# Krual-T/OutfitX

Hardware: AMD Instinct MI355X
Metric: outfits/sec CP forward (8-item sets, 224^2, bf16) (higher is better)
Workload: dtype f16

## Files before the change

include/ofx.h:

```cpp
#ifndef OFX_H
#define OFX_H
#include <stddef.h>
#include <stdint.h>

#ifdef __cplusplus
extern "C" {
#endif

#define OFX_ABI_VERSION 6

enum { OFX_OK = 0, OFX_EINVAL = -1, OFX_ESHAPE = -2, OFX_EHIP = -3, OFX_EWORKSPACE = -4, OFX_ESTATE = -5 };
enum ofx_dtype { OFX_F32 = 0, OFX_BF16 = 1, OFX_F16 = 2 };
enum ofx_act { OFX_ACT_NONE = 0, OFX_ACT_QUICK_GELU = 1, OFX_ACT_GELU = 2, OFX_ACT_MISH = 3, OFX_ACT_MISH_GRAD = 4 };
enum ofx_precision { OFX_PREC_BF16 = 0, OFX_PREC_F16 = 1, OFX_PREC_BF16X3 = 2, OFX_PREC_F16W2 = 3 };
enum ofx_out_kind { OFX_OUT_F32 = 0, OFX_OUT_OP = 1, OFX_OUT_SPLIT3 = 2 };

typedef struct ofx_handle ofx_handle;
typedef void* ofx_stream;

const char* ofx_last_error(void);
int ofx_abi_version(void);

typedef struct ofx_model_desc {
    int d_model, n_head, d_ffn, n_layers, max_items;
    int outfit_act;
    int outfit_precision;
    int vit_width, vit_layers, vit_heads, vit_mlp, vit_patch, vit_image, vit_act;
    int txt_width, txt_layers, txt_heads, txt_mlp, txt_vocab, txt_max_pos, txt_act, txt_eos_id;
    int proj_dim;
    int tower_precision;
    float ln_eps;
    int vit_w2_mask, txt_x3, proj_x3, vit_x3;
    int txt_w2_mask, vit_w2_qkv_layers, vit_w2_fc1_layers, vit_w2_out_layers, vit_w2_fc2_layers;
} ofx_model_desc;
enum { OFX_W2_PATCH = 1, OFX_W2_QKV = 2, OFX_W2_OUT = 4, OFX_W2_FC1 = 8, OFX_W2_FC2 = 16 };

void ofx_default_desc(ofx_model_desc* d);

ofx_handle* ofx_create(int device, const ofx_model_desc* desc);
void ofx_destroy(ofx_handle* h);

int ofx_pack_outfit_weights(ofx_handle* h, const void* const* fp32_params, int n_params, ofx_stream stream);
int ofx_pack_vision_weights(ofx_handle* h, const void* const* fp32_params, int n_params, ofx_stream stream);
int ofx_pack_text_weights(ofx_handle* h, const void* const* fp32_params, int n_params, ofx_stream stream);

enum ofx_op { OFX_OP_SET_ENCODER = 0, OFX_OP_VIT = 1, OFX_OP_TEXT = 2, OFX_OP_TOPK = 3 };
size_t ofx_workspace_bytes(ofx_handle* h, int op, int n, int len);

int ofx_set_encoder_fwd(ofx_handle* h, const float* x, const uint8_t* pad_mask, const float* prefix,
                        int prefix_stride, int B, int L, float* out_row0, void* ws, size_t ws_bytes,
                        ofx_stream stream);
int ofx_cp_head(ofx_handle* h, const float* row0, int B, float* logits, ofx_stream stream);
int ofx_cir_head(ofx_handle* h, const float* row0, int B, float* emb, void* ws, size_t ws_bytes, ofx_stream stream);
int ofx_cir_prefix(ofx_handle* h, const float* target_text_emb, int B, float* prefix_out, ofx_stream stream);

int ofx_vit_b32_fwd(ofx_handle* h, const float* pixels, int N, float* emb, int emb_ld, int emb_col,
                    int normalize, void* ws, size_t ws_bytes, ofx_stream stream);
int ofx_clip_text_fwd(ofx_handle* h, const int64_t* ids, const int64_t* attn_mask, const int* lengths_host,
                      int N, int T, float* emb, int emb_ld, int emb_col, int normalize, void* ws,
                      size_t ws_bytes, ofx_stream stream);
int ofx_clip_text_fwd_shared(ofx_handle* h, const int64_t* ids, const int64_t* attn_mask, const int* lengths_host,
                             int N, int T, float* emb, int emb_ld, int emb_col, int normalize, int shared_first, void* ws,
                             size_t ws_bytes, ofx_stream stream);

int ofx_fitb_argmin(const float* y_hat, const float* cand, int B, int C, int D, int64_t* idx, float* dist,
                    ofx_stream stream);
int ofx_fitb_argmin_indexed(const float* table, int ld, long long n_table, const int* cand_index, const float* y_hat, int B, int C, int D,
                            const int64_t* answer, int64_t* idx, float* dist, int* n_correct, ofx_stream stream);
// ... 32 lines not shown
int ofx_cp_train_fwd_indexed(ofx_handle* h, const float* table, int ld, long long n_table, const int* item_index, const int* cu_items,
                             int B, int max_len, float* logits, void* tape, size_t tape_bytes, void* ws, size_t ws_bytes,
                             float dropout_p, unsigned seed, ofx_stream stream);
int ofx_cir_train_fwd(ofx_handle* h, const float* x, const uint8_t* pad_mask, const float* table, int ld, long long n_table,
                      const int* item_index, const int* cu_items, const float* target_text, int B, int L, float* y, void* tape,
                      size_t tape_bytes, void* ws, size_t ws_bytes, float dropout_p, unsigned seed, ofx_stream stream);
int ofx_cir_train_bwd(ofx_handle* h, void* tape, size_t tape_bytes, const float* dy, int B, int L, float* grads, size_t grad_floats,
                      void* ws, size_t ws_bytes, float dropout_p, unsigned seed, ofx_stream stream);
int ofx_cp_train_bwd_into(ofx_handle* h, void* tape, size_t tape_bytes, const float* dlogits, int B, int L, float* const* grad_ptrs,
                          int n_ptrs, int accumulate, void* ws, size_t ws_bytes, float dropout_p, unsigned seed, ofx_stream stream);
int ofx_cir_train_bwd_into(ofx_handle* h, void* tape, size_t tape_bytes, const float* dy, int B, int L, float* const* grad_ptrs,
                           int n_ptrs, int accumulate, void* ws, size_t ws_bytes, float dropout_p, unsigned seed, ofx_stream stream);
int ofx_train_arm_layer_events(ofx_handle* h, void* const* events, int n);
int ofx_dropout_mask(float dropout_p, unsigned seed, int site, int rows, int cols, float* out, ofx_stream stream);
int ofx_focal_loss(const float* logits, const float* labels, int B, float alpha, float gamma, float upstream, float* loss, float* dlogits,
                   ofx_stream stream);
int ofx_focal_loss_ex(const float* logits, const float* labels, int B, float alpha, float gamma, float upstream, int reduction, float* loss,
                      float* per_elem, float* dlogits, ofx_stream stream);
size_t ofx_set_rank_loss_ws_bytes(int B, int K, int D);
int ofx_set_rank_loss(const float* y, const float* y_hat, const float* neg, const uint8_t* neg_mask, int B, int K, int D, float margin,
                      float upstream, float* loss, float* dy_hat, float* d_pos, float* d_neg, void* ws, size_t ws_bytes, ofx_stream stream);
int ofx_set_rank_loss_indexed(const float* table, int ld, long long n_table, const int* pos_index, const int* neg_index, const float* y_hat,
                              int B, int K, int D, float margin, float upstream, float* loss, float* dy_hat, float* d_pos, float* d_neg,
                              void* ws, size_t ws_bytes, ofx_stream stream);

int ofx_cir_sample_batch(const int* outfit_cu, const int* outfit_rows, int n_outfits, int n_outfit_rows, const int* pos_cu, const int* pos_slots,
                         int n_pos_slots, const int* pool_cu, const int* pool_rows, int n_pools, int n_pool_rows, const int* row_pool,
                         const int* row_slot, int n_table, const int* outfit_ids, int B, unsigned seed, unsigned draw, int K, int max_len,
                         int* item_index, int* cu_seqlens, int* target_item_index, int* neg_items_index, ofx_stream stream);

typedef struct ofx_opt_segment { float* param; long long offset; long long numel; } ofx_opt_segment;
size_t ofx_adamw_step_ws_bytes(long long n_arena);
int ofx_adamw_step(const ofx_opt_segment* segments, int n_segments, float* grad, float* exp_avg, float* exp_avg_sq, long long n_arena,
                   float* step, double lr, double beta1, double beta2, double eps, double weight_decay, double max_norm, double grad_scale,
                   float* grad_norm, int* skipped, void* ws, size_t ws_bytes, ofx_stream stream);

void ofx_profile_enable(int on);
int ofx_profile_read(double* ms, double* flops, long long* launches);
typedef struct ofx_prof_record { int cat, M, N, K, kind, kmul; float ms; double flops; double bytes; } ofx_prof_record;
int ofx_profile_records(ofx_prof_record* out, int cap);

int ofx_tune(int knob, int value);
unsigned ofx_config_generation(void);
int ofx_profile_enabled(void);
int ofx_stream_create_low_priority(int device, ofx_stream* out);
int ofx_stream_destroy(ofx_stream stream);

int ofx_gemm(const void* A, const void* W, void* C, const float* bias, const float* resid, int M, int N, int K,
             int lda, int ldc, int ldr, int act, int out_kind, int op_dtype, ofx_stream stream);
int ofx_gemm_w2(const void* A, const void* W2, void* C, const float* bias, const float* resid, int M, int N, int K,
                int lda, int ldc, int ldr, int act, int out_kind, int op_dtype, ofx_stream stream);
int ofx_gemm_x3(const void* A3, const void* W3, void* C, const float* bias, const float* resid, int M, int N, int K,
                int lda, int ldc, int ldr, int act, int out_kind, int op_dtype, ofx_stream stream);
int ofx_pack_lo8(const void* W2, void* W8, void* scale8, int N, int K, ofx_stream stream);
int ofx_gemm_w2f8(const void* A, const void* W2, const void* W8, const void* scale8, void* C, const float* bias, const float* resid, int M, int N, int K,
                  int lda, int ldc, int ldr, int act, int out_kind, ofx_stream stream);
int ofx_gemm_w2f8_fold(const void* A, const void* W2, const void* W8, const void* scale8, void* C, const float* bias, const float* row_stat, const float* col_sum,
                       int M, int N, int K, int lda, int ldc, int act, ofx_stream stream);
size_t ofx_gemm_tn_ws(int M, int N, int K);
int ofx_gemm_tn(const void* A, int lda, const void* B, int ldb, float* C, int ldc, int M, int N, int K, const int* k_dev,
                void* slab, size_t slab_bytes, int op_dtype, ofx_stream stream);
size_t ofx_gemm_splitk_ws(int M, int N, int K);
int ofx_gemm_splitk(const void* A, const void* W, void* C, const float* bias, const float* resid, int M, int N, int K,
                    int lda, int ldc, int ldr, int act, int out_kind, int op_dtype, void* slab, size_t slab_bytes, ofx_stream stream);
int ofx_gemm_train(const void* A, const void* W, void* C, const float* bias, const float* resid, float* aux_out, int M, const int* m_dev,
                   int N, int K, int lda, int ldc, int ldr, int act, int out_kind, float dropout_p, unsigned seed, int site, int op_dtype,
                   void* slab, size_t slab_bytes, ofx_stream stream);
int ofx_gemm_tn_into(const void* A, int lda, const void* B, int ldb, float* C, int ldc, int M, int N, int K, const int* k_dev,
                     int m_valid, int n_valid, int accumulate, void* slab, size_t slab_bytes, int op_dtype, ofx_stream stream);
int ofx_transpose_cast(const float* src, void* dst, int R, int C, int ldd, void* row_dst, int ld_row, int op_dtype, ofx_stream stream);
size_t ofx_layernorm_bwd_ws(int D);
int ofx_layernorm_bwd(const float* dy, const float* x, const float* stats, const float* gamma, const float* add, const int* add_map,
                      float* dx, void* dx_op, float* dgamma, float* dbeta, float* dcols, int M, const int* m_dev, int D, float dropout_p,
                      unsigned seed, int site, int accumulate, int op_dtype, void* ws, size_t ws_bytes, ofx_stream stream);
size_t ofx_colsum_ws(int C);
int ofx_colsum(const void* x, int x_kind, int ld, const int* gather, const float* row_scale, float* out0, float* out1, float* out2, int seg,
               int C, int valid, int M, const int* m_dev, int accumulate, int op_dtype, void* ws, size_t ws_bytes, ofx_stream stream);
int ofx_head_bwd(const float* dlogits, const float* w, const int* cu, float* dX, void* dXb, float* db, int B, int D, float dropout_p,
                 unsigned seed, int head_site, int below_site, int accumulate, int op_dtype, ofx_stream stream);
int ofx_gemm_fold_producer(const void* A, const void* W, const void* W8, const void* scale8, void* xb, void* xlo, float* stat_part, const float* bias,
                           const float* resid, int M, int N, int K, int lda, int ldr, int act, int w_form, int op_dtype, ofx_stream stream);
int ofx_gemm_fold(const void* A, const void* W, void* C, const float* bias, const float* row_stat, int stat_ld, const float* col_sum, int M, int N, int K,
                  int lda, int ldc, int act, int w_form, int op_dtype, ofx_stream stream);
int ofx_stats_finalize(const float* stat_part, int slots, int W, float eps, float* stat, int rows, ofx_stream stream);
int ofx_row_stats_cast(const float* x, void* xb, void* xlo, float* stat, int rows, int W, float eps, int op_dtype, ofx_stream stream);
int ofx_fold_pack(const float* w, const float* gamma, const float* beta, const float* bias, void* wf, float* col_sum, float* bias_f, int N, int K, int split,
                  int op_dtype, ofx_stream stream);
int ofx_vit_embed_ln(const float* patch_out, const float* cls, const float* pos, const float* gamma, const float* beta, float* x, void* xb, void* xlo,
                     float* stat, int N, int S, int D, float eps, int op_dtype, ofx_stream stream);
int ofx_gather_hilo(const void* hi, const void* lo, const int* idx, float* dst, int rows, int W, int op_dtype, ofx_stream stream);
int ofx_layernorm(const float* x, const int* row_idx, const float* gamma, const float* beta, void* y, int rows,
                  int D, int ldy, int out_kind, int op_dtype, float eps, ofx_stream stream);
int ofx_attention(const void* qkv, void* out, const int64_t* key_mask, int nseq, int seq_len, int n_head, int ld,
                  int ldo, int k_off, int v_off, int mask_ld, int causal, float scale, int op_dtype, ofx_stream stream);
int ofx_attention_ex(const void* qkv, void* out, const int64_t* key_mask, int nseq, int seq_len, int n_head, int ld, int ldo, int k_off,
                     int v_off, int mask_ld, int causal, int only_row0, int split3_w, float scale, int op_dtype, ofx_stream stream);
int ofx_set_attention(const float* qkv, void* out, const int* cu_seqlens, int nseq, int n_head, int D, int ldo,
                      int out_kind, int max_len, int only_row0, float scale, int op_dtype, ofx_stream stream);
int ofx_set_attention_slabs(const float* slabs, size_t plane_floats, int splits, const float* bias, void* out, const int* cu_seqlens, int nseq,
                            int n_head, int D, int ldo, int out_kind, int max_len, int only_row0, float scale, int op_dtype, ofx_stream stream);
int ofx_splitk_reduce_ln(const float* slab, size_t plane_floats, int splits, const float* bias, const float* resid, int ldr, float* x, int ldx,
                         const float* gamma, const float* beta, void* y, int ldy, int out_kind, float eps, int rows, const int* m_dev, int D,
                         int op_dtype, ofx_stream stream);
int ofx_attention_varlen(const void* qkv, void* out, const int* cu_seqlens, int nseq, int max_len, int n_head, int ld, int ldo, int k_off,
                         int v_off, int only_row0, float scale, float dropout_p, unsigned seed, int site, int op_dtype, ofx_stream stream);
int ofx_set_attention_op(const void* qkv, void* out, const int* cu_seqlens, int nseq, int n_head, int D, int ldo, int out_kind, int max_len,
                         int only_row0, float scale, float dropout_p, unsigned seed, int site, int op_dtype, ofx_stream stream);
int ofx_set_attention_bwd(const void* qkv, const float* d_o, void* dqkv, const int* cu_seqlens, int nseq, int n_head, int D, int max_len,
                          int only_row0, float scale, float dropout_p, unsigned seed, int site, int mfma, int op_dtype, ofx_stream stream);
int ofx_fused_qkv_attention(const void* X, const void* Wqkv, const float* bias, const float* row_stat, const float* col_sum, void* out,
                            int nseq, int seq_len, int width, int n_head, int ldx, int ldo, float scale, int op_dtype, ofx_stream stream);
int ofx_fused_qkv_attention_w2(const void* X, const void* Wqkv2, const float* bias, const float* row_stat, const float* col_sum, void* out,
                               int nseq, int seq_len, int width, int n_head, int ldx, int ldo, float scale, int op_dtype, ofx_stream stream);
int ofx_attention_f32(const float* qkv, void* out, const int64_t* key_mask, int nseq, int seq_len, int n_head, int D, int ldo, int out_kind,
                      int mask_ld, int causal, float scale, int op_dtype, ofx_stream stream);
int ofx_convert(const float* src, void* dst, int rows, int cols, int mode, int op_dtype, ofx_stream stream);

#ifdef __cplusplus
}
#endif
#endif
```

outfitx_amd/_lib.py:

```python
from __future__ import annotations

import ctypes as C
import os

_HERE = os.path.dirname(os.path.abspath(__file__))
LIB_PATH = os.environ.get("OFX_LIB") or os.path.join(_HERE, "libofx_hip.so")

OFX_OK = 0
ABI_VERSION = 6
F32, BF16, F16 = 0, 1, 2
ACT_NONE, ACT_QUICK_GELU, ACT_GELU, ACT_MISH = 0, 1, 2, 3
PREC_BF16, PREC_F16, PREC_BF16X3 = 0, 1, 2
OUT_F32, OUT_OP, OUT_SPLIT3 = 0, 1, 2
OP_SET_ENCODER, OP_VIT, OP_TEXT, OP_TOPK = 0, 1, 2, 3
PREC_F16W2 = 3
PRECISIONS = {"bf16": PREC_BF16, "f16": PREC_F16, "fp16": PREC_F16, "bf16x3": PREC_BF16X3, "f16w2": PREC_F16W2}
W2_PATCH, W2_QKV, W2_OUT, W2_FC1, W2_FC2 = 1, 2, 4, 8, 16
TOWER_SCHEMES = {
    "bf16": (PREC_BF16, 0, 0, 0, 0), "f16": (PREC_F16, 0, 0, 0, 0), "fp16": (PREC_F16, 0, 0, 0, 0),
    "f16w2": (PREC_F16, W2_PATCH | W2_OUT | W2_FC2, 1, 1, 0),
    "bf16w2": (PREC_BF16, W2_PATCH | W2_OUT | W2_FC2, 1, 1, 0),
    "f16w2q": (PREC_F16, W2_PATCH | W2_QKV | W2_OUT | W2_FC2, 1, 1, 0),
    "f16w2f": (PREC_F16, W2_PATCH | W2_OUT | W2_FC1 | W2_FC2, 1, 1, 0),
    "f16w2x": (PREC_F16, W2_PATCH | W2_QKV | W2_OUT | W2_FC1 | W2_FC2, 1, 1, 0),
    "f16x3": (PREC_F16, W2_PATCH, 1, 1, 1), "bf16x3": (PREC_BF16, W2_PATCH, 1, 1, 1),
}
SCHEME_ALIASES = {"f16w2h": "f16w2x@qkv=0-5"}
DEFAULT_TOWER_PRECISION = "f16w2x"


def _layer_bits(spec: str) -> int:
    m = 0
    for part in spec.split(","):
        a, _, b = part.partition("-")
        for l in range(int(a), int(b or a) + 1):
            m |= 1 << l
    return m


def tower_scheme(name: str) -> dict:
    name = SCHEME_ALIASES.get(name, name)
    base, _, opts = name.partition("@")
    if base not in TOWER_SCHEMES:
        raise ValueError(f"unknown tower_precision {name!r}; one of {sorted(list(TOWER_SCHEMES) + list(SCHEME_ALIASES))} [+ '@txt=w2;qkv=<layers>;fc1=<layers>']")
    prec, mask, txt_x3, proj_x3, vit_x3 = TOWER_SCHEMES[base]
    d = {"tower_precision": prec, "vit_w2_mask": mask, "txt_x3": txt_x3, "proj_x3": proj_x3, "vit_x3": vit_x3,
         "txt_w2_mask": 0, "vit_w2_qkv_layers": 0, "vit_w2_fc1_layers": 0, "vit_w2_out_layers": 0, "vit_w2_fc2_layers": 0}
    for o in filter(None, opts.split(";")):
        k, _, v = o.partition("=")
        try:
            if k == "txt" and v == "w2":
                d["txt_x3"], d["txt_w2_mask"] = 0, W2_QKV | W2_OUT | W2_FC1 | W2_FC2
            elif k in ("qkv", "fc1", "out", "fc2"):
                bits = _layer_bits(v) if v not in ("", "none") else 0
                if bits == 0:
                    d["vit_w2_mask"] &= ~{"qkv": W2_QKV, "fc1": W2_FC1, "out": W2_OUT, "fc2": W2_FC2}[k]
                d[f"vit_w2_{k}_layers"] = bits
            else:
                raise ValueError
        except ValueError:
            raise ValueError(f"tower_precision {name!r}: bad option {o!r} (txt=w2 | qkv= / fc1= / out= / fc2=<layers>, layers like 0-5,8 or none)") from None
    return d
ACTS = {"none": ACT_NONE, "quick_gelu": ACT_QUICK_GELU, "gelu": ACT_GELU, "mish": ACT_MISH}


class OfxError(RuntimeError):
# ... 29 lines not shown
    "ofx_pack_outfit_weights": (_i, [_vp, C.POINTER(_vp), _i, _vp]),
    "ofx_pack_vision_weights": (_i, [_vp, C.POINTER(_vp), _i, _vp]),
    "ofx_pack_text_weights": (_i, [_vp, C.POINTER(_vp), _i, _vp]),
    "ofx_workspace_bytes": (_sz, [_vp, _i, _i, _i]),
    "ofx_set_encoder_fwd": (_i, [_vp, _vp, _vp, _vp, _i, _i, _i, _vp, _vp, _sz, _vp]),
    "ofx_cp_head": (_i, [_vp, _vp, _i, _vp, _vp]),
    "ofx_cir_head": (_i, [_vp, _vp, _i, _vp, _vp, _sz, _vp]),
    "ofx_cir_prefix": (_i, [_vp, _vp, _i, _vp, _vp]),
    "ofx_vit_b32_fwd": (_i, [_vp, _vp, _i, _vp, _i, _i, _i, _vp, _sz, _vp]),
    "ofx_clip_text_fwd": (_i, [_vp, _vp, _vp, C.POINTER(_i), _i, _i, _vp, _i, _i, _i, _vp, _sz, _vp]),
    "ofx_clip_text_fwd_shared": (_i, [_vp, _vp, _vp, C.POINTER(_i), _i, _i, _vp, _i, _i, _i, _i, _vp, _sz, _vp]),
    "ofx_fitb_argmin": (_i, [_vp, _vp, _i, _i, _i, _vp, _vp, _vp]),
    "ofx_fitb_argmin_indexed": (_i, [_vp, _i, C.c_longlong, _vp, _vp, _i, _i, _i, _vp, _vp, _vp, _vp, _vp]),
    "ofx_l2_topk": (_i, [_vp, _vp, _vp, _i, _i, _i, _i, _i64, _vp, _vp, _vp, _sz, _vp]),
    "ofx_l2_topk_grouped_ws": (_sz, [_i, _i, _i]),
    "ofx_l2_topk_grouped": (_i, [_vp, _vp, _vp, _i, _i, _i, _i, _vp, _i, _i, _vp, _vp, _vp, _vp, _vp, _sz, _vp]),
    "ofx_topk_merge": (_i, [_vp, _vp, _i, _i, _i, _vp, _vp, _vp]),
    "ofx_clip_preprocess_ws": (_sz, [_vp, _vp, _i, _i, _i]),
    "ofx_clip_preprocess": (_i, [_vp, _vp, _vp, _vp, _i, _i, _i, _vp, _vp, _vp, _vp, _sz, _vp]),
    "ofx_clip_preprocess_patches": (_i, [_vp, _vp, _vp, _vp, _i, _i, _i, _i, _vp, _vp, _vp, _i, _vp, _sz, _vp]),
    "ofx_patchify": (_i, [_vp, _vp, _i, _i, _i, _i, _vp]),
    "ofx_vit_b32_u8_ws_bytes": (_sz, [_vp, _vp, _vp, _i, _i]),
    "ofx_vit_b32_fwd_u8": (_i, [_vp, _vp, _vp, _vp, _vp, _i, _i, _vp, _vp, _vp, _i, _i, _i, _vp, _sz, _vp]),
    "ofx_set_encoder_fwd_indexed": (_i, [_vp, _vp, _i, C.c_longlong, _vp, _vp, _vp, _i, _i, _i, _vp, _vp, _sz, _vp]),
    "ofx_cp_train_fwd_indexed": (_i, [_vp, _vp, _i, C.c_longlong, _vp, _vp, _i, _i, _vp, _vp, _sz, _vp, _sz, _f, C.c_uint, _vp]),
    "ofx_cp_train_tape_bytes": (_sz, [_vp, _i, _i]),
    "ofx_cp_train_ws_bytes": (_sz, [_vp, _i, _i]),
    "ofx_cp_train_grad_floats": (_sz, [_vp, C.POINTER(_sz), _i]),
    "ofx_cp_train_fwd": (_i, [_vp, _vp, _vp, _i, _i, _vp, _vp, _sz, _vp, _sz, _f, C.c_uint, _vp]),
    "ofx_cp_train_bwd": (_i, [_vp, _vp, _sz, _vp, _i, _i, _vp, _sz, _vp, _sz, _f, C.c_uint, _vp]),
    "ofx_cir_train_fwd": (_i, [_vp, _vp, _vp, _vp, _i, C.c_longlong, _vp, _vp, _vp, _i, _i, _vp, _vp, _sz, _vp, _sz, _f, C.c_uint, _vp]),
    "ofx_cir_train_bwd": (_i, [_vp, _vp, _sz, _vp, _i, _i, _vp, _sz, _vp, _sz, _f, C.c_uint, _vp]),
    "ofx_cp_train_bwd_into": (_i, [_vp, _vp, _sz, _vp, _i, _i, C.POINTER(_vp), _i, _i, _vp, _sz, _f, C.c_uint, _vp]),
    "ofx_cir_train_bwd_into": (_i, [_vp, _vp, _sz, _vp, _i, _i, C.POINTER(_vp), _i, _i, _vp, _sz, _f, C.c_uint, _vp]),
    "ofx_train_arm_layer_events": (_i, [_vp, C.POINTER(_vp), _i]),
    "ofx_dropout_mask": (_i, [_f, C.c_uint, _i, _i, _i, _vp, _vp]),
    "ofx_focal_loss": (_i, [_vp, _vp, _i, _f, _f, _f, _vp, _vp, _vp]),
    "ofx_focal_loss_ex": (_i, [_vp, _vp, _i, _f, _f, _f, _i, _vp, _vp, _vp, _vp]),
    "ofx_set_rank_loss_ws_bytes": (_sz, [_i, _i, _i]),
    "ofx_set_rank_loss": (_i, [_vp, _vp, _vp, _vp, _i, _i, _i, _f, _f, _vp, _vp, _vp, _vp, _vp, _sz, _vp]),
    "ofx_set_rank_loss_indexed": (_i, [_vp, _i, C.c_longlong, _vp, _vp, _vp, _i, _i, _i, _f, _f, _vp, _vp, _vp, _vp, _vp, _sz, _vp]),
    "ofx_cir_sample_batch": (_i, [_vp, _vp, _i, _i, _vp, _vp, _i, _vp, _vp, _i, _i, _vp, _vp, _i, _vp, _i, C.c_uint, C.c_uint, _i, _i, _vp, _vp, _vp, _vp, _vp]),
    "ofx_adamw_step_ws_bytes": (_sz, [C.c_longlong]),
    "ofx_adamw_step": (_i, [_vp, _i, _vp, _vp, _vp, C.c_longlong, _vp] + [C.c_double] * 7 + [_vp, _vp, _vp, _sz, _vp]),
    "ofx_profile_enable": (None, [_i]),
    "ofx_profile_read": (_i, [C.POINTER(C.c_double), C.POINTER(C.c_double), C.POINTER(C.c_longlong)]),
    "ofx_profile_records": (_i, [C.POINTER(ProfRecord), _i]),
    "ofx_tune": (_i, [_i, _i]),
    "ofx_config_generation": (C.c_uint, []),
    "ofx_profile_enabled": (_i, []),
    "ofx_gemm": (_i, [_vp, _vp, _vp, _vp, _vp, _i, _i, _i, _i, _i, _i, _i, _i, _i, _vp]),
    "ofx_gemm_w2": (_i, [_vp, _vp, _vp, _vp, _vp, _i, _i, _i, _i, _i, _i, _i, _i, _i, _vp]),
    "ofx_gemm_x3": (_i, [_vp, _vp, _vp, _vp, _vp, _i, _i, _i, _i, _i, _i, _i, _i, _i, _vp]),
    "ofx_pack_lo8": (_i, [_vp, _vp, _vp, _i, _i, _vp]),
    "ofx_gemm_w2f8": (_i, [_vp, _vp, _vp, _vp, _vp, _vp, _vp, _i, _i, _i, _i, _i, _i, _i, _i, _vp]),
    "ofx_gemm_w2f8_fold": (_i, [_vp, _vp, _vp, _vp, _vp, _vp, _vp, _vp, _i, _i, _i, _i, _i, _i, _vp]),
    "ofx_gemm_tn_ws": (_sz, [_i, _i, _i]),
    "ofx_gemm_tn": (_i, [_vp, _i, _vp, _i, _vp, _i, _i, _i, _i, _vp, _vp, _sz, _i, _vp]),
    "ofx_gemm_splitk_ws": (_sz, [_i, _i, _i]),
    "ofx_gemm_splitk": (_i, [_vp, _vp, _vp, _vp, _vp, _i, _i, _i, _i, _i, _i, _i, _i, _i, _vp, _sz, _vp]),
    "ofx_gemm_train": (_i, [_vp, _vp, _vp, _vp, _vp, _vp, _i, _vp, _i, _i, _i, _i, _i, _i, _i, _f, C.c_uint, _i, _i, _vp, _sz, _vp]),
    "ofx_gemm_tn_into": (_i, [_vp, _i, _vp, _i, _vp, _i, _i, _i, _i, _vp, _i, _i, _i, _vp, _sz, _i, _vp]),
    "ofx_transpose_cast": (_i, [_vp, _vp, _i, _i, _i, _vp, _i, _i, _vp]),
    "ofx_layernorm_bwd_ws": (_sz, [_i]),
    "ofx_layernorm_bwd": (_i, [_vp] * 11 + [_i, _vp, _i, _f, C.c_uint, _i, _i, _i, _vp, _sz, _vp]),
    "ofx_colsum_ws": (_sz, [_i]),
    "ofx_colsum": (_i, [_vp, _i, _i, _vp, _vp, _vp, _vp, _vp, _i, _i, _i, _i, _vp, _i, _i, _vp, _sz, _vp]),
    "ofx_head_bwd": (_i, [_vp, _vp, _vp, _vp, _vp, _vp, _i, _i, _f, C.c_uint, _i, _i, _i, _i, _vp]),
    "ofx_gemm_fold_producer": (_i, [_vp] * 9 + [_i] * 8 + [_vp]),
    "ofx_gemm_fold": (_i, [_vp, _vp, _vp, _vp, _vp, _i, _vp, _i, _i, _i, _i, _i, _i, _i, _i, _vp]),
    "ofx_stats_finalize": (_i, [_vp, _i, _i, _f, _vp, _i, _vp]),
    "ofx_row_stats_cast": (_i, [_vp, _vp, _vp, _vp, _i, _i, _f, _i, _vp]),
    "ofx_fold_pack": (_i, [_vp] * 7 + [_i, _i, _i, _i, _vp]),
    "ofx_vit_embed_ln": (_i, [_vp] * 9 + [_i, _i, _i, _f, _i, _vp]),
    "ofx_gather_hilo": (_i, [_vp, _vp, _vp, _vp, _i, _i, _i, _vp]),
    "ofx_layernorm": (_i, [_vp, _vp, _vp, _vp, _vp, _i, _i, _i, _i, _i, _f, _vp]),
    "ofx_attention": (_i, [_vp, _vp, _vp, _i, _i, _i, _i, _i, _i, _i, _i, _i, _f, _i, _vp]),
    "ofx_attention_ex": (_i, [_vp, _vp, _vp, _i, _i, _i, _i, _i, _i, _i, _i, _i, _i, _i, _f, _i, _vp]),
    "ofx_set_attention_slabs": (_i, [_vp, _sz, _i, _vp, _vp, _vp, _i, _i, _i, _i, _i, _i, _i, _f, _i, _vp]),
    "ofx_splitk_reduce_ln": (_i, [_vp, _sz, _i, _vp, _vp, _i, _vp, _i, _vp, _vp, _vp, _i, _i, _f, _i, _vp, _i, _i, _vp]),
    "ofx_fused_qkv_attention": (_i, [_vp, _vp, _vp, _vp, _vp, _vp, _i, _i, _i, _i, _i, _i, _f, _i, _vp]),
    "ofx_fused_qkv_attention_w2": (_i, [_vp, _vp, _vp, _vp, _vp, _vp, _i, _i, _i, _i, _i, _i, _f, _i, _vp]),
    "ofx_set_attention": (_i, [_vp, _vp, _vp, _i, _i, _i, _i, _i, _i, _i, _f, _i, _vp]),
    "ofx_attention_varlen": (_i, [_vp, _vp, _vp, _i, _i, _i, _i, _i, _i, _i, _i, _f, _f, C.c_uint, _i, _i, _vp]),
    "ofx_set_attention_op": (_i, [_vp, _vp, _vp, _i, _i, _i, _i, _i, _i, _i, _f, _f, C.c_uint, _i, _i, _vp]),
    "ofx_set_attention_bwd": (_i, [_vp, _vp, _vp, _vp, _i, _i, _i, _i, _i, _f, _f, C.c_uint, _i, _i, _i, _vp]),
    "ofx_attention_f32": (_i, [_vp, _vp, _vp, _i, _i, _i, _i, _i, _i, _i, _i, _f, _i, _vp]),
    "ofx_convert": (_i, [_vp, _vp, _i, _i, _i, _i, _vp]),
}

_lib = None


def load() -> C.CDLL:
    global _lib
    if _lib is not None:
        return _lib
    if not os.path.exists(LIB_PATH):
        raise OfxError(f"{LIB_PATH} not found: build it with `make` (or __graft_entry__.build()); "
                       "outfitx_amd has no CPU/PyTorch fallback for the scoring path")
    lib = C.CDLL(LIB_PATH)
    for name, (res, args) in SIGNATURES.items():
        fn = getattr(lib, name)
        fn.restype, fn.argtypes = res, args
    if lib.ofx_abi_version() != ABI_VERSION:
        raise OfxError("libofx_hip.so ABI version mismatch; rebuild")
    for kv in filter(None, os.environ.get("OFX_TUNE", "").split(",")):
        knob, _, val = kv.partition(":")
        if lib.ofx_tune(int(knob), int(val)) != OFX_OK:
            raise OfxError(f"OFX_TUNE: ofx_tune({knob}, {val}) was refused")
    _lib = lib
    return lib


def check(rc: int, what: str = "") -> None:
    if rc != OFX_OK:
        msg = load().ofx_last_error()
        raise OfxError(f"{what or 'ofx call'} failed (code {rc}): {msg.decode() if msg else ''}")


def default_desc() -> ModelDesc:
    d = ModelDesc()
    load().ofx_default_desc(C.byref(d))
    return d
```

outfitx_amd/csrc/api.hip:

```cpp
#include <stdarg.h>
#include <string.h>

#include <algorithm>
#include <vector>
#include <mutex>
#include <cstring>

#include "ofx_weights.h"

static thread_local char g_err[512] = "";
void ofx_set_error(const char* fmt, ...) {
    va_list ap;
    va_start(ap, fmt);
    vsnprintf(g_err, sizeof(g_err), fmt, ap);
    va_end(ap);
}
extern "C" const char* ofx_last_error(void) { return g_err; }
extern "C" int ofx_abi_version(void) { return OFX_ABI_VERSION; }
extern "C" int ofx_stream_create_low_priority(int device, ofx_stream* out) {
    OFX_REQUIRE(out, OFX_EINVAL, "stream_create_low_priority: NULL argument");
    int prev = 0, least = 0, greatest = 0;
    OFX_HIP(hipGetDevice(&prev));
    OFX_HIP(hipSetDevice(device));
    hipStream_t s = nullptr;
// ... 499 lines not shown
    if (fused) {
        TRY(ofx_launch_fused_qkv_attn(w.XB, L.qkv.w, L.qkv.bias, w.S, L.qkv.col_sum, w.H, nseq, S, W, heads, W, W, 0.125f, dt, s, L.qkv.form == W_SPLIT));
    } else {
        GemmArgs g1{}; g1.A = w.XB; g1.C = w.QKV; g1.row_stat = w.S; g1.M = rows; g1.N = 3 * W;
        g1.ldc = 3 * W; g1.act = OFX_ACT_NONE; g1.out_kind = OFX_OUT_OP;
        use_gemm(g1, L.qkv, W);
        const bool prune = pool_idx && pool_first && g_prune_q;
        if (prune) {
            GemmArgs kv = g1;
            kv.W = (const char*)g1.W + (size_t)W * g1.K * 2; kv.bias = g1.bias + W; kv.col_sum = g1.col_sum + W; kv.C = (char*)w.QKV + (size_t)W * 2; kv.N = 2 * W;
            if (g1.W8) { kv.W8 = (const char*)g1.W8 + (size_t)W * W; kv.w8_scale = (const char*)g1.w8_scale + W; }
            TRY(ofx_launch_gemm(kv, dt, s));
            GemmArgs q = g1;
            q.M = nseq; q.N = W; q.lda = S * W; q.ldc = S * 3 * W; q.stat_ld = S;
            TRY(ofx_launch_gemm(q, dt, s));
        } else
            TRY(ofx_launch_gemm(g1, dt, s));
        AttnArgs at{w.QKV, w.H, key_mask, nseq, S, heads, 3 * W, W, W, 2 * W, mask_ld, causal, 0.125f};
        at.only_row0 = prune ? 1 : 0;
        TRY(ofx_launch_attention_mfma(at, dt, s));
    }
    char* H = w.H; char* U = w.U; int M = rows;
    if (pool_idx) {
        TRY(ofx_launch_gather_rows(w.H, pool_idx, w.HP, nseq, W * 2, W * 2, s));
        TRY(ofx_launch_gather_hilo(w.XB, w.XLO, pool_idx, w.XP, nseq, W, dt, s));
        H = w.HP; U = w.UP; M = nseq;
    }
    auto to_stream = [&](GemmArgs& g) {
        g.M = M; g.N = W; g.ldc = W; g.ldr = W; g.act = OFX_ACT_NONE;
        if (pool_idx) { g.C = w.XP; g.resid = w.XP; g.out_kind = OFX_OUT_F32; g.slab = w.slab; g.slab_bytes = w.slab_bytes; }
        else { g.C = w.XB; g.xb_out = w.XB; g.xlo = w.XLO; g.stat_part = w.P; g.out_kind = OFX_OUT_OP; }
    };
    GemmArgs g2{}; g2.A = H;
    use_gemm(g2, L.o, W); to_stream(g2);
    TRY(ofx_launch_gemm(g2, dt, s));
    GemmArgs g3{}; g3.C = U; g3.M = M; g3.N = MLP; g3.ldc = MLP; g3.act = act; g3.out_kind = OFX_OUT_OP;
    if (pool_idx) {
        LnArgs ln2{w.XP, nullptr, L.g2, L.be2, H, M, W, W, OFX_OUT_OP, eps};
        TRY(ofx_launch_layernorm(ln2, dt, s));
        g3.A = H; g3.slab = w.slab; g3.slab_bytes = w.slab_bytes;
    } else {
        TRY(ofx_launch_stats_finalize(w.P, W / 64, W, eps, w.S, M, s));
        g3.A = w.XB; g3.row_stat = w.S;
    }
    use_gemm(g3, L.fc1, W);
    TRY(ofx_launch_gemm(g3, dt, s));
    GemmArgs g4{}; g4.A = U;
    use_gemm(g4, L.fc2, MLP); to_stream(g4);
    TRY(ofx_launch_gemm(g4, dt, s));
    if (!pool_idx) TRY(ofx_launch_stats_finalize(w.P, W / 64, W, eps, w.S, M, s));
    return OFX_OK;
}

static int clip_layer_x3(const ClipLayer& L, const ClipWs& w, int rows, int nseq, int S, int W, int MLP, int heads, int act,
                         float eps, int causal, const int64_t* key_mask, int mask_ld, int dt, const int* pool_idx, hipStream_t s, bool mfma_attn = false,
                         int shared_first = 0) {
    LnArgs ln{w.X, nullptr, L.g1, L.be1, w.H, rows, W, 3 * W, OFX_OUT_SPLIT3, eps};
    TRY(ofx_launch_layernorm(ln, dt, s));
    GemmArgs g1{}; g1.A = w.H; g1.C = w.QKV; g1.M = rows; g1.N = 3 * W;
    use_gemm(g1, L.qkv, W);
    const bool f32_attn = S <= 64 && !mfma_attn;
    OFX_REQUIRE(!shared_first || f32_attn, OFX_EINVAL, "clip_layer_x3: a shared first row needs the fp32 set attention");
    g1.ldc = 3 * W; g1.act = OFX_ACT_NONE; g1.out_kind = f32_attn ? OFX_OUT_F32 : OFX_OUT_OP;
    TRY(ofx_launch_gemm(g1, dt, s));
    if (f32_attn) {
        SetAttnArgs sa{w.QKV, w.H, nullptr, nseq, heads, W, 3 * W, OFX_OUT_SPLIT3, S, 0, 0.125f};
        sa.fixed_len = S; sa.causal = causal; sa.key_mask = key_mask; sa.mask_ld = mask_ld; sa.shared_first = shared_first;
        TRY(ofx_launch_set_attention(sa, dt, s));
    } else {
        AttnArgs at{w.QKV, w.H, key_mask, nseq, S, heads, 3 * W, 3 * W, W, 2 * W, mask_ld, causal, 0.125f};
        at.split3_w = W;
        TRY(ofx_launch_attention_mfma(at, dt, s));
    }
    float* X = w.X; char* H = w.H; char* U = w.U; int M = rows;
    if (pool_idx) {
        TRY(ofx_launch_gather_rows(w.H, pool_idx, w.HP, nseq, 3 * W * 2, 3 * W * 2, s));
        TRY(ofx_launch_gather_rows(w.X, pool_idx, w.XP, nseq, W * 4, W * 4, s));
        X = w.XP; H = w.HP; U = w.UP; M = nseq;
    }
    GemmArgs g2{}; g2.A = H; g2.C = X; g2.resid = X; g2.M = M; g2.N = W; g2.ldc = W; g2.ldr = W; g2.act = OFX_ACT_NONE; g2.out_kind = OFX_OUT_F32;
    use_gemm(g2, L.o, W);
    if (pool_idx) { g2.slab = w.slab; g2.slab_bytes = w.slab_bytes; }
    TRY(ofx_launch_gemm(g2, dt, s));
    LnArgs ln2{X, nullptr, L.g2, L.be2, H, M, W, 3 * W, OFX_OUT_SPLIT3, eps};
    TRY(ofx_launch_layernorm(ln2, dt, s));
    GemmArgs g3{}; g3.A = H; g3.C = U; g3.M = M; g3.N = MLP; g3.ldc = 3 * MLP; g3.act = act; g3.out_kind = OFX_OUT_SPLIT3;
    use_gemm(g3, L.fc1, W);
    if (pool_idx) { g3.slab = w.slab; g3.slab_bytes = w.slab_bytes; }
    TRY(ofx_launch_gemm(g3, dt, s));
    GemmArgs g4{}; g4.A = U; g4.C = X; g4.resid = X; g4.M = M; g4.N = W; g4.ldc = W; g4.ldr = W; g4.act = OFX_ACT_NONE; g4.out_kind = OFX_OUT_F32;
    use_gemm(g4, L.fc2, MLP);
    if (pool_idx) { g4.slab = w.slab; g4.slab_bytes = w.slab_bytes; }
    return ofx_launch_gemm(g4, dt, s);
}

static int clip_layers(const std::vector<ClipLayer>& Ls, const ClipWs& w, int rows, int nseq, int S, int W, int MLP,
                       int heads, int act, float eps, int causal, const int64_t* key_mask, int mask_ld, int dt,
                       const int* pool_idx, hipStream_t s, bool pool_first, bool x3, int shared_first = 0) {
    OFX_REQUIRE(!shared_first || x3, OFX_EINVAL, "clip_layers: a shared first row exists in the three-product path only");
    if (x3) {
        for (size_t l = 0; l < Ls.size(); ++l)
            TRY(clip_layer_x3(Ls[l], w, rows, nseq, S, W, MLP, heads, act, eps, causal, key_mask, mask_ld, dt, l + 1 == Ls.size() ? pool_idx : nullptr, s, !causal && !key_mask && !g_x3_vit_f32_attn,
                              shared_first));
        return OFX_OK;
    }
    for (size_t l = 0; l < Ls.size(); ++l)
        TRY(clip_layer(Ls[l], w, rows, nseq, S, W, MLP, heads, act, eps, causal, key_mask, mask_ld, dt,
                       l + 1 == Ls.size() ? pool_idx : nullptr, s, pool_first));
    return OFX_OK;
}

struct RawImages {
    const uint8_t* src; const long long* offsets; const int* heights; const int* widths; int channels; const float* mean; const float* stdv;
    void* ws; size_t ws_bytes;
};

static int vit_core(ofx_handle* h, const float* pixels, const RawImages* raw, int N, float* emb, int emb_ld, int emb_col,
                    int normalize, void* ws, size_t ws_bytes, ofx_stream stream) {
    OFX_REQUIRE(h && h->vis_ready, OFX_ESTATE, "vit_b32_fwd: vision weights not packed");
    OFX_REQUIRE((pixels || raw) && emb && ws && N > 0, OFX_EINVAL, "vit_b32_fwd: bad argument");
    const ofx_model_desc& d = h->d;
    OFX_REQUIRE(emb_ld >= emb_col + d.proj_dim && emb_ld % 4 == 0 && emb_col % 4 == 0, OFX_ESHAPE, "vit_b32_fwd: bad emb_ld/emb_col");
    hipStream_t s = (hipStream_t)stream;
    const int g = d.vit_image / d.vit_patch, S = g * g + 1, W = d.vit_width, KP = 3 * d.vit_patch * d.vit_patch, dt = h->tw_dtype;
    int chunk = std::min(N, VIT_CHUNK_MAX);
    while (chunk > 1 && vit_bytes(h, chunk, nullptr, nullptr, ~(size_t)0) > ws_bytes) chunk = (chunk + 1) / 2;
    OFX_REQUIRE(vit_bytes(h, chunk, nullptr, nullptr, ~(size_t)0) <= ws_bytes, OFX_EWORKSPACE, "vit_b32_fwd: workspace %zu bytes cannot hold one image", ws_bytes);
    const size_t px_per_img = (size_t)3 * d.vit_image * d.vit_image;
    for (int n0 = 0; n0 < N; n0 += chunk) {
        const int n = std::min(chunk, N - n0);
        ClipWs w;
        vit_bytes(h, n, &w, ws, ws_bytes);
        const int rows = n * S;
        if (raw)
            TRY(ofx_preprocess_to(raw->src, raw->offsets + n0, raw->heights + n0, raw->widths + n0, n, raw->channels, d.vit_image, raw->mean, raw->stdv,
                                  nullptr, w.U, d.vit_patch, dt, raw->ws, raw->ws_bytes, s));
        else
            TRY(ofx_launch_patchify(pixels + (size_t)n0 * px_per_img, w.U, n, d.vit_image, d.vit_patch, dt, s));
        GemmArgs gp{}; gp.A = w.U; gp.C = w.QKV; gp.M = n * g * g; gp.N = W; gp.ldc = W;
        gp.act = OFX_ACT_NONE; gp.out_kind = OFX_OUT_F32;
        use_gemm(gp, h->v_patch, KP);
        TRY(ofx_launch_gemm(gp, dt, s));
        TRY(ofx_launch_vit_embed_ln((const float*)w.QKV, h->v_cls, h->v_pos, h->v_pre_g, h->v_pre_b, w.X, n, S, W, d.ln_eps, s, w.XB, w.S, dt, w.XLO));
        TRY(ofx_launch_iota_rows(w.idx, n, S, s));
        TRY(clip_layers(h->vl, w, rows, n, S, W, d.vit_mlp, d.vit_heads, d.vit_act, d.ln_eps, 0, nullptr, 0, dt, w.idx, s, true, h->vit_x3 != 0));
// ... 430 lines not shown
extern "C" int ofx_cir_sample_batch(const int* outfit_cu, const int* outfit_rows, int n_outfits, int n_outfit_rows, const int* pos_cu, const int* pos_slots,
                                    int n_pos_slots, const int* pool_cu, const int* pool_rows, int n_pools, int n_pool_rows, const int* row_pool,
                                    const int* row_slot, int n_table, const int* outfit_ids, int B, unsigned seed, unsigned draw, int K, int max_len,
                                    int* item_index, int* cu_seqlens, int* target_item_index, int* neg_items_index, ofx_stream stream) {
    OFX_REQUIRE(B >= 1, OFX_EINVAL, "cir_sample_batch: B = %d; needs B >= 1", B);
    OFX_REQUIRE(K >= 0 && K <= 64 && max_len >= 1 && max_len <= 31, OFX_ESHAPE, "cir_sample_batch: K = %d, max_len = %d; needs 0 <= K <= 64, 1 <= max_len <= 31",
                K, max_len);
    OFX_REQUIRE(n_outfits >= 1 && n_table >= 1 && n_outfit_rows >= 0 && n_pos_slots >= 0 && n_pools >= 0 && n_pool_rows >= 0, OFX_ESHAPE,
                "cir_sample_batch: n_outfits = %d, n_table = %d (both >= 1), n_outfit_rows = %d, n_pos_slots = %d, n_pools = %d, n_pool_rows = %d (all >= 0)",
                n_outfits, n_table, n_outfit_rows, n_pos_slots, n_pools, n_pool_rows);
    OFX_REQUIRE((long long)B * std::max(K, max_len) <= INT_MAX, OFX_ESHAPE, "cir_sample_batch: B * max(K, max_len) = %lld exceeds INT_MAX",
                (long long)B * std::max(K, max_len));
    const void* ptrs[] = {outfit_cu, outfit_rows, pos_cu, pos_slots, pool_cu, pool_rows, row_pool, row_slot, outfit_ids, item_index, cu_seqlens, target_item_index};
    uintptr_t bits = (uintptr_t)neg_items_index;
    for (const void* p : ptrs) {
        OFX_REQUIRE(p, OFX_EINVAL, "cir_sample_batch: NULL argument");
        bits |= (uintptr_t)p;
    }
    OFX_REQUIRE(neg_items_index || K == 0, OFX_EINVAL, "cir_sample_batch: NULL neg_items_index with K = %d", K);
    OFX_REQUIRE((bits & 15) == 0, OFX_EINVAL, "cir_sample_batch: every array must be 16-byte aligned");
    CirSampleArgs a{outfit_cu, outfit_rows, pos_cu, pos_slots, pool_cu, pool_rows, row_pool, row_slot, outfit_ids,
                    n_outfits, n_outfit_rows, n_pos_slots, n_pools, n_pool_rows, n_table, B, K, max_len, seed, draw,
                    item_index, cu_seqlens, target_item_index, neg_items_index};
    return ofx_launch_cir_sample_batch(a, (hipStream_t)stream);
}

static bool adamw_shape_ok(long long n_arena) { return n_arena > 0 && n_arena % 64 == 0; }
extern "C" size_t ofx_adamw_step_ws_bytes(long long n_arena) { return adamw_shape_ok(n_arena) ? ofx_adamw_step_ws(n_arena) : 0; }
extern "C" int ofx_adamw_step(const ofx_opt_segment* segments, int n_segments, float* grad, float* exp_avg, float* exp_avg_sq, long long n_arena,
                              float* step, double lr, double beta1, double beta2, double eps, double weight_decay, double max_norm, double grad_scale,
                              float* grad_norm, int* skipped, void* ws, size_t ws_bytes, ofx_stream stream) {
    OFX_REQUIRE(segments && grad && exp_avg && exp_avg_sq && step && grad_norm && skipped && ws, OFX_EINVAL, "adamw_step: NULL argument");
    OFX_REQUIRE(n_segments >= 1 && n_segments <= 1024, OFX_ESHAPE, "adamw_step: n_segments = %d; needs 1 <= n_segments <= 1024", n_segments);
    OFX_REQUIRE(adamw_shape_ok(n_arena), OFX_ESHAPE, "adamw_step: n_arena = %lld; needs a positive multiple of 64", n_arena);
    OFX_REQUIRE((((uintptr_t)grad | (uintptr_t)exp_avg | (uintptr_t)exp_avg_sq | (uintptr_t)ws) & 15) == 0 && ((uintptr_t)segments & 7) == 0, OFX_EINVAL,
                "adamw_step: grad, exp_avg, exp_avg_sq and ws must be 16-byte aligned, segments 8-byte aligned");
    OFX_REQUIRE(ws_bytes >= ofx_adamw_step_ws(n_arena), OFX_EWORKSPACE, "adamw_step: workspace %zu < %zu bytes", ws_bytes, ofx_adamw_step_ws(n_arena));
    return ofx_launch_adamw_step(segments, n_segments, grad, exp_avg, exp_avg_sq, n_arena, step, lr, beta1, beta2, eps, weight_decay, max_norm,
                                 grad_scale, grad_norm, skipped, ws, (hipStream_t)stream);
}

extern "C" int ofx_tune(int knob, int value) {
    ++g_config_generation;
    switch (knob) {
        case 2: case 5: case 11: case 15: case 16: case 18: return ofx_gemm_tune(knob, value);
        case 6: if (value != 2) { ofx_set_error("ofx_tune(6): %d is not 2 (the towers' LayerNorms are always folded)", value); return OFX_EINVAL; } return OFX_OK;
        case 7: g_train_mfma_attn = value; return OFX_OK;
        case 8: g_prune_q = value; return OFX_OK;
        case 9: g_fuse_qkv = value; return OFX_OK;
        case 10: g_set_fuse = value; return OFX_OK;
        case 17: g_topk_filter = value != 0; return OFX_OK;
        case 20: g_x3_vit_f32_attn = value != 0; return OFX_OK;
        case 21: g_text_shared_first = value != 0; return OFX_OK;
        default: ofx_set_error("ofx_tune: unknown knob %d", knob); return OFX_EINVAL;
    }
}

static GemmArgs op_gemm(const void* A, const void* W, void* C, const float* bias, const float* resid, int M, int N, int K, int lda, int ldc, int ldr,
                        int act, int out_kind) {
    GemmArgs g{}; g.A = A; g.W = W; g.C = C; g.bias = bias; g.resid = resid; g.M = M; g.N = N; g.K = K; g.lda = lda; g.ldc = ldc;
    g.ldr = ldr; g.act = act; g.out_kind = out_kind;
    return g;
}
extern "C" int ofx_gemm(const void* A, const void* W, void* C, const float* bias, const float* resid, int M, int N, int K,
                        int lda, int ldc, int ldr, int act, int out_kind, int op_dtype, ofx_stream stream) {
    return ofx_launch_gemm(op_gemm(A, W, C, bias, resid, M, N, K, lda, ldc, ldr, act, out_kind), op_dtype, (hipStream_t)stream);
}
extern "C" int ofx_gemm_w2(const void* A, const void* W2, void* C, const float* bias, const float* resid, int M, int N, int K,
                           int lda, int ldc, int ldr, int act, int out_kind, int op_dtype, ofx_stream stream) {
    GemmArgs g = op_gemm(A, W2, C, bias, resid, M, N, 2 * K, lda, ldc, ldr, act, out_kind); g.a_wrap = K;
    return ofx_launch_gemm(g, op_dtype, (hipStream_t)stream);
}
extern "C" int ofx_gemm_x3(const void* A3, const void* W3, void* C, const float* bias, const float* resid, int M, int N, int K,
                           int lda, int ldc, int ldr, int act, int out_kind, int op_dtype, ofx_stream stream) {
    GemmArgs g = op_gemm(A3, W3, C, bias, resid, M, N, 3 * K, lda, ldc, ldr, act, out_kind); g.k_mult = 3;
    return ofx_launch_gemm(g, op_dtype, (hipStream_t)stream);
}
extern "C" int ofx_pack_lo8(const void* W2, void* W8, void* scale8, int N, int K, ofx_stream stream) {
    return ofx_launch_pack_lo8(W2, W8, scale8, N, K, (hipStream_t)stream);
}
extern "C" int ofx_gemm_w2f8(const void* A, const void* W2, const void* W8, const void* scale8, void* C, const float* bias, const float* resid, int M, int N, int K,
                             int lda, int ldc, int ldr, int act, int out_kind, ofx_stream stream) {
    GemmArgs g = op_gemm(A, W2, C, bias, resid, M, N, 2 * K, lda, ldc, ldr, act, out_kind); g.a_wrap = K; g.W8 = W8; g.w8_scale = scale8;
    return ofx_launch_gemm(g, OFX_F16, (hipStream_t)stream);
}
extern "C" int ofx_gemm_w2f8_fold(const void* A, const void* W2, const void* W8, const void* scale8, void* C, const float* bias, const float* row_stat, const float* col_sum,
                                  int M, int N, int K, int lda, int ldc, int act, ofx_stream stream) {
    OFX_REQUIRE(row_stat && col_sum, OFX_EINVAL, "gemm_w2f8_fold: row_stat and col_sum are required");
    GemmArgs g = op_gemm(A, W2, C, bias, nullptr, M, N, 2 * K, lda, ldc, 0, act, OFX_OUT_OP); g.a_wrap = K; g.W8 = W8; g.w8_scale = scale8;
    g.row_stat = row_stat; g.col_sum = col_sum; g.stat_ld = 1;
    return ofx_launch_gemm(g, OFX_F16, (hipStream_t)stream);
}
extern "C" size_t ofx_gemm_splitk_ws(int M, int N, int K) { return ofx_gemm_splitk_bytes(M, N, K); }
extern "C" int ofx_gemm_splitk(const void* A, const void* W, void* C, const float* bias, const float* resid, int M, int N, int K,
                               int lda, int ldc, int ldr, int act, int out_kind, int op_dtype, void* slab, size_t slab_bytes, ofx_stream stream) {
    GemmArgs g = op_gemm(A, W, C, bias, resid, M, N, K, lda, ldc, ldr, act, out_kind); g.slab = slab; g.slab_bytes = slab_bytes;
    return ofx_launch_gemm(g, op_dtype, (hipStream_t)stream);
}
extern "C" size_t ofx_gemm_tn_ws(int M, int N, int K) { return ofx_gemm_tn_slab_bytes(M, N, K); }
extern "C" int ofx_gemm_tn(const void* A, int lda, const void* B, int ldb, float* C, int ldc, int M, int N, int K, const int* k_dev,
                           void* slab, size_t slab_bytes, int op_dtype, ofx_stream stream) {
    return ofx_launch_gemm_tn(A, lda, B, ldb, C, ldc, M, N, K, k_dev, slab, slab_bytes, op_dtype, (hipStream_t)stream);
}
static bool op_dtype_ok(int op_dtype) { return op_dtype == OFX_BF16 || op_dtype == OFX_F16; }
static bool drop_p_ok(float p) { return p >= 0.f && p < 1.f; }
static bool aligned_to(size_t mask, std::initializer_list<const void*> ptrs) {
    for (const void* p : ptrs) if ((uintptr_t)p & mask) return false;
    return true;
}
extern "C" int ofx_gemm_train(const void* A, const void* W, void* C, const float* bias, const float* resid, float* aux_out, int M, const int* m_dev,
                              int N, int K, int lda, int ldc, int ldr, int act, int out_kind, float dropout_p, unsigned seed, int site, int op_dtype,
                              void* slab, size_t slab_bytes, ofx_stream stream) {
    OFX_REQUIRE(A && W && C && drop_p_ok(dropout_p) && (act != OFX_ACT_MISH_GRAD || resid), OFX_EINVAL, "gemm_train: bad argument");
    OFX_REQUIRE(aligned_to(15, {bias, resid, aux_out, slab}) && aligned_to(3, {m_dev}), OFX_EINVAL,
                "gemm_train: bias, resid, aux_out and slab must be 16-byte aligned");
    GemmArgs g = op_gemm(A, W, C, bias, resid, M, N, K, lda, ldc, ldr, act, out_kind); g.slab = slab; g.slab_bytes = slab_bytes;
    g.aux_out = aux_out; g.m_dev = m_dev; g.drop = make_drop(dropout_p, seed, (unsigned)site);
    return ofx_launch_gemm(g, op_dtype, (hipStream_t)stream);
}
extern "C" int ofx_gemm_tn_into(const void* A, int lda, const void* B, int ldb, float* C, int ldc, int M, int N, int K, const int* k_dev,
                                int m_valid, int n_valid, int accumulate, void* slab, size_t slab_bytes, int op_dtype, ofx_stream stream) {
    OFX_REQUIRE(A && B && C && m_valid >= 0 && n_valid >= 0, OFX_EINVAL, "gemm_tn_into: bad argument");
    OFX_REQUIRE(aligned_to(15, {slab}) && aligned_to(3, {k_dev}), OFX_EINVAL, "gemm_tn_into: slab must be 16-byte aligned");
    return ofx_launch_gemm_tn(A, lda, B, ldb, C, ldc, M, N, K, k_dev, slab, slab_bytes, op_dtype, (hipStream_t)stream, m_valid, n_valid, accumulate ? 1 : 0);
}
extern "C" int ofx_transpose_cast(const float* src, void* dst, int R, int C, int ldd, void* row_dst, int ld_row, int op_dtype, ofx_stream stream) {
    OFX_REQUIRE(src && dst && op_dtype_ok(op_dtype), OFX_EINVAL, "transpose_cast: bad argument");
    OFX_REQUIRE(aligned_to(3, {src}) && aligned_to(1, {dst, row_dst}), OFX_EINVAL, "transpose_cast: misaligned pointer");
    OFX_REQUIRE(R > 0 && C > 0, OFX_ESHAPE, "transpose_cast: R=%d C=%d", R, C);
// ... 149 lines not shown
                                    const float* gamma, const float* beta, void* y, int ldy, int out_kind, float eps, int rows, const int* m_dev, int D,
                                    int op_dtype, ofx_stream stream) {
    OFX_REQUIRE(slab && x && gamma && beta && y && op_dtype_ok(op_dtype) && aligned_to(15, {slab, bias, resid, x, gamma, beta}) && aligned_to(out_kind == 0 ? 15 : 7, {y}) && aligned_to(3, {m_dev}) &&
                    plane_floats % 4 == 0,
                OFX_EINVAL, "splitk_reduce_ln: bad argument (a NULL or misaligned pointer or op_dtype = %d)", op_dtype);
    OFX_REQUIRE(out_kind >= 0 && out_kind <= 2 && (splits <= 1 || plane_floats >= (size_t)rows * D), OFX_ESHAPE, "splitk_reduce_ln: out_kind=%d, or slabs that overlap", out_kind);
    SplitKLnArgs a{slab, plane_floats, splits, bias, resid, ldr, x, ldx, gamma, beta, y, ldy, out_kind, eps, rows, D, m_dev};
    return ofx_launch_splitk_reduce_ln(a, op_dtype, (hipStream_t)stream);
}
extern "C" int ofx_fused_qkv_attention(const void* X, const void* Wqkv, const float* bias, const float* row_stat, const float* col_sum, void* out,
                                       int nseq, int seq_len, int width, int n_head, int ldx, int ldo, float scale, int op_dtype, ofx_stream stream) {
    return ofx_launch_fused_qkv_attn(X, Wqkv, bias, row_stat, col_sum, out, nseq, seq_len, width, n_head, ldx, ldo, scale, op_dtype, (hipStream_t)stream);
}
extern "C" int ofx_fused_qkv_attention_w2(const void* X, const void* Wqkv2, const float* bias, const float* row_stat, const float* col_sum, void* out,
                                          int nseq, int seq_len, int width, int n_head, int ldx, int ldo, float scale, int op_dtype, ofx_stream stream) {
    return ofx_launch_fused_qkv_attn(X, Wqkv2, bias, row_stat, col_sum, out, nseq, seq_len, width, n_head, ldx, ldo, scale, op_dtype, (hipStream_t)stream, true);
}
extern "C" int ofx_set_attention(const float* qkv, void* out, const int* cu_seqlens, int nseq, int n_head, int D, int ldo,
                                 int out_kind, int max_len, int only_row0, float scale, int op_dtype, ofx_stream stream) {
    SetAttnArgs a{qkv, out, cu_seqlens, nseq, n_head, D, ldo, out_kind, max_len, only_row0, scale};
    return ofx_launch_set_attention(a, op_dtype, (hipStream_t)stream);
}
static bool train_attn_args_ok(const void* a, const void* b, const void* c, int nseq, float dropout_p) {
    return a && b && c && nseq > 0 && dropout_p >= 0.f && dropout_p < 1.f;
}
extern "C" int ofx_attention_varlen(const void* qkv, void* out, const int* cu_seqlens, int nseq, int max_len, int n_head, int ld, int ldo, int k_off,
                                    int v_off, int only_row0, float scale, float dropout_p, unsigned seed, int site, int op_dtype, ofx_stream stream) {
    OFX_REQUIRE(train_attn_args_ok(qkv, out, cu_seqlens, nseq, dropout_p), OFX_EINVAL, "attention_varlen: bad argument");
    OFX_REQUIRE(n_head > 0 && k_off == n_head * 64 && v_off == 2 * k_off && ld >= 3 * k_off, OFX_ESHAPE,
                "attention_varlen: q | k | v rows of D = n_head * 64 columns (k_off=%d v_off=%d ld=%d n_head=%d); heads of 96 take ofx_set_attention", k_off, v_off, ld, n_head);
    AttnArgs a{qkv, out, nullptr, nseq, max_len, n_head, ld, ldo, k_off, v_off, 0, 0, scale};
    a.cu_seqlens = cu_seqlens; a.only_row0 = only_row0 ? 1 : 0; a.drop = make_drop(dropout_p, seed, (unsigned)site);
    return ofx_launch_attention_mfma(a, op_dtype, (hipStream_t)stream);
}
extern "C" int ofx_set_attention_op(const void* qkv, void* out, const int* cu_seqlens, int nseq, int n_head, int D, int ldo, int out_kind, int max_len,
                                    int only_row0, float scale, float dropout_p, unsigned seed, int site, int op_dtype, ofx_stream stream) {
    OFX_REQUIRE(train_attn_args_ok(qkv, out, cu_seqlens, nseq, dropout_p) && n_head > 0, OFX_EINVAL, "set_attention_op: bad argument");
    SetAttnArgs a{qkv, out, cu_seqlens, nseq, n_head, D, ldo, out_kind, max_len, only_row0 ? 1 : 0, scale};
    a.drop = make_drop(dropout_p, seed, (unsigned)site); a.qkv_op = 1;
    return ofx_launch_set_attention(a, op_dtype, (hipStream_t)stream);
}
extern "C" int ofx_set_attention_bwd(const void* qkv, const float* d_o, void* dqkv, const int* cu_seqlens, int nseq, int n_head, int D, int max_len,
                                     int only_row0, float scale, float dropout_p, unsigned seed, int site, int mfma, int op_dtype, ofx_stream stream) {
    OFX_REQUIRE(train_attn_args_ok(qkv, d_o, dqkv, nseq, dropout_p) && cu_seqlens && n_head > 0, OFX_EINVAL, "set_attention_bwd: bad argument");
    const auto launch = mfma ? ofx_launch_set_attention_bwd_mfma : ofx_launch_set_attention_bwd;
    return launch(qkv, d_o, dqkv, cu_seqlens, nseq, n_head, D, max_len, scale, op_dtype, make_drop(dropout_p, seed, (unsigned)site), only_row0 ? 1 : 0, (hipStream_t)stream);
}
extern "C" int ofx_attention_f32(const float* qkv, void* out, const int64_t* key_mask, int nseq, int seq_len, int n_head, int D, int ldo, int out_kind,
                                 int mask_ld, int causal, float scale, int op_dtype, ofx_stream stream) {
    SetAttnArgs a{qkv, out, nullptr, nseq, n_head, D, ldo, out_kind, seq_len, 0, scale};
    a.fixed_len = seq_len; a.causal = causal; a.key_mask = key_mask; a.mask_ld = mask_ld;
    return ofx_launch_set_attention(a, op_dtype, (hipStream_t)stream);
}
extern "C" int ofx_convert(const float* src, void* dst, int rows, int cols, int mode, int op_dtype, ofx_stream stream) {
    return ofx_launch_pack_rows(src, dst, rows, rows, cols, cols, cols, mode, op_dtype, (hipStream_t)stream);
}
```

outfitx_amd/csrc/attention.hip:

```cpp
#include "attn_wave.h"

namespace {

struct AttnK {
    const char* qkv;
    char* out;
    const int64_t* key_mask;
    int nseq, S, n_head, ld, ldo, k_off, v_off, mask_ld, causal;
    float scale;
    const int* cu;
    int only_row0;
    DropArgs drop;
    int split3_w;
};

template <typename T, int NT>
__global__ __launch_bounds__(256, 3) void attention_mfma_kernel(AttnK a) {
    typedef typename OpT<T>::v8 v8;
    constexpr int KS = attn_ksteps(NT), VROWS = 32 * KS, VT = VROWS * ATTN_V_ROW;
    __shared__ __attribute__((aligned(16))) char smem[4 * VT];
    const int lane = threadIdx.x & 63, wave = threadIdx.x >> 6;
    const int npairs = a.nseq * a.n_head;
    const int pair_raw = blockIdx.x * 4 + wave;
    const bool live = pair_raw < npairs;
    const int pair = live ? pair_raw : npairs - 1;
    const int seq = pair / a.n_head, head = pair % a.n_head;
    const int row_first = a.cu ? a.cu[seq] : seq * a.S;
    const int S = a.cu ? min(a.cu[seq + 1] - row_first, 16 * NT) : a.S;
    const T* base = (const T*)a.qkv + (size_t)row_first * a.ld + head * 64;
    const int r16 = lane & 15, q4 = lane >> 4;

    OFX_LDS char* vl = (OFX_LDS char*)smem + wave * VT;
#pragma unroll
    for (int it = 0; it < VROWS / 8; ++it) {
        const int key = it * 8 + (lane >> 3);
        v8 val;
#pragma unroll
        for (int e = 0; e < 8; ++e) val[e] = (T)0.0f;
        if (key < S) val = *(const v8*)(base + (size_t)key * a.ld + a.v_off + (lane & 7) * 8);
        *(OFX_LDS v8*)(vl + key * ATTN_V_ROW + (lane & 7) * 16) = val;
    }

    v8 kf[NT][2], qf[NT][2];
#pragma unroll
    for (int t = 0; t < NT; ++t) {
        int row = 16 * t + r16;
        row = row < S ? row : S - 1;
        const T* rp = base + (size_t)row * a.ld + q4 * 8;
#pragma unroll
        for (int ks = 0; ks < 2; ++ks) {
            kf[t][ks] = *(const v8*)(rp + a.k_off + ks * 32);
            qf[t][ks] = *(const v8*)(rp + ks * 32);
        }
// ... 148 lines not shown
        for (int c = 0; c < C4; ++c) {
            const f32x4 x = qp[c], y = kp[c];
            d += x[0] * y[0] + x[1] * y[1] + x[2] * y[2] + x[3] * y[3];
        }
        bool dead = a.causal && j > i;
        if (!dead && a.key_mask) dead = a.key_mask[(size_t)mb * a.mask_ld + j] == 0;
        sc[i * (SMAX + 4) + j] = dead ? -INFINITY : d * a.scale;
    }
    __syncthreads();
    if (lane >= q0 && lane < nq) {
        float* row = sc + lane * (SMAX + 4);
        float m = -INFINITY;
        for (int j = 0; j < S; ++j) m = fmaxf(m, row[j]);
        if (m == -INFINITY) m = 0.f;
        float sum = 0.f;
        for (int j = 0; j < S; ++j) { const float e = expf(row[j] - m); row[j] = e; sum += e; }
        const float inv = sum > 0.f ? 1.0f / sum : 0.f;
        if (a.drop.thresh) for (int j = 0; j < S; ++j) row[j] *= inv * drop_mul(a.drop, blockIdx.x, lane * 32 + j);
        else for (int j = 0; j < S; ++j) row[j] *= inv;
    }
    __syncthreads();
    if (a.out_kind == 0) {
        for (int i = q0; i < nq; ++i) {
            const float* row = sc + i * (SMAX + 4);
            float acc = 0.f;
#pragma unroll
            for (int j = 0; j < SMAX; ++j) acc += (j < S ? row[j] : 0.f) * vreg[j];
            ((float*)a.out)[(size_t)row_of(i) * a.ldo + h * HD + lane] = acc;
            if constexpr (WIDE) {
                float acc2 = 0.f;
#pragma unroll
                for (int j = 0; j < SMAX; ++j) acc2 += (j < S ? row[j] : 0.f) * vreg2[j];
                if (two) ((float*)a.out)[(size_t)row_of(i) * a.ldo + h * HD + 64 + lane] = acc2;
            }
        }
        return;
    }
    for (int i = q0; i < nq; ++i) {
        const float* row = sc + i * (SMAX + 4);
        float acc = 0.f;
#pragma unroll
        for (int j = 0; j < SMAX; ++j) acc += (j < S ? row[j] : 0.f) * vreg[j];
        qs[i * STR + lane] = acc;
        if constexpr (WIDE) {
            float acc2 = 0.f;
#pragma unroll
            for (int j = 0; j < SMAX; ++j) acc2 += (j < S ? row[j] : 0.f) * vreg2[j];
            if (two) qs[i * STR + 64 + lane] = acc2;
        }
    }
    __syncthreads();
    auto store_row = [&](int i, int c8) {
        const f32x4 x0 = *(const f32x4*)(qs + i * STR + c8), x1 = *(const f32x4*)(qs + i * STR + c8 + 4);
        store8<T>(a.out, (size_t)row_of(i) * a.ldo + h * HD + c8, x0, x1, a.out_kind, D);
    };
    if constexpr (!WIDE) {
        const int c8 = (lane & 7) * 8, r8 = lane >> 3;
        for (int i0 = 0; i0 < nq; i0 += 8) {
            const int i = i0 + r8;
            if (i >= q0 && i < nq) store_row(i, c8);
        }
    } else {
        for (int f = lane + q0 * C8; f < nq * C8; f += 64) store_row(f / C8, (f % C8) * 8);
    }
}


struct AttnBwdK {
    const char* qkv;
    const float* d_o;
    char* dqkv;
    const int* cu;
    int nseq, n_head, D, only_row0;
    float scale;
    DropArgs drop;
};

__device__ __forceinline__ float drop_dp(float dp, float mk) {
#pragma clang fp contract(off)
    return dp * mk;
}

template <typename T, int NT>
__global__ __launch_bounds__(256) void set_attention_bwd_mfma_kernel(AttnBwdK a) {
    typedef typename OpT<T>::v8 v8;
    typedef typename OpT<T>::v4 v4;
    constexpr int KS = attn_ksteps(NT), VROWS = 32 * KS, VT = VROWS * ATTN_V_ROW;
    __shared__ __attribute__((aligned(16))) char smem[4 * 3 * VT];
    const int lane = threadIdx.x & 63, wave = threadIdx.x >> 6;
    const int npairs = a.nseq * a.n_head;
    const int pair_raw = blockIdx.x * 4 + wave;
    const bool live = pair_raw < npairs;
    const int pair = live ? pair_raw : npairs - 1;
    const int seq = pair / a.n_head, head = pair % a.n_head;
    const int D = a.D, ld = 3 * D;
    const int row_first = a.cu[seq];
    const int S = min(a.cu[seq + 1] - row_first, 16 * NT);
    const T* base = (const T*)a.qkv + (size_t)row_first * ld + head * 64;
    const int r16 = lane & 15, q4 = lane >> 4;
    const int n_go = a.only_row0 ? 1 : S;

    OFX_LDS char* kl = (OFX_LDS char*)smem + wave * 3 * VT;
    OFX_LDS char* ql = kl + VT;
    OFX_LDS char* gl = ql + VT;
#pragma unroll
    for (int it = 0; it < VROWS / 8; ++it) {
        const int row = it * 8 + (lane >> 3), c8 = (lane & 7) * 8;
        v8 kv, qv, gv;
#pragma unroll
        for (int e = 0; e < 8; ++e) { kv[e] = (T)0.0f; qv[e] = (T)0.0f; gv[e] = (T)0.0f; }
        if (row < S) {
            kv = *(const v8*)(base + (size_t)row * ld + D + c8);
            qv = *(const v8*)(base + (size_t)row * ld + c8);
        }
        if (row < n_go) {
            const float* gp = a.d_o + (size_t)(a.only_row0 ? seq : row_first + row) * D + head * 64 + c8;
// ... 129 lines not shown
        for (int nd = 0; nd < 4; ++nd) {
            v8 af[KS];
#pragma unroll
            for (int ks = 0; ks < KS; ++ks) af[ks] = attn_tr_frag<T>(img, 32 * ks, 16 * nd + 4 * (r16 & 3));
#pragma unroll
            for (int u = 0; u < NT; ++u) {
                f32x4 c = {0.f, 0.f, 0.f, 0.f};
#pragma unroll
                for (int ks = 0; ks < KS; ++ks) c = OpT<T>::mfma16(af[ks], bop[u][ks], c);
                const int orow = 16 * u + r16;
                if (live && orow < n_rows_out) {
                    v4 o;
#pragma unroll
                    for (int r = 0; r < 4; ++r) o[r] = (T)c[r];
                    *(v4*)(obase + (size_t)orow * ld + col_off + 16 * nd + 4 * q4) = o;
                }
            }
        }
    };
    product(kl, dsT, 0, S);
    product(ql, dsN, D, S);
    product(gl, pdN, 2 * D, S);
}

}

int ofx_launch_attention_mfma(const AttnArgs& g, int op_dtype, hipStream_t s) {
    OFX_REQUIRE(g.seq_len >= 1 && g.seq_len <= 64, OFX_ESHAPE, "attention: seq_len=%d must be in [1,64]", g.seq_len);
    OFX_REQUIRE(g.nseq > 0 && g.n_head > 0, OFX_ESHAPE, "attention: nseq=%d n_head=%d", g.nseq, g.n_head);
    OFX_REQUIRE(g.seq_len <= 32 || !g.drop.thresh, OFX_ESHAPE, "attention: dropout columns are keyed query * 32 + key");
    OFX_REQUIRE(g.ld % 8 == 0 && g.ldo % 4 == 0 && g.k_off % 8 == 0 && g.v_off % 8 == 0, OFX_ESHAPE, "attention: strides must keep 16-byte alignment");
    OFX_REQUIRE((uintptr_t)g.qkv % 16 == 0 && (uintptr_t)g.out % 8 == 0, OFX_EINVAL, "attention: misaligned pointers");
    AttnK k;
    k.qkv = (const char*)g.qkv; k.out = (char*)g.out; k.key_mask = g.key_mask; k.nseq = g.nseq; k.S = g.seq_len;
    k.n_head = g.n_head; k.ld = g.ld; k.ldo = g.ldo; k.k_off = g.k_off; k.v_off = g.v_off; k.mask_ld = g.mask_ld;
    k.causal = g.causal; k.scale = g.scale; k.cu = g.cu_seqlens; k.only_row0 = g.only_row0; k.drop = g.drop; k.split3_w = g.split3_w;
    OFX_REQUIRE(g.split3_w == 0 || (g.split3_w % 8 == 0 && g.ldo >= 3 * g.split3_w), OFX_ESHAPE, "attention: split3 output needs ldo >= 3 W");
    const int grid = (g.nseq * g.n_head + 3) / 4;
    ProfScope prof(PROF_ATTN, s);
#define AT(T, N) hipLaunchKernelGGL((attention_mfma_kernel<T, N>), dim3(grid), dim3(256), 0, s, k)
    const int nt = g.seq_len <= 16 ? 1 : g.seq_len <= 32 ? 2 : 4;
    if (op_dtype == OFX_F16) { if (nt == 1) AT(f16_t, 1); else if (nt == 2) AT(f16_t, 2); else AT(f16_t, 4); }
    else { if (nt == 1) AT(bf16_t, 1); else if (nt == 2) AT(bf16_t, 2); else AT(bf16_t, 4); }
#undef AT
    OFX_LAUNCH_CHECK();
    return OFX_OK;
}

int ofx_launch_set_attention(const SetAttnArgs& g, int op_dtype, hipStream_t s) {
    OFX_REQUIRE(g.n_head > 0 && (g.D == g.n_head * 64 || g.D == g.n_head * 96), OFX_ESHAPE, "set_attention: head_dim must be 64 or 96 (D=%d heads=%d)", g.D, g.n_head);
    const bool wide = g.D == g.n_head * 96;
    OFX_REQUIRE(g.max_len >= 1 && g.max_len <= 64, OFX_ESHAPE, "set_attention: %d rows per sequence exceed 64", g.max_len);
    OFX_REQUIRE(g.max_len <= 32 || !g.drop.thresh, OFX_ESHAPE, "set_attention: dropout columns are keyed query * 32 + key");
    OFX_REQUIRE(g.ldo >= (g.out_kind == 2 ? 3 * g.D : g.D) && (g.out_kind == 0 || g.ldo % 8 == 0), OFX_ESHAPE, "set_attention: bad ldo=%d (operand-type rows leave as 16-byte stores)", g.ldo);
    OFX_REQUIRE(g.cu_seqlens || (g.fixed_len >= 1 && g.fixed_len <= g.max_len), OFX_EINVAL, "set_attention: needs cu_seqlens or a fixed length <= max_len");
    SetK k;
    k.qkv = g.qkv; k.out = (char*)g.out; k.cu = g.cu_seqlens; k.nseq = g.nseq; k.n_head = g.n_head; k.D = g.D; k.ldo = g.ldo;
    k.out_kind = g.out_kind; k.only_row0 = g.only_row0; k.scale = g.scale; k.drop = g.drop;
    k.fixed_S = g.fixed_len; k.causal = g.causal; k.mask_ld = g.mask_ld; k.key_mask = g.key_mask;
    OFX_REQUIRE(!g.shared_first || (!g.cu_seqlens && g.causal && g.fixed_len >= 2 && !g.only_row0 && !g.qkv_op && g.splits <= 1 && !g.drop.thresh), OFX_EINVAL,
                "set_attention: a shared first row needs the fixed-length causal mode on fp32 q|k|v, >= 2 rows per sequence, all queries, no slabs, no dropout");
    k.shared_first = g.shared_first ? 1 : 0;
    OFX_REQUIRE(g.splits <= 1 || (!g.qkv_op && g.bias && g.plane > 0 && g.max_len <= 32), OFX_EINVAL, "set_attention: slab input needs fp32 q|k|v, the bias, the slab stride and sets of <= 32 rows");
    k.splits = g.splits > 1 ? g.splits : 1; k.plane = g.plane; k.bias = g.bias;
    const int grid = (g.nseq + (g.shared_first ? 1 : 0)) * g.n_head;
    ProfScope prof(PROF_ATTN, s);
#define SA(T, N) do { if (wide) { if (g.qkv_op) hipLaunchKernelGGL((set_attention_kernel<T, N, T, 96>), dim3(grid), dim3(64), 0, s, k); \
                                      else hipLaunchKernelGGL((set_attention_kernel<T, N, float, 96>), dim3(grid), dim3(64), 0, s, k); } \
                      else if (g.qkv_op) hipLaunchKernelGGL((set_attention_kernel<T, N, T>), dim3(grid), dim3(64), 0, s, k); \
                      else hipLaunchKernelGGL((set_attention_kernel<T, N, float>), dim3(grid), dim3(64), 0, s, k); } while (0)
    if (op_dtype == OFX_F16) { if (g.max_len <= 8) SA(f16_t, 8); else if (g.max_len <= 20) SA(f16_t, 20); else if (g.max_len <= 32) SA(f16_t, 32); else SA(f16_t, 64); }
    else { if (g.max_len <= 8) SA(bf16_t, 8); else if (g.max_len <= 20) SA(bf16_t, 20); else if (g.max_len <= 32) SA(bf16_t, 32); else SA(bf16_t, 64); }
#undef SA
    OFX_LAUNCH_CHECK();
    return OFX_OK;
}

int ofx_launch_set_attention_bwd_mfma(const void* qkv, const float* d_o, void* dqkv, const int* cu, int nseq, int n_head, int D, int max_len,
                                      float scale, int op_dtype, const DropArgs& drop, int only_row0, hipStream_t s) {
    OFX_REQUIRE(D == n_head * 64 && max_len >= 1 && max_len <= 32, OFX_ESHAPE, "set_attention_bwd_mfma: bad shape");
    AttnBwdK k{(const char*)qkv, d_o, (char*)dqkv, cu, nseq, n_head, D, only_row0, scale, drop};
    const int grid = (nseq * n_head + 3) / 4;
    ProfScope prof(PROF_ATTN, s);
#define AB(T, N) hipLaunchKernelGGL((set_attention_bwd_mfma_kernel<T, N>), dim3(grid), dim3(256), 0, s, k)
    if (op_dtype == OFX_F16) { if (max_len <= 16) AB(f16_t, 1); else AB(f16_t, 2); }
    else { if (max_len <= 16) AB(bf16_t, 1); else AB(bf16_t, 2); }
#undef AB
    OFX_LAUNCH_CHECK();
    return OFX_OK;
}
```

outfitx_amd/csrc/gemm.hip:

```cpp
#include "gemm_common.h"

namespace {
template <typename T, int MT = 4>
__global__ __launch_bounds__(256, 2) void gemm_128x128_kernel(KArgs p) {
    constexpr int BMT = 32 * MT, STAGE_T = (BMT + BN) * BK * 2, EPI_T = 16 * MT * EPI_STRIDE * 4;
    typedef typename OpT<T>::v8 v8;
    extern __shared__ __attribute__((aligned(16))) char smem[];
    OFX_LDS char* lds = (OFX_LDS char*)smem;

    const int tid = threadIdx.x, lane = tid & 63;
    const int wave = __builtin_amdgcn_readfirstlane(tid >> 6);
    const int wm = wave >> 1, wn = wave & 1;

    int tm, tn;
    grouped_tile(xcd_remap(blockIdx.x, p.nwg), p.group_m, p.tiles_m, p.tiles_n, tm, tn);
    const int m0 = tm * BMT, n0 = tn * BN;
    if (clamp_live_rows(p.m_dev, p.M, m0)) return;

    const int lrow = lane >> 3, lchk = lane & 7;
    const char* a_src[MT];
    const char* w_src[4];
#pragma unroll
    for (int i = 0; i < 4; ++i) {
        const int c = wave * 4 + i;
// ... 55 lines not shown
        __builtin_amdgcn_s_setprio(1);
#pragma unroll
        for (int ks = 0; ks < 2; ++ks)
#pragma unroll
            for (int i = 0; i < MT; ++i)
#pragma unroll
                for (int j = 0; j < 4; ++j) acc[i][j] = OpT<T>::mfma16(wf[ks][j], af[ks][i], acc[i][j]);
        __builtin_amdgcn_s_setprio(0);
        asm volatile("s_waitcnt lgkmcnt(0)" ::: "memory");
        __builtin_amdgcn_s_barrier();
    }

    OFX_LDS float* ep = (OFX_LDS float*)(lds + wave * EPI_T);
#pragma unroll
    for (int i = 0; i < MT; ++i)
#pragma unroll
        for (int j = 0; j < 4; ++j)
            *(OFX_LDS f32x4*)(ep + (i * 16 + fr) * EPI_STRIDE + j * 16 + fq * 4) = acc[i][j];
    asm volatile("s_waitcnt lgkmcnt(0)" ::: "memory");
    if (p.splits > 1) {
        KArgs q = p;
        q.C = (char*)(p.slab + (size_t)blockIdx.y * p.m_slab * p.N); q.ldc = p.N; q.out_kind = 0; q.bias = nullptr; q.resid = nullptr; q.aux_out = nullptr; q.drop.thresh = 0;
        epilogue<T, OFX_ACT_NONE>(q, ep, m0 + wm * 16 * MT, n0 + wn * 64, lane, 16 * MT);
        return;
    }
    switch (p.act) {
        case OFX_ACT_QUICK_GELU: epilogue<T, OFX_ACT_QUICK_GELU>(p, ep, m0 + wm * 16 * MT, n0 + wn * 64, lane, 16 * MT); break;
        case OFX_ACT_GELU: epilogue<T, OFX_ACT_GELU>(p, ep, m0 + wm * 16 * MT, n0 + wn * 64, lane, 16 * MT); break;
        case OFX_ACT_MISH: epilogue<T, OFX_ACT_MISH>(p, ep, m0 + wm * 16 * MT, n0 + wn * 64, lane, 16 * MT); break;
        case OFX_ACT_MISH_GRAD: epilogue<T, OFX_ACT_MISH_GRAD>(p, ep, m0 + wm * 16 * MT, n0 + wn * 64, lane, 16 * MT); break;
        default: epilogue<T, OFX_ACT_NONE>(p, ep, m0 + wm * 16 * MT, n0 + wn * 64, lane, 16 * MT); break;
    }
}


}

static GemmKnobs g_knobs;
int ofx_gemm_tune(int knob, int value) {
    switch (knob) {
        case 2: g_knobs.kernel = value; return OFX_OK;
        case 5:
            if (value >= 2 && (value & 0xff) == 0) { ofx_set_error("ofx_tune(5): %d forces a split-K plan of 0 slices (low byte = slices, 1-16)", value); return OFX_EINVAL; }
            g_knobs.splitk = value; return OFX_OK;
        case 11: g_knobs.w2_persist = value; return OFX_OK;
        case 15: g_knobs.x3_kernel = value; return OFX_OK;
        case 16: g_knobs.x3_persist = value != 0; return OFX_OK;
        case 18: if (value != 0 && value != 1) { ofx_set_error("ofx_tune(18): %d is not 0 or 1", value); return OFX_EINVAL; } g_knobs.epi_direct = value; return OFX_OK;
        default: ofx_set_error("ofx_tune: unknown knob %d", knob); return OFX_EINVAL;
    }
}
size_t ofx_gemm_splitk_bytes(int M, int N, int K) { return gemm_splitk_slab_bytes(M, N, K, g_knobs); }

int ofx_launch_gemm(const GemmArgs& g, int op_dtype, hipStream_t s) {
    OFX_REQUIRE(g.M > 0 && g.N > 0 && g.K > 0, OFX_ESHAPE, "gemm: empty problem M=%d N=%d K=%d", g.M, g.N, g.K);
    OFX_REQUIRE(g.N % BN == 0, OFX_ESHAPE, "gemm: N=%d must be a multiple of %d (pad the weight at pack time)", g.N, BN);
    OFX_REQUIRE(g.K % BK == 0, OFX_ESHAPE, "gemm: K=%d must be a multiple of %d", g.K, BK);
    OFX_REQUIRE(g.a_wrap == 0 || (g.a_wrap > 0 && g.a_wrap % BK == 0 && g.K % g.a_wrap == 0), OFX_ESHAPE, "gemm: a_wrap=%d must be a multiple of %d dividing K=%d", g.a_wrap, BK, g.K);
    const int ka = g.a_wrap ? g.a_wrap : g.K;
    OFX_REQUIRE(g.lda >= ka && g.lda % 8 == 0, OFX_ESHAPE, "gemm: lda=%d must be >= K and a multiple of 8", g.lda);
    OFX_REQUIRE(g.ldc % (g.out_kind == 0 ? 4 : 8) == 0 && g.ldc >= (g.out_kind == 2 ? 3 * g.N : g.N), OFX_ESHAPE, "gemm: bad ldc=%d", g.ldc);
    OFX_REQUIRE(!g.resid || (g.ldr % 4 == 0 && g.ldr >= g.N), OFX_ESHAPE, "gemm: bad ldr=%d", g.ldr);
    OFX_REQUIRE(((uintptr_t)g.A % 16 == 0) && ((uintptr_t)g.W % 16 == 0) && ((uintptr_t)g.C % 16 == 0), OFX_EINVAL,
                "gemm: operands must be 16-byte aligned");
    OFX_REQUIRE(op_dtype == OFX_BF16 || op_dtype == OFX_F16, OFX_EINVAL, "gemm: operand dtype must be bf16 or f16");
    if (g.defer_splits) *g.defer_splits = 1;
    if (g.ln_done) *g.ln_done = false;
    const bool producer = g.xb_out || g.stat_part || g.xlo;
    OFX_REQUIRE(!producer || (g.xb_out && g.stat_part && g.xlo && g.C == g.xb_out && g.out_kind == 1 && g.ldc == g.N && g.N % 64 == 0), OFX_EINVAL,
                "gemm: a LayerNorm-fold producer takes xb_out, stat_part and xlo together, with C == xb_out in the operand type");
    OFX_REQUIRE(!g.row_stat || g.col_sum, OFX_EINVAL, "gemm: row_stat needs col_sum");
    OFX_REQUIRE(!(g.row_stat || producer) || (!g.aux_out && !g.drop.thresh && g.act != OFX_ACT_MISH && g.act != OFX_ACT_MISH_GRAD), OFX_EINVAL,
                "gemm: LayerNorm folding does not combine with the training epilogue features");
    OFX_REQUIRE(!(g.row_stat || producer) || !g.resid, OFX_EINVAL, "gemm: LayerNorm folding takes no residual (a producer's stream is (xb_out, xlo))");
    OFX_REQUIRE(!producer || g.act == OFX_ACT_NONE, OFX_EINVAL, "gemm: a LayerNorm-fold producer has no activation");

    GemmShape sh;
    sh.M = g.M; sh.N = g.N; sh.K = g.K; sh.lda = g.lda; sh.a_wrap = g.a_wrap; sh.k_mult = g.k_mult;
    sh.f16 = op_dtype == OFX_F16; sh.has_w8 = g.W8 && g.w8_scale; sh.has_m_dev = g.m_dev != nullptr;
    sh.can_split = g.slab && !producer && !g.row_stat; sh.defer = g.defer_splits != nullptr;
    sh.ln_fusable = g.ln_gamma && g.out_kind == 0 && g.act == OFX_ACT_NONE && !g.aux_out && !g.drop.thresh;
    sh.out_kind = g.out_kind; sh.resid = g.resid != nullptr; sh.aux = g.aux_out != nullptr; sh.xlo = g.xlo != nullptr;
    const GemmPlan pl = gemm_plan(sh, g_knobs, device_cu_count());
    if (pl.splits > 1) OFX_REQUIRE(g.slab_bytes >= (size_t)pl.splits * g.M * g.N * 4, OFX_EWORKSPACE, "gemm: split-K slab too small");

    if (g_ofx_prof_on) ofx_prof_set_tag(g.M, g.N, pl.k_logical, pl.kind, pl.kmul, pl.bytes);
    ProfScope prof(PROF_GEMM, s, pl.flops, true);
    KArgs k;
    k.A = (const char*)g.A; k.W = (const char*)g.W; k.C = (char*)g.C; k.bias = g.bias; k.resid = g.resid; k.aux_out = g.aux_out; k.m_dev = g.m_dev;
    k.M = g.M; k.N = g.N; k.K = g.K; k.lda = g.lda; k.ldc = g.ldc; k.ldr = g.ldr; k.act = g.act; k.out_kind = g.out_kind; k.drop = g.drop; k.n_valid = g.N;
    k.ka_tiles = ka / BK;
    k.xb_out = (char*)g.xb_out; k.stat_part = g.stat_part; k.row_stat = g.row_stat; k.col_sum = g.col_sum; k.stat_ld = g.stat_ld > 0 ? g.stat_ld : 1; k.xlo = (char*)g.xlo;
    k.tiles_m = pl.tiles_m; k.tiles_n = pl.tiles_n; k.nwg = pl.nwg; k.group_m = pl.group_m; k.epi_direct = pl.epi_direct;
    k.splits = pl.splits; k.kt_per_split = pl.kt_per_split; k.slab = (float*)g.slab; k.m_slab = g.M;
    if (gemm_kind_big_tile(pl.kind)) {
        if (pl.kind == GEMM_W2F8) { k.W8 = (const char*)g.W8; k.w8_scale = (const char*)g.w8_scale; TRY(ofx_gemm_launch_w2f8(&k, pl, s)); }
        else if (pl.kind == GEMM_X3) TRY(ofx_gemm_launch_x3(&k, pl, op_dtype, s));
        else if (pl.kind == GEMM_W2) TRY(ofx_gemm_launch_w2(&k, pl, op_dtype, s));
        else if (pl.kind == GEMM_PP) TRY(ofx_gemm_launch_pp(&k, pl, op_dtype, s));
        else TRY(ofx_gemm_launch_big(&k, pl, op_dtype, s));
        OFX_LAUNCH_CHECK();
        return OFX_OK;
    }
    static DeviceOnce attr_set;
    TRY(attr_set.run([]() -> int {
        OFX_HIP(hipFuncSetAttribute((const void*)gemm_128x128_kernel<bf16_t>, hipFuncAttributeMaxDynamicSharedMemorySize, GEMM_LDS_BYTES));
        OFX_HIP(hipFuncSetAttribute((const void*)gemm_128x128_kernel<f16_t>, hipFuncAttributeMaxDynamicSharedMemorySize, GEMM_LDS_BYTES));
        OFX_HIP(hipFuncSetAttribute((const void*)gemm_128x128_kernel<bf16_t, 2>, hipFuncAttributeMaxDynamicSharedMemorySize, GEMM64_LDS_BYTES));
        OFX_HIP(hipFuncSetAttribute((const void*)gemm_128x128_kernel<f16_t, 2>, hipFuncAttributeMaxDynamicSharedMemorySize, GEMM64_LDS_BYTES));
        return OFX_OK;
    }));
    const dim3 grid(pl.grid_x, pl.grid_y);
    const bool one = pl.second_pass == GEMM_PASS_NONE || pl.second_pass == GEMM_PASS_DEFERRED;
    if (pl.tile_m == 64) {
        if (op_dtype == OFX_F16) OFX_PLAUNCH(one, (gemm_128x128_kernel<f16_t, 2>), grid, dim3(256), GEMM64_LDS_BYTES, s, k);
        else OFX_PLAUNCH(one, (gemm_128x128_kernel<bf16_t, 2>), grid, dim3(256), GEMM64_LDS_BYTES, s, k);
    } else if (op_dtype == OFX_F16) OFX_PLAUNCH(one, gemm_128x128_kernel<f16_t>, grid, dim3(256), GEMM_LDS_BYTES, s, k);
    else OFX_PLAUNCH(one, gemm_128x128_kernel<bf16_t>, grid, dim3(256), GEMM_LDS_BYTES, s, k);
    if (pl.second_pass == GEMM_PASS_DEFERRED) *g.defer_splits = pl.splits;
    else if (pl.second_pass == GEMM_PASS_REDUCE_LN) {
        SplitKLnArgs a{(const float*)g.slab, (size_t)g.M * g.N, pl.splits, g.bias, g.resid, g.ldr, (float*)g.C, g.ldc,
                       g.ln_gamma, g.ln_beta, g.ln_out, g.ln_ld, g.ln_kind, g.ln_eps, g.M, g.N, g.m_dev};
        TRY(ofx_launch_splitk_reduce_ln(a, op_dtype, s, true));
        if (g.ln_done) *g.ln_done = true;
    } else if (pl.second_pass == GEMM_PASS_REDUCE) {
        if (op_dtype == OFX_F16) OFX_PLAUNCH(true, splitk_reduce_kernel<f16_t>, dim3(pl.reduce_grid), dim3(256), 0, s, k);
        else OFX_PLAUNCH(true, splitk_reduce_kernel<bf16_t>, dim3(pl.reduce_grid), dim3(256), 0, s, k);
    }
    OFX_LAUNCH_CHECK();
    return OFX_OK;
}
```

outfitx_amd/csrc/gemm_common.h:

```cpp
#pragma once
#include <type_traits>

#include "gemm_pingpong.h"
#include "gemm_plan.h"
#include "gemm_walk.h"
#include "ofx_common.h"

namespace {

constexpr int BM = 128, BN = 128, BK = 64;
constexpr int STAGE_BYTES = (BM + BN) * BK * 2;
constexpr int EPI_STRIDE = 68;
constexpr int EPI_BYTES_PER_WAVE = 64 * EPI_STRIDE * 4;
constexpr int GEMM_LDS_BYTES = 4 * EPI_BYTES_PER_WAVE > 2 * STAGE_BYTES ? 4 * EPI_BYTES_PER_WAVE : 2 * STAGE_BYTES;
constexpr int GEMM64_LDS_BYTES = 2 * (64 + BN) * BK * 2;

struct KArgs {
    const char* A;
    const char* W;
    char* C;
    const float* bias;
    const float* resid;
    float* aux_out;
    const int* m_dev;
// ... 47 lines not shown
    return v;
}

template <typename T, int ACT>
__device__ __forceinline__ void epilogue(const KArgs& p, OFX_LDS float* ep, int gm0, int gn0, int lane, int nrows = 64) {
    typedef typename OpT<T>::v4 v4;
    const int col = (lane & 15) * 4;
    const int gn = gn0 + col;
    f32x4 bias4 = {0.f, 0.f, 0.f, 0.f};
    if (p.bias) bias4 = *(const f32x4*)(p.bias + gn);
#pragma unroll 4
    for (int it = 0; it < nrows / 4; ++it) {
        const int row = it * 4 + (lane >> 4);
        const int gm = gm0 + row;
        f32x4 v = *(OFX_LDS f32x4*)(ep + row * EPI_STRIDE + col);
        if (gm < p.M) {
            if (p.row_stat) {
                const float mu = p.row_stat[2 * (size_t)gm * p.stat_ld], rs = p.row_stat[2 * (size_t)gm * p.stat_ld + 1];
                v = (v - *(const f32x4*)(p.col_sum + gn) * mu) * rs + bias4;
            } else v += bias4;
            if (p.aux_out) *(f32x4*)(p.aux_out + (size_t)gm * p.N + gn) = v;
#pragma unroll
            for (int e = 0; e < 4; ++e) v[e] = apply_act(v[e], ACT);
            if (p.drop.thresh) {
#pragma unroll
                for (int e = 0; e < 4; ++e) v[e] *= drop_mul(p.drop, gm, gn + e);
            }
            if (p.resid) {
                const f32x4 rr = *(const f32x4*)(p.resid + (size_t)gm * p.ldr + gn);
                if (ACT == OFX_ACT_MISH_GRAD) {
#pragma unroll
                    for (int e = 0; e < 4; ++e) v[e] *= act_mish_grad(rr[e]);
                } else v += rr;
            }
            if (p.xlo) {
                T* hp = (T*)p.xb_out + (size_t)gm * p.N + gn;
                T* lp = (T*)p.xlo + (size_t)gm * p.N + gn;
                const v4 h0 = *(const v4*)hp, l0 = *(const v4*)lp;
                v4 hb, lb;
#pragma unroll
                for (int e = 0; e < 4; ++e) { v[e] += (float)h0[e] + (float)l0[e]; hb[e] = (T)v[e]; lb[e] = lo_of<T>(v[e], hb[e]); }
                *(v4*)hp = hb; *(v4*)lp = lb;
                const float ssum = row16_sum_to_lane15((v[0] + v[1]) + (v[2] + v[3]));
                const float ssq = row16_sum_to_lane15((v[0] * v[0] + v[1] * v[1]) + (v[2] * v[2] + v[3] * v[3]));
                if ((lane & 15) == 15) *(f32x2*)(p.stat_part + ((size_t)gm * (p.N >> 6) + (gn0 >> 6)) * 2) = f32x2{ssum, ssq};
            } else store4<T>(p.C, (size_t)gm * p.ldc + gn, v, p.out_kind, p.N);
        }
    }
}

constexpr int EPI2_BYTES_PER_WAVE = 16 * 64 * 4;
constexpr int EPI_CONST_BIAS = 128, EPI_CONST_CSUM = 256, EPI_CONST_BYTES_PER_WAVE = 2048;

template <typename T, int ACT, int FOLD = 0, int RAMP = 0, int NP = 8, int JW = 4, int J0 = 0>
__device__ __forceinline__ void epilogue2(const KArgs& p, OFX_LDS char* ep, f32x4 (&acc)[NP][JW], int gm0, int gn0, int lane,
                                          OFX_LDS float* st = nullptr, OFX_LDS const float* cst = nullptr) {
    typedef typename OpT<T>::v8 v8;
    const int fr = lane & 15, fq = lane >> 4;
    if (FOLD != 3 && p.out_kind == 0) {
        constexpr int DEPTH = 2;
        const int chunk = lane & 15, rsub = lane >> 4;
        const int gn = gn0 + chunk * 4;
        f32x4 bias4 = {0.f, 0.f, 0.f, 0.f};
        if (cst) bias4 = *(OFX_LDS const f32x4*)(cst + EPI_CONST_BIAS + J0 * 16 + chunk * 4);
        else if (p.bias) bias4 = *(const f32x4*)(p.bias + gn);
        const bool has_res = p.resid != nullptr;
        f32x4 res[DEPTH + 1][4];
        auto fetch = [&](int pass, f32x4 (&dst)[4]) {
#pragma unroll
            for (int it = 0; it < 4; ++it) {
                const int gm = gm0 + pass * 16 + it * 4 + rsub;
                dst[it] = f32x4{0.f, 0.f, 0.f, 0.f};
                if (has_res && gm < p.M && gn < p.n_valid) dst[it] = *(const f32x4*)(p.resid + (size_t)gm * p.ldr + gn);
            }
        };
        f32x4 resr[RAMP ? NP : 1][4];
#pragma unroll
        for (int d = 0; d < DEPTH; ++d) {
            if (RAMP) fetch(d, resr[RAMP ? d : 0]);
            else fetch(d, res[d]);
        }
        if (RAMP) fetch(2, resr[RAMP ? 2 : 0]);
#pragma unroll
        for (int i = 0; i < NP; ++i) {
            if (RAMP) {
                if (i >= 1 && 2 * i + 1 < NP) fetch(2 * i + 1, resr[RAMP ? (2 * i + 1) % NP : 0]);
                if (i >= 1 && 2 * i + 2 < NP) fetch(2 * i + 2, resr[RAMP ? (2 * i + 2) % NP : 0]);
            } else if (i + DEPTH < NP) fetch(i + DEPTH, res[(i + DEPTH) % (DEPTH + 1)]);
#pragma unroll
            for (int j = 0; j < 4; ++j) *(OFX_LDS f32x4*)(ep + fr * 256 + (((j * 4 + fq) ^ (fr & 7)) << 4)) = acc[i][J0 + j];
#pragma unroll
            for (int it = 0; it < 4; ++it) {
                const int row = it * 4 + rsub;
                const int gm = gm0 + i * 16 + row;
                f32x4 v = *(OFX_LDS f32x4*)(ep + row * 256 + ((chunk ^ (row & 7)) << 4));
                if (gm < p.M && gn < p.n_valid) {
                    float mu = 0.f, rs = 1.f;
                    f32x4 cs = {0.f, 0.f, 0.f, 0.f};
                    if (FOLD == 2) { mu = p.row_stat[2 * (size_t)gm * p.stat_ld]; rs = p.row_stat[2 * (size_t)gm * p.stat_ld + 1]; cs = *(const f32x4*)(p.col_sum + gn); }
                    v = epi_value(p, v, ACT, FOLD == 2, mu, rs, cs, bias4, FOLD == 0, gm, gn);
                    v = epi_residual(v, RAMP ? resr[RAMP ? i : 0][it] : res[i % (DEPTH + 1)][it], ACT);
                    *(f32x4*)(p.C + ((size_t)gm * p.ldc + gn) * 4) = v;
                }
            }
        }
    } else {
        const int c8 = lane & 7, rsub = lane >> 3;
// ... 16 lines not shown
            else {
                const f32x2 a2 = *(const f32x2*)(p.row_stat + 2 * (size_t)ra * p.stat_ld), b2 = *(const f32x2*)(p.row_stat + 2 * (size_t)rb * p.stat_ld);
                pr = f32x4{a2[0], a2[1], b2[0], b2[1]};
            }
            *(OFX_LDS f32x4*)(st + 4 * lane) = pr;
            asm volatile("s_waitcnt lgkmcnt(0)" ::: "memory");
        }
        constexpr int D3 = NP < 2 ? NP : 2;
        v8 rh[FOLD == 3 ? D3 + 1 : 1][2], rl[FOLD == 3 ? D3 + 1 : 1][2];
        auto fetch_hl = [&](int pass, v8 (&dh)[2], v8 (&dl)[2]) {
#pragma unroll
            for (int it = 0; it < 2; ++it) {
                const int gm = min(gm0 + pass * 16 + it * 8 + rsub, p.M - 1);
                dh[it] = *(const v8*)((const T*)p.xb_out + (size_t)gm * p.N + gn);
                dl[it] = *(const v8*)((const T*)p.xlo + (size_t)gm * p.N + gn);
            }
        };
        if (FOLD == 3) {
#pragma unroll
            for (int d = 0; d < D3; ++d) fetch_hl(d, rh[FOLD == 3 ? d : 0], rl[FOLD == 3 ? d : 0]);
        }
        constexpr int KS = FOLD == 3 ? (NP + 3) / 4 : 1;
        float keep_s[KS], keep_q[KS];
#pragma unroll
        for (int k = 0; k < KS; ++k) { keep_s[k] = 0.f; keep_q[k] = 0.f; }
#pragma unroll
        for (int i = 0; i < NP; ++i) {
            if (FOLD == 3 && i + D3 < NP) fetch_hl(i + D3, rh[FOLD == 3 ? (i + D3) % (D3 + 1) : 0], rl[FOLD == 3 ? (i + D3) % (D3 + 1) : 0]);
#pragma unroll
            for (int j = 0; j < 4; ++j) *(OFX_LDS f32x4*)(ep + fr * 256 + (((j * 4 + fq) ^ (fr & 7)) << 4)) = acc[i][J0 + j];
#pragma unroll
            for (int it = 0; it < 2; ++it) {
                const int row = it * 8 + rsub;
                const int gm = gm0 + i * 16 + row;
                f32x4 v0 = *(OFX_LDS f32x4*)(ep + row * 256 + (((2 * c8) ^ (row & 7)) << 4));
                f32x4 v1 = *(OFX_LDS f32x4*)(ep + row * 256 + (((2 * c8 + 1) ^ (row & 7)) << 4));
                if (gm < p.M) {
                    float mu = 0.f, rs = 1.f;
                    if (FOLD == 2) {
                        if (st_lds) { const f32x2 ms = *(OFX_LDS f32x2*)(st + 2 * (i * 16 + row)); mu = ms[0]; rs = ms[1]; }
                        else { mu = p.row_stat[2 * (size_t)gm * p.stat_ld]; rs = p.row_stat[2 * (size_t)gm * p.stat_ld + 1]; }
                    }
                    v0 = epi_value(p, v0, ACT, FOLD == 2, mu, rs, cs0, b0, FOLD == 0, gm, gn);
                    v1 = epi_value(p, v1, ACT, FOLD == 2, mu, rs, cs1, b1, FOLD == 0, gm, gn + 4);
                    if (p.resid) {
                        const f32x4 r0 = *(const f32x4*)(p.resid + (size_t)gm * p.ldr + gn), r1 = *(const f32x4*)(p.resid + (size_t)gm * p.ldr + gn + 4);
                        v0 = epi_residual(v0, r0, ACT); v1 = epi_residual(v1, r1, ACT);
                    }
                    if (FOLD == 3) {
                        const v8 h = rh[FOLD == 3 ? i % (D3 + 1) : 0][it], l = rl[FOLD == 3 ? i % (D3 + 1) : 0][it];
#pragma unroll
                        for (int e = 0; e < 4; ++e) { v0[e] += (float)h[e] + (float)l[e]; v1[e] += (float)h[4 + e] + (float)l[4 + e]; }
                    }
                    store8<T>(p.C, (size_t)gm * p.ldc + gn, v0, v1, FOLD == 3 ? 1 : p.out_kind, p.N, FOLD == 3 ? p.xlo : nullptr);
                    if (FOLD == 3) {
                        const float ssum = row8_sum(((v0[0] + v0[1]) + (v0[2] + v0[3])) + ((v1[0] + v1[1]) + (v1[2] + v1[3])));
                        const float ssq = row8_sum(((v0[0] * v0[0] + v0[1] * v0[1]) + (v0[2] * v0[2] + v0[3] * v0[3])) +
                                                   ((v1[0] * v1[0] + v1[1] * v1[1]) + (v1[2] * v1[2] + v1[3] * v1[3])));
                        if (c8 == ((2 * i + it) & 7)) { keep_s[FOLD == 3 ? (2 * i + it) >> 3 : 0] = ssum; keep_q[FOLD == 3 ? (2 * i + it) >> 3 : 0] = ssq; }
                    }
                }
            }
        }
        if (FOLD == 3) {
#pragma unroll
            for (int k = 0; k < KS; ++k) {
                const int c = k * 8 + c8;
                const int gm = gm0 + (c >> 1) * 16 + (c & 1) * 8 + rsub;
                if (c < 2 * NP && gm < p.M) *(f32x2*)(p.stat_part + ((size_t)gm * (p.N >> 6) + (gn0 >> 6)) * 2) = f32x2{keep_s[k], keep_q[k]};
            }
        }
    }
}

template <typename T, int ACT, int FOLD, int NP, int JW>
__device__ __forceinline__ void epilogue_direct(const KArgs& p, f32x4 (&acc)[NP][JW], int gm0, int gn0, int lane, OFX_LDS const float* cst) {
    static_assert(JW % 4 == 0 && (FOLD == 0 || FOLD == 2), "whole 64-column halves; bias or LayerNorm-fold consumer");
    typedef T t2 __attribute__((ext_vector_type(2)));
    typedef unsigned u32x2 __attribute__((ext_vector_type(2)));
    typedef unsigned u32x4 __attribute__((ext_vector_type(4)));
    const int fr = lane & 15, fq = lane >> 4;
    const __amdgpu_buffer_rsrc_t rc = make_rsrc(p.C, (size_t)p.M * p.ldc * 2);
    const unsigned vo = ((unsigned)(gm0 + fr) * (unsigned)p.ldc + (unsigned)(gn0 + (fq & 1) * 16 + (fq >> 1) * 8)) * 2u;
    const unsigned pass_bytes = 16u * (unsigned)p.ldc * 2u;
#pragma unroll
    for (int h = 0; h < JW / 4; ++h) {
        f32x4 bb[4], cs[4];
#pragma unroll
        for (int jb = 0; jb < 4; ++jb) {
            OFX_LDS const float* cc = cst + (h * 4 + jb) * 16 + fq * 4;
            bb[jb] = *(OFX_LDS const f32x4*)(cc + EPI_CONST_BIAS);
            cs[jb] = FOLD == 2 ? *(OFX_LDS const f32x4*)(cc + EPI_CONST_CSUM) : f32x4{0.f, 0.f, 0.f, 0.f};
        }
#pragma unroll
        for (int i = 0; i < NP; ++i) {
            float mu = 0.f, rs = 1.f;
            if (FOLD == 2) { const f32x2 ms = *(OFX_LDS const f32x2*)(cst + 2 * (i * 16 + fr)); mu = ms[0]; rs = ms[1]; }
#pragma unroll
            for (int jp = 0; jp < 2; ++jp) {
                const f32x4 va = epi_value(p, acc[i][h * 4 + 2 * jp], ACT, FOLD == 2, mu, rs, cs[2 * jp], bb[2 * jp], false);
                const f32x4 vb = epi_value(p, acc[i][h * 4 + 2 * jp + 1], ACT, FOLD == 2, mu, rs, cs[2 * jp + 1], bb[2 * jp + 1], false);
                const unsigned a_lo = __builtin_bit_cast(unsigned, t2{(T)va[0], (T)va[1]}), a_hi = __builtin_bit_cast(unsigned, t2{(T)va[2], (T)va[3]});
                const unsigned b_lo = __builtin_bit_cast(unsigned, t2{(T)vb[0], (T)vb[1]}), b_hi = __builtin_bit_cast(unsigned, t2{(T)vb[2], (T)vb[3]});
                const u32x2 s0 = __builtin_amdgcn_permlane16_swap(a_lo, b_lo, false, false), s1 = __builtin_amdgcn_permlane16_swap(a_hi, b_hi, false, false);
                __builtin_amdgcn_raw_buffer_store_b128(u32x4{s0[0], s1[0], s0[1], s1[1]}, rc, (int)(vo + (unsigned)i * pass_bytes + (unsigned)(h * 128 + jp * 64)), 0, 0);
            }
        }
    }
}

template <typename T, int NP, int JW>
__device__ __forceinline__ bool epilogue_direct_dispatch(const KArgs& p, f32x4 (&acc)[NP][JW], int gm0, int gn0, int lane, OFX_LDS const float* cst) {
    if (!p.epi_direct || p.out_kind != 1 || p.resid || p.xlo || p.aux_out || p.drop.thresh || p.n_valid != p.N) return false;
    if ((size_t)p.M * p.ldc * 2 >= 0x7fffffff) return false;
#define OFX_EPD(ACT_, FOLD_) { epilogue_direct<T, ACT_, FOLD_, NP, JW>(p, acc, gm0, gn0, lane, cst); return true; }
    if (p.row_stat) {
        switch (p.act) {
            case OFX_ACT_QUICK_GELU: OFX_EPD(OFX_ACT_QUICK_GELU, 2)
            case OFX_ACT_GELU: OFX_EPD(OFX_ACT_GELU, 2)
            case OFX_ACT_NONE: OFX_EPD(OFX_ACT_NONE, 2)
            default: return false;
        }
    }
    switch (p.act) {
        case OFX_ACT_QUICK_GELU: OFX_EPD(OFX_ACT_QUICK_GELU, 0)
        case OFX_ACT_GELU: OFX_EPD(OFX_ACT_GELU, 0)
        case OFX_ACT_NONE: OFX_EPD(OFX_ACT_NONE, 0)
        default: return false;
    }
#undef OFX_EPD
}

template <typename T, int NP = 8, int JW = 4, int J0 = 0>
__device__ __forceinline__ void epilogue2_dispatch(const KArgs& p, OFX_LDS char* ep, f32x4 (&acc)[NP][JW], int gm0, int gn0, int lane,
                                                   OFX_LDS float* st = nullptr, OFX_LDS const float* cst = nullptr) {
    if (p.row_stat) {
        switch (p.act) {
            case OFX_ACT_QUICK_GELU: epilogue2<T, OFX_ACT_QUICK_GELU, 2, 0, NP, JW, J0>(p, ep, acc, gm0, gn0, lane, st, cst); break;
            case OFX_ACT_GELU: epilogue2<T, OFX_ACT_GELU, 2, 0, NP, JW, J0>(p, ep, acc, gm0, gn0, lane, st, cst); break;
            default: epilogue2<T, OFX_ACT_NONE, 2, 0, NP, JW, J0>(p, ep, acc, gm0, gn0, lane, st, cst); break;
        }
        return;
    }
    if (p.xlo) {
        epilogue2<T, OFX_ACT_NONE, 3, 1, NP, JW, J0>(p, ep, acc, gm0, gn0, lane, nullptr, cst);
        return;
    }
    switch (p.act) {
        case OFX_ACT_QUICK_GELU: epilogue2<T, OFX_ACT_QUICK_GELU, 0, 0, NP, JW, J0>(p, ep, acc, gm0, gn0, lane, nullptr, cst); break;
        case OFX_ACT_GELU: epilogue2<T, OFX_ACT_GELU, 0, 0, NP, JW, J0>(p, ep, acc, gm0, gn0, lane, nullptr, cst); break;
        case OFX_ACT_MISH: epilogue2<T, OFX_ACT_MISH, 0, 0, NP, JW, J0>(p, ep, acc, gm0, gn0, lane, nullptr, cst); break;
        case OFX_ACT_MISH_GRAD: epilogue2<T, OFX_ACT_MISH_GRAD, 0, 0, NP, JW, J0>(p, ep, acc, gm0, gn0, lane, nullptr, cst); break;
        default:
            if (p.resid && p.out_kind == 0) epilogue2<T, OFX_ACT_NONE, 0, 1, NP, JW, J0>(p, ep, acc, gm0, gn0, lane, nullptr, cst);
            else epilogue2<T, OFX_ACT_NONE, 0, 0, NP, JW, J0>(p, ep, acc, gm0, gn0, lane, nullptr, cst);
            break;
    }
}

template <typename T>
__global__ __launch_bounds__(256) void splitk_reduce_kernel(KArgs p) {
    const int M = p.m_dev ? min(*p.m_dev, p.M) : p.M;
    const int n4 = p.N / 4;
    const size_t total = (size_t)M * n4, plane = (size_t)p.m_slab * p.N;
    for (size_t i = blockIdx.x * (size_t)blockDim.x + threadIdx.x; i < total; i += (size_t)gridDim.x * blockDim.x) {
        const int gm = (int)(i / n4), gn = (int)(i % n4) * 4;
        if (gn >= p.n_valid) continue;
        const float* sp = p.slab + (size_t)gm * p.N + gn;
        f32x4 v = *(const f32x4*)sp;
        for (int s = 1; s < p.splits; ++s) v += *(const f32x4*)(sp + s * plane);
        f32x4 bias4 = {-0.f, -0.f, -0.f, -0.f};
        if (p.bias) bias4 = *(const f32x4*)(p.bias + gn);
        v = epi_value(p, v, p.act, false, 0.f, 1.f, bias4, bias4, true, gm, gn);
        if (p.resid) v = epi_residual(v, *(const f32x4*)(p.resid + (size_t)gm * p.ldr + gn), p.act);
        store4<T>(p.C, (size_t)gm * p.ldc + gn, v, p.out_kind, p.N);
    }
}

}

int ofx_gemm_launch_big(void* kargs, const GemmPlan& plan, int op_dtype, hipStream_t s);
int ofx_gemm_launch_pp(void* kargs, const GemmPlan& plan, int op_dtype, hipStream_t s);
int ofx_gemm_launch_w2(void* kargs, const GemmPlan& plan, int op_dtype, hipStream_t s);
int ofx_gemm_launch_w2f8(void* kargs, const GemmPlan& plan, hipStream_t s);
int ofx_gemm_launch_x3(void* kargs, const GemmPlan& plan, int op_dtype, hipStream_t s);
```

outfitx_amd/csrc/gemm_plan.h:

```cpp
#pragma once
#include <cstddef>

enum GemmKind { GEMM_AUTO = 0, GEMM_128 = 1, GEMM_256 = 2, GEMM_256x128 = 3, GEMM_PP = 4, GEMM_64 = 5, GEMM_W2 = 6, GEMM_W2F8 = 8, GEMM_X3 = 9 };
inline bool gemm_kind_big_tile(int kind) {
    return kind == GEMM_256 || kind == GEMM_256x128 || kind == GEMM_PP || kind == GEMM_W2 || kind == GEMM_W2F8 || kind == GEMM_X3;
}

struct GemmKnobs {
    int kernel = GEMM_AUTO;
    int splitk = 1;
    int x3_kernel = 1;
    int x3_persist = 1;
    int w2_persist = -1;
    int epi_direct = 1;
};

struct GemmShape {
    int M, N, K, lda;
    int a_wrap;
    int k_mult;
    bool f16;
    bool has_w8;
    bool has_m_dev;
    bool can_split;
// ... 34 lines not shown
    if (splitk >= 2) {
        GemmSmallPlan f{(splitk >> 8) & 1, (splitk & 0xff) > 16 ? 16 : (splitk & 0xff), 0.0};
        if (f.tile64 && !allow64) f.tile64 = 0;
        if (!allow_split || f.splits > nk) f.splits = 1;
        const int kps = (nk + f.splits - 1) / f.splits;
        f.splits = (nk + kps - 1) / kps;
        return f;
    }
    for (int t64 = 0; t64 <= (allow64 ? 1 : 0); ++t64) {
        const long blocks = (long)((M + (t64 ? 63 : 127)) / (t64 ? 64 : 128)) * (N / 128);
        const long slots = t64 ? 768 : 512;
        const double per = t64 ? 0.65 : 1.06;
        for (int sp = 1; sp <= 16; ++sp) {
            if (sp > 1 && !(allow_split && splitk != 0 && blocks < 256 && nk >= 16 && sp <= nk / 4)) break;
            const int kps = (nk + sp - 1) / sp;
            if ((nk + kps - 1) / kps != sp) continue;
            double t = (double)((blocks * sp + slots - 1) / slots) * kps * per + (t64 ? 1.0 : 0.0);
            if (sp > 1) t += 2.0 * sp * M * N * 4.0 / 5.0e6 + 3.0;
            if (t < best.cost) best = GemmSmallPlan{t64, sp, t};
        }
    }
    return best;
}
inline size_t gemm_splitk_slab_bytes(int M, int N, int K, const GemmKnobs& kn) {
    const int a = gemm_plan_small(M, N, K, true, true, kn.splitk).splits, b = gemm_plan_small(M, N, K, true, false, kn.splitk).splits;
    const int sp = a > b ? a : b;
    return sp > 1 ? (size_t)sp * M * N * 4 : 0;
}

inline GemmPlan gemm_plan(const GemmShape& g, const GemmKnobs& kn, int cu_count) {
    GemmPlan p{};
    int kind = kn.kernel == GEMM_W2 ? GEMM_AUTO : kn.kernel;
    if (g.a_wrap) {
        const long t2 = (long)((g.M + 255) / 256) * (g.N / 256);
        kind = (g.K == 2 * g.a_wrap && g.a_wrap % 32 == 0 && g.a_wrap >= 64 && g.N % 256 == 0 && (t2 >= 256 || kn.kernel == GEMM_W2) && kn.kernel != GEMM_128) ? GEMM_W2 : GEMM_128;
        if (kind == GEMM_W2 && g.has_w8 && g.f16 && g.a_wrap % 128 == 0) kind = GEMM_W2F8;
    } else if (kind == GEMM_AUTO) {
        const long t2 = (long)((g.M + 255) / 256) * (g.N / 256), t3 = (long)((g.M + 255) / 256) * (g.N / 128);
        if (g.N % 256 == 0 && t2 >= 1024) kind = g.K <= 1024 ? GEMM_PP : GEMM_256;
        else if (g.N % 128 == 0 && t3 >= 512) kind = GEMM_256x128;
        else kind = GEMM_128;
    }
    if (g.k_mult == 3 && !g.a_wrap && kn.x3_kernel && (kn.kernel == GEMM_AUTO || kn.kernel == GEMM_W2) && g.K % 96 == 0 && g.N % 128 == 0 && g.lda >= g.K &&
        (kn.x3_kernel >= 2 || (long)((g.M + 255) / 256) * (g.N / 128) >= 192))
        kind = GEMM_X3;
    if ((kind == GEMM_256 || kind == GEMM_PP) && g.N % 256) kind = GEMM_128;
    if (kind == GEMM_64 && g.N % 128) kind = GEMM_128;
    p.kind = kind;

    p.kmul = g.a_wrap ? g.K / g.a_wrap : (g.k_mult > 0 ? g.k_mult : 1);
    p.k_logical = g.K / p.kmul;
    const double ab = kind == GEMM_X3 ? 2.0 * g.M * (g.K / 3) * 2 : 2.0 * g.M * (g.a_wrap ? g.a_wrap : g.K);
    const double wb = kind == GEMM_W2F8 ? 3.0 * g.N * g.a_wrap : (kind == GEMM_X3 ? 2.0 * g.N * (g.K / 3) * 2 : 2.0 * g.N * g.K);
    double ob = g.out_kind == 0 ? 4.0 : (g.out_kind == 2 ? 6.0 : 2.0);
    if (g.xlo) ob = 8.0;
    else if (g.resid) ob += 4.0;
    if (g.aux) ob += 4.0;
    p.bytes = ab + wb + ob * g.M * g.N;
    p.flops = 2.0 * g.M * g.N * g.K * (kind == GEMM_W2F8 ? 0.75 : 1.0);

    p.splits = 1; p.kt_per_split = 0; p.grid_y = 1; p.second_pass = GEMM_PASS_NONE;
    if (gemm_kind_big_tile(kind)) {
        p.tile_m = 256; p.tile_n = (kind == GEMM_256x128 || kind == GEMM_X3) ? 128 : 256;
        p.group_m = kind == GEMM_256x128 ? 4 : 8;
        p.tiles_n = g.N / p.tile_n; p.tiles_m = (g.M + p.tile_m - 1) / p.tile_m; p.nwg = p.tiles_m * p.tiles_n;
        p.grid_x = p.nwg;
        if (kind == GEMM_W2 || kind == GEMM_W2F8) p.grid_x = gemm_persistent_grid(p.nwg, kn.w2_persist, g.has_m_dev, cu_count);
        if (kind == GEMM_X3) p.grid_x = gemm_persistent_grid(p.nwg, kn.x3_persist == 1 ? kn.w2_persist : 0, g.has_m_dev, cu_count);
        if (kind == GEMM_W2F8) p.epi_direct = kn.epi_direct;
        return p;
    }
    p.tile_m = 128; p.tile_n = 128;
    p.tiles_n = g.N / 128; p.tiles_m = (g.M + 127) / 128;
    int gm = (int)((3u << 20) / ((size_t)128 * g.K * 2) / 2);
    gm = gm < 1 ? 1 : (gm > 8 ? 8 : gm);
    p.group_m = gm;
    const bool can64 = (kind == GEMM_64) || (kind == GEMM_128 && kn.kernel == GEMM_AUTO && g.M > 64 && (long)p.tiles_m * p.tiles_n <= 384);
    GemmSmallPlan pl = gemm_plan_small(g.M, g.N, g.K, g.can_split, can64, kn.splitk);
    if (kind == GEMM_64) pl.tile64 = 1;
    if (pl.tile64) {
        p.tile_m = 64; p.tiles_m = (g.M + 63) / 64; p.group_m = 2 * gm;
    }
    p.nwg = p.tiles_m * p.tiles_n;
    p.splits = pl.splits;
    p.grid_x = p.nwg; p.grid_y = p.splits > 1 ? p.splits : 1;
    if (p.splits > 1) {
        p.kt_per_split = (g.K / 64 + p.splits - 1) / p.splits;
        p.second_pass = g.defer ? GEMM_PASS_DEFERRED : ((g.ln_fusable && splitk_reduce_ln_width_ok(g.N)) ? GEMM_PASS_REDUCE_LN : GEMM_PASS_REDUCE);
        if (p.second_pass == GEMM_PASS_REDUCE) {
            const size_t tot = (size_t)g.M * (g.N / 4);
            const int rg = (int)((tot + 255) / 256);
            p.reduce_grid = rg > 2048 ? 2048 : rg;
        }
    }
    return p;
}

inline int gemm_tn_splits(int M, int N, int K) {
#pragma clang fp contract(off)
    const long tiles = (long)((M + 255) / 256) * (N / 256);
    const int nkt = (K + 63) / 64;
    int best = 1;
    double best_t = 1e30;
    for (int s = 1; s <= 16 && s <= nkt; ++s) {
        const double waves = (double)((tiles * s + 255) / 256);
        const double t = waves * ((nkt + s - 1) / s) * 1.6 + 4.0 + (s > 1 ? 2.0 * s * M * N * 4.0 / 4.0e6 + 3.0 : 0.0);
        if (t < best_t) { best_t = t; best = s; }
// ... 8 lines not shown
```

outfitx_amd/csrc/gemm_x3.hip:

```cpp
#include "gemm_common.h"

namespace {

template <typename T>
__global__ __launch_bounds__(512, 2) void gemm_x3_kernel(KArgs p) {
    typedef typename OpT<T>::v8 v8;
    constexpr int TM = 256, TN = 128, BK2 = 32, PA = TM * BK2 * 2, PW = TN * BK2 * 2, STAGE = 2 * PA + 2 * PW, NST = 3;
    extern __shared__ __attribute__((aligned(16))) char smem[];
    OFX_LDS char* lds = (OFX_LDS char*)smem;
    const int tid = threadIdx.x, lane = tid & 63;
    const int wave = __builtin_amdgcn_readfirstlane(tid >> 6);
    const int wr = wave >> 1, wc = wave & 1;
    int grp = wave >> 2;
    asm volatile("" : "+s"(grp));
    const int Kl = p.K / 3;
    p.K = Kl;
    clamp_live_rows(p.m_dev, p.M);
    const int nk = Kl / BK2;
    const unsigned a_lo_off = (unsigned)Kl * 2, w_lo_off = (unsigned)Kl * 4;

    PpWalk<NST, TM, TN> w(p.nwg, p.group_m, p.tiles_m, p.tiles_n, nk);
    if (w.m0 >= p.M) return;
    for (;;) {
        const bool has_next = w.has_next();
// ... 20 lines not shown
            bload16(ra, a_off[0], koff, stg + wave * 2048); bload16(ra, a_off[1], koff, stg + wave * 2048 + 1024);
            bload16(ra, a_off[0], koff + a_lo_off, stg + PA + wave * 2048); bload16(ra, a_off[1], koff + a_lo_off, stg + PA + wave * 2048 + 1024);
            bload16(rw, w_off, koff, stg + 2 * PA + wave * 1024);
            bload16(rw, w_off, koff + w_lo_off, stg + 2 * PA + PW + wave * 1024);
        };

        f32x4 acc[4][4];
#pragma unroll
        for (int i = 0; i < 4; ++i)
#pragma unroll
            for (int j = 0; j < 4; ++j) acc[i][j] = f32x4{0.f, 0.f, 0.f, 0.f};
        v8 ah[4], al[4], wh[4], wl[4];

        auto read = [&](int step) {
            OFX_LDS char* stg = lds + w.stage(step) * STAGE;
#pragma unroll
            for (int j = 0; j < 4; ++j) { wh[j] = *(OFX_LDS v8*)(stg + w_frag + j * 1024); wl[j] = *(OFX_LDS v8*)(stg + PW + w_frag + j * 1024); }
#pragma unroll
            for (int i = 0; i < 4; ++i) { ah[i] = *(OFX_LDS v8*)(stg + a_frag + i * 1024); al[i] = *(OFX_LDS v8*)(stg + PA + a_frag + i * 1024); }
        };
        auto mfma = [&]() {
            __builtin_amdgcn_s_setprio(1);
#pragma unroll
            for (int i = 0; i < 4; ++i)
#pragma unroll
                for (int j = 0; j < 4; ++j) {
                    acc[i][j] = OpT<T>::mfma16(wh[j], ah[i], acc[i][j]);
                    acc[i][j] = OpT<T>::mfma16(wh[j], al[i], acc[i][j]);
                    acc[i][j] = OpT<T>::mfma16(wl[j], ah[i], acc[i][j]);
                }
            __builtin_amdgcn_s_setprio(0);
        };
        if (w.first) {
            issue_step(0); issue_step(1);
            asm volatile("s_waitcnt vmcnt(6)" ::: "memory");
        } else {
            asm volatile("s_waitcnt vmcnt(0)" ::: "memory");
        }
        __builtin_amdgcn_s_barrier();
        auto run = [&](auto G) {
            pp_group_begin<G.value>();
            int t = 0;
            do {
                pp_slot<G.value, 6>([&] { issue_step(t + 2); }, [&] { read(t); }, mfma);
            } while (++t < nk);
            pp_group_end<G.value>();
        };
        if (grp == 0) run(std::integral_constant<int, 0>());
        else run(std::integral_constant<int, 1>());
        OFX_LDS char* estage = lds + w.epilogue_stage() * STAGE;
        OFX_LDS char* ep = estage + wave * EPI2_BYTES_PER_WAVE;
        OFX_LDS float* st = nullptr;
        if (p.row_stat && p.out_kind != 0) st = (OFX_LDS float*)(estage + 8 * EPI2_BYTES_PER_WAVE + wave * 1024);
        epilogue2_dispatch<T, 4, 4, 0>(p, ep, acc, m0 + wr * 64, n0 + wc * 64, ln, st);
        if (!has_next) break;
        w.advance();
    }
    asm volatile("s_waitcnt vmcnt(0)" ::: "memory");
}

template <typename T>
static int launch_x3(const KArgs& k, const GemmPlan& plan, hipStream_t s) {
    constexpr int LDSB = 3 * (2 * 256 + 2 * 128) * 32 * 2;
    static DeviceOnce attr;
    TRY(set_max_dynamic_lds(attr, gemm_x3_kernel<T>, LDSB));
    OFX_PLAUNCH(true, (gemm_x3_kernel<T>), dim3(plan.grid_x), dim3(512), LDSB, s, k);
    return OFX_OK;
}

}

int ofx_gemm_launch_x3(void* kargs, const GemmPlan& plan, int op_dtype, hipStream_t s) {
    const KArgs& k = *(const KArgs*)kargs;
    return op_dtype == OFX_F16 ? launch_x3<f16_t>(k, plan, s) : launch_x3<bf16_t>(k, plan, s);
}
```

outfitx_amd/csrc/norm_act.hip:

```cpp
#include <algorithm>
#include "ofx_common.h"

namespace {

template <typename T, int NCH>
__global__ __launch_bounds__(256) void layernorm_kernel(LnArgs a, const int* rows_dev) {
    const int lane = threadIdx.x & 63, w = threadIdx.x >> 6;
    const int rows = rows_dev ? *rows_dev : a.rows;
    const int D = NCH * 256;
    for (int r = blockIdx.x * 4 + w; r < rows; r += gridDim.x * 4) {
        const int src = a.row_idx ? a.row_idx[r] : r;
        const f32x4* xp = (const f32x4*)(a.x + (size_t)src * D);
        f32x4 v[NCH];
        float s = 0.f;
#pragma unroll
        for (int c = 0; c < NCH; ++c) {
            v[c] = xp[lane + 64 * c];
            s += v[c][0] + v[c][1] + v[c][2] + v[c][3];
        }
        const float mu = wave_sum(s) * (1.0f / D);
        float q = 0.f;
#pragma unroll
        for (int c = 0; c < NCH; ++c) {
            v[c] -= mu;
            q += v[c][0] * v[c][0] + v[c][1] * v[c][1] + v[c][2] * v[c][2] + v[c][3] * v[c][3];
        }
        const float rstd = rsqrtf(wave_sum(q) * (1.0f / D) + a.eps);
        if (a.stats && lane == 0) { a.stats[2 * (size_t)r] = mu; a.stats[2 * (size_t)r + 1] = rstd; }
#pragma unroll
        for (int c = 0; c < NCH; ++c) {
            const int col = (lane + 64 * c) * 4;
            const f32x4 g = *(const f32x4*)(a.gamma + col), b = *(const f32x4*)(a.beta + col);
            store4<T>(a.y, (size_t)r * a.ldy + col, v[c] * rstd * g + b, a.out_kind, D);
        }
    }
}

}

int ofx_launch_layernorm_dev(const LnArgs& a, const int* rows_dev, int op_dtype, hipStream_t s) {
    OFX_REQUIRE(a.D == 512 || a.D == 768 || a.D == 1024 || a.D == 1536, OFX_ESHAPE, "layernorm: D=%d not in {512,768,1024,1536}", a.D);
    OFX_REQUIRE(a.rows > 0, OFX_ESHAPE, "layernorm: rows=%d", a.rows);
    OFX_REQUIRE(a.ldy % 4 == 0 && a.ldy >= (a.out_kind == 2 ? 3 * a.D : a.D), OFX_ESHAPE, "layernorm: bad ldy=%d", a.ldy);
    int grid = (a.rows + 3) / 4;
    if (grid > 8192) grid = 8192;
    ProfScope prof(PROF_NORM, s);
#define LN_CASE(T, N) hipLaunchKernelGGL((layernorm_kernel<T, N>), dim3(grid), dim3(256), 0, s, a, rows_dev)
    if (op_dtype == OFX_F16) {
        if (a.D == 512) LN_CASE(f16_t, 2); else if (a.D == 768) LN_CASE(f16_t, 3); else if (a.D == 1024) LN_CASE(f16_t, 4); else LN_CASE(f16_t, 6);
    } else {
        if (a.D == 512) LN_CASE(bf16_t, 2); else if (a.D == 768) LN_CASE(bf16_t, 3); else if (a.D == 1024) LN_CASE(bf16_t, 4); else LN_CASE(bf16_t, 6);
    }
#undef LN_CASE
    OFX_LAUNCH_CHECK();
    return OFX_OK;
}
int ofx_launch_layernorm(const LnArgs& a, int op_dtype, hipStream_t s) { return ofx_launch_layernorm_dev(a, nullptr, op_dtype, s); }

namespace {
template <typename T, int NW = 4>
__global__ __launch_bounds__(64 * NW) void splitk_reduce_ln_kernel(SplitKLnArgs a) {
    __shared__ float part[2][NW];
    const int lane = threadIdx.x & 63, w = threadIdx.x >> 6, nw = blockDim.x >> 6;
    const int rows = a.m_dev ? min(*a.m_dev, a.rows) : a.rows;
    const int D = a.D, col = threadIdx.x * 4;
    for (int r = blockIdx.x; r < rows; r += gridDim.x) {
        const float* sp = a.slab + (size_t)r * D + col;
        f32x4 t = *(const f32x4*)sp;
        for (int k = 1; k < a.splits; ++k) t += *(const f32x4*)(sp + k * a.plane);
        if (a.bias) t += *(const f32x4*)(a.bias + col);
        if (a.resid) t += *(const f32x4*)(a.resid + (size_t)r * a.ldr + col);
        *(f32x4*)(a.x + (size_t)r * a.ldx + col) = t;
        const float s = wave_sum(t[0] + t[1] + t[2] + t[3]);
        if (lane == 0) part[0][w] = s;
        __syncthreads();
        float tot = 0.f;
        for (int i = 0; i < nw; ++i) tot += part[0][i];
        const float mu = tot * (1.0f / D);
        t -= mu;
        const float q = wave_sum(t[0] * t[0] + t[1] * t[1] + t[2] * t[2] + t[3] * t[3]);
        if (lane == 0) part[1][w] = q;
        __syncthreads();
        float tq = 0.f;
        for (int i = 0; i < nw; ++i) tq += part[1][i];
        const float rstd = rsqrtf(tq * (1.0f / D) + a.eps);
        const f32x4 g = *(const f32x4*)(a.gamma + col), b = *(const f32x4*)(a.beta + col);
        store4<T>(a.y, (size_t)r * a.ldy + col, t * rstd * g + b, a.out_kind, D);
        __syncthreads();
    }
}
}

int ofx_launch_splitk_reduce_ln(const SplitKLnArgs& a, int op_dtype, hipStream_t s, bool in_gemm_scope) {
    OFX_REQUIRE(splitk_reduce_ln_width_ok(a.D), OFX_ESHAPE, "splitk_reduce_ln: D=%d not in {512,768,1024,1536}", a.D);
    OFX_REQUIRE(a.rows > 0 && a.splits >= 1 && a.ldx % 4 == 0 && a.ldx >= a.D && (!a.resid || (a.ldr % 4 == 0 && a.ldr >= a.D)), OFX_ESHAPE, "splitk_reduce_ln: bad shape");
    OFX_REQUIRE(a.ldy % 4 == 0 && a.ldy >= (a.out_kind == 2 ? 3 * a.D : a.D), OFX_ESHAPE, "splitk_reduce_ln: bad ldy=%d", a.ldy);
    const int grid = a.rows > 8192 ? 8192 : a.rows;
    ProfScope prof(PROF_NORM, s, 0.0, false, !in_gemm_scope);
    if (a.D > 1024) {
        if (op_dtype == OFX_F16) OFX_PLAUNCH(in_gemm_scope, (splitk_reduce_ln_kernel<f16_t, 6>), dim3(grid), dim3(a.D / 4), 0, s, a);
        else OFX_PLAUNCH(in_gemm_scope, (splitk_reduce_ln_kernel<bf16_t, 6>), dim3(grid), dim3(a.D / 4), 0, s, a);
    } else if (op_dtype == OFX_F16) OFX_PLAUNCH(in_gemm_scope, splitk_reduce_ln_kernel<f16_t>, dim3(grid), dim3(a.D / 4), 0, s, a);
    else OFX_PLAUNCH(in_gemm_scope, splitk_reduce_ln_kernel<bf16_t>, dim3(grid), dim3(a.D / 4), 0, s, a);
    OFX_LAUNCH_CHECK();
    return OFX_OK;
}

namespace {
template <typename T>
__global__ __launch_bounds__(256) void pack_rows_kernel(const float* src, T* dst, int rows_src, int rows_dst, int K_src,
                                                       int K_dst, int ld_src, int mode) {
    const int chunks = K_dst / 4;
    const size_t total = (size_t)rows_dst * chunks;
    const int ld = mode == 3 ? 2 * K_dst : (mode ? 3 * K_dst : K_dst);
    for (size_t i = blockIdx.x * (size_t)blockDim.x + threadIdx.x; i < total; i += (size_t)gridDim.x * blockDim.x) {
        const int r = (int)(i / chunks), c = (int)(i % chunks) * 4;
        f32x4 v = {0.f, 0.f, 0.f, 0.f};
        if (r < rows_src) {
            if (c + 3 < K_src && (ld_src % 4 == 0)) v = *(const f32x4*)(src + (size_t)r * ld_src + c);
            else {
#pragma unroll
                for (int e = 0; e < 4; ++e) if (c + e < K_src) v[e] = src[(size_t)r * ld_src + c + e];
            }
        }
        typedef typename OpT<T>::v4 v4;
        v4 hi, lo;
#pragma unroll
        for (int e = 0; e < 4; ++e) { hi[e] = (T)v[e]; lo[e] = lo_of<T>(v[e], hi[e]); }
        T* p = dst + (size_t)r * ld + c;
        *(v4*)p = hi;
        if (mode == 1) { *(v4*)(p + K_dst) = lo; *(v4*)(p + 2 * K_dst) = hi; }
        if (mode == 2) { *(v4*)(p + K_dst) = hi; *(v4*)(p + 2 * K_dst) = lo; }
        if (mode == 3) *(v4*)(p + K_dst) = lo;
    }
}
}

int ofx_launch_pack_rows(const float* src, void* dst, int rows_src, int rows_dst, int K_src, int K_dst, int ld_src,
                         int mode, int op_dtype, hipStream_t s) {
    OFX_REQUIRE(K_dst % 4 == 0 && K_dst >= K_src && rows_dst >= rows_src, OFX_ESHAPE, "pack_rows: bad shape");
    size_t total = (size_t)rows_dst * (K_dst / 4);
    int grid = (int)((total + 255) / 256);
    if (grid > 16384) grid = 16384;
    if (grid < 1) grid = 1;
    if (op_dtype == OFX_F16)
        hipLaunchKernelGGL(pack_rows_kernel<f16_t>, dim3(grid), dim3(256), 0, s, src, (f16_t*)dst, rows_src, rows_dst, K_src, K_dst, ld_src, mode);
    else
        hipLaunchKernelGGL(pack_rows_kernel<bf16_t>, dim3(grid), dim3(256), 0, s, src, (bf16_t*)dst, rows_src, rows_dst, K_src, K_dst, ld_src, mode);
    OFX_LAUNCH_CHECK();
// ... 451 lines not shown
```

outfitx_amd/csrc/ofx_common.h:

```cpp
#pragma once
#include <hip/hip_runtime.h>
#include <hip/hip_ext.h>
#include <mutex>
#include <stdint.h>
#include <stdio.h>

#include "../../include/ofx.h"
#include "gemm_plan.h"

typedef __bf16 bf16_t;
typedef _Float16 f16_t;
typedef __bf16 bf16x8 __attribute__((ext_vector_type(8)));
typedef __bf16 bf16x4 __attribute__((ext_vector_type(4)));
typedef _Float16 f16x8 __attribute__((ext_vector_type(8)));
typedef _Float16 f16x4 __attribute__((ext_vector_type(4)));
typedef float f32x4 __attribute__((ext_vector_type(4)));
typedef float f32x2 __attribute__((ext_vector_type(2)));
typedef float f32x16 __attribute__((ext_vector_type(16)));
typedef short s16x4 __attribute__((ext_vector_type(4)));
typedef short s16x8 __attribute__((ext_vector_type(8)));

#define OFX_LDS __attribute__((address_space(3)))
#define OFX_GLB __attribute__((address_space(1)))

void ofx_set_error(const char* fmt, ...);

#define OFX_REQUIRE(cond, code, ...)            \
    do {                                        \
        if (!(cond)) {                          \
            ofx_set_error(__VA_ARGS__);         \
            return (code);                      \
        }                                       \
    } while (0)

#define OFX_HIP(call)                                                                  \
    do {                                                                               \
        hipError_t e_ = (call);                                                        \
        if (e_ != hipSuccess) {                                                        \
            ofx_set_error("%s failed: %s (%s:%d)", #call, hipGetErrorString(e_), __FILE__, __LINE__); \
            return OFX_EHIP;                                                           \
        }                                                                              \
    } while (0)

#define OFX_LAUNCH_CHECK()                                                             \
    do {                                                                               \
        hipError_t e_ = hipGetLastError();                                             \
        if (e_ != hipSuccess) {                                                        \
            ofx_set_error("kernel launch failed: %s (%s:%d)", hipGetErrorString(e_), __FILE__, __LINE__); \
            return OFX_EHIP;                                                           \
        }                                                                              \
    } while (0)

template <typename T> struct OpT;
template <> struct OpT<bf16_t> {
    typedef bf16x8 v8;
    typedef bf16x4 v4;
    static __device__ __forceinline__ f32x4 mfma16(v8 a, v8 b, f32x4 c) {
        return __builtin_amdgcn_mfma_f32_16x16x32_bf16(a, b, c, 0, 0, 0);
    }
};
template <> struct OpT<f16_t> {
    typedef f16x8 v8;
    typedef f16x4 v4;
    static __device__ __forceinline__ f32x4 mfma16(v8 a, v8 b, f32x4 c) {
        return __builtin_amdgcn_mfma_f32_16x16x32_f16(a, b, c, 0, 0, 0);
    }
};

template <typename T>
__device__ __forceinline__ T lo_of(float v, T hi) { return (T)(v - (float)hi); }
template <typename T, int NV>
__device__ __forceinline__ void store_cols(void* y, size_t off, const f32x4 (&v)[NV], int out_kind, int D, void* ylo = nullptr) {
    typedef T vt __attribute__((ext_vector_type(4 * NV)));
    if (out_kind == 0) {
#pragma unroll
        for (int k = 0; k < NV; ++k) *(f32x4*)((float*)y + off + 4 * k) = v[k];
        return;
    }
    vt hi;
#pragma unroll
    for (int e = 0; e < 4 * NV; ++e) hi[e] = (T)v[e >> 2][e & 3];
    T* p = (T*)y + off;
    *(vt*)p = hi;
    if (out_kind == 2 || ylo) {
        vt lo;
#pragma unroll
        for (int e = 0; e < 4 * NV; ++e) lo[e] = lo_of<T>(v[e >> 2][e & 3], hi[e]);
        if (ylo) *(vt*)((T*)ylo + off) = lo;
        else { *(vt*)(p + D) = lo; *(vt*)(p + 2 * D) = hi; }
    }
}
template <typename T>
__device__ __forceinline__ void store4(void* y, size_t off, f32x4 v, int out_kind, int D, void* ylo = nullptr) {
    const f32x4 vs[1] = {v};
    store_cols<T, 1>(y, off, vs, out_kind, D, ylo);
}
template <typename T>
__device__ __forceinline__ void store8(void* y, size_t off, f32x4 v0, f32x4 v1, int out_kind, int D, void* ylo = nullptr) {
    const f32x4 vs[2] = {v0, v1};
    store_cols<T, 2>(y, off, vs, out_kind, D, ylo);
}

__device__ __forceinline__ float act_quick_gelu(float u) { return u * __builtin_amdgcn_rcpf(1.0f + __builtin_amdgcn_exp2f(-2.4554669595930157f * u)); }
__device__ __forceinline__ float act_gelu(float u) { return 0.5f * u * (1.0f + erff(u * 0.70710678118654752f)); }
__device__ __forceinline__ float act_mish(float u) {
    if (u > 20.0f) return u;
    float e = __expf(u);
    float n = e * (e + 2.0f);
    return u * (n * __builtin_amdgcn_rcpf(n + 2.0f));
}
__device__ __forceinline__ float act_mish_grad(float u) {
    if (u > 20.0f) return 1.0f;
    const float e = __expf(u), n = e * (e + 2.0f);
    const float t = n * __builtin_amdgcn_rcpf(n + 2.0f);
    const float sg = e * __builtin_amdgcn_rcpf(1.0f + e);
    return t + u * sg * (1.0f - t * t);
}
__device__ __forceinline__ float apply_act(float u, int act) {
    switch (act) {
        case OFX_ACT_QUICK_GELU: return act_quick_gelu(u);
        case OFX_ACT_GELU: return act_gelu(u);
        case OFX_ACT_MISH: return act_mish(u);
        default: return u;
    }
}

__device__ __forceinline__ float row16_sum_to_lane15(float v) {
    v += __builtin_bit_cast(float, __builtin_amdgcn_update_dpp(0, __builtin_bit_cast(int, v), 0x111, 0xf, 0xf, true));
    v += __builtin_bit_cast(float, __builtin_amdgcn_update_dpp(0, __builtin_bit_cast(int, v), 0x112, 0xf, 0xf, true));
    v += __builtin_bit_cast(float, __builtin_amdgcn_update_dpp(0, __builtin_bit_cast(int, v), 0x114, 0xf, 0xf, true));
    v += __builtin_bit_cast(float, __builtin_amdgcn_update_dpp(0, __builtin_bit_cast(int, v), 0x118, 0xf, 0xf, true));
    return v;
}
__device__ __forceinline__ float row8_sum(float v) {
    v += __builtin_bit_cast(float, __builtin_amdgcn_update_dpp(0, __builtin_bit_cast(int, v), 0xB1, 0xf, 0xf, true));
    v += __builtin_bit_cast(float, __builtin_amdgcn_update_dpp(0, __builtin_bit_cast(int, v), 0x4E, 0xf, 0xf, true));
    v += __builtin_bit_cast(float, __builtin_amdgcn_update_dpp(0, __builtin_bit_cast(int, v), 0x141, 0xf, 0xf, true));
    return v;
}
__device__ __forceinline__ float wave_sum(float v) {
#pragma unroll
    for (int o = 32; o > 0; o >>= 1) v += __shfl_xor(v, o, 64);
    return v;
}
__device__ __forceinline__ float wave_max(float v) {
#pragma unroll
    for (int o = 32; o > 0; o >>= 1) v = fmaxf(v, __shfl_xor(v, o, 64));
    return v;
}

enum { PROF_GEMM = 0, PROF_NORM = 1, PROF_ATTN = 2, PROF_OTHER = 3, PROF_NCAT = 4 };
extern bool g_ofx_prof_on;
extern int g_ofx_prof_mask;
// ... 69 lines not shown
    float scale = 1.0f;
};
__host__ __device__ __forceinline__ unsigned ofx_fmix32(unsigned h) {
    h ^= h >> 16; h *= 0x85EBCA6Bu; h ^= h >> 13; h *= 0xC2B2AE35u; h ^= h >> 16;
    return h;
}
__host__ __device__ __forceinline__ float drop_mul(const DropArgs& d, unsigned row, unsigned col) {
    unsigned h = ofx_fmix32(d.seed + d.site * 0x9E3779B9u + row * 0x632BE5ABu);
    h = ofx_fmix32(h ^ (col * 0x9E3779B1u + 0x7F4A7C15u));
    return h >= d.thresh ? d.scale : 0.0f;
}
__host__ __device__ __forceinline__ unsigned ofx_draw_u32(unsigned seed, unsigned draw, unsigned stream, unsigned b, unsigned i) {
    unsigned h = ofx_fmix32(seed + 0x6A09E667u);
    h = ofx_fmix32(h ^ draw);
    h = ofx_fmix32(h + stream * 0x9E3779B9u + 0x7F4A7C15u);
    h = ofx_fmix32(h ^ (b * 0x632BE5ABu));
    return ofx_fmix32(h + i * 0x9E3779B1u);
}
__host__ __device__ __forceinline__ unsigned ofx_draw_below(unsigned u, unsigned n) { return (unsigned)(((unsigned long long)u * n) >> 32); }
inline DropArgs make_drop(float p, unsigned seed, unsigned site) {
    DropArgs d;
    if (p > 0.f) { d.seed = seed; d.site = site; d.thresh = (unsigned)((double)p * 4294967296.0); d.scale = 1.0f / (1.0f - p); }
    return d;
}

struct GemmArgs {
    const void* A;
    const void* W;
    void* C;
    const float* bias;
    const float* resid;
    const int* m_dev = nullptr;
    float* aux_out = nullptr;
    void* slab = nullptr;
    size_t slab_bytes = 0;
    int M, N, K, lda, ldc, ldr;
    int act;
    int out_kind;
    DropArgs drop;
    void* xb_out = nullptr;
    float* stat_part = nullptr;
    const float* row_stat = nullptr;
    int stat_ld = 1;
    void* xlo = nullptr;
    const float* col_sum = nullptr;
    int a_wrap = 0;
    const void* W8 = nullptr; const void* w8_scale = nullptr;
    int k_mult = 1;
    int* defer_splits = nullptr;
    const float* ln_gamma = nullptr; const float* ln_beta = nullptr; void* ln_out = nullptr; int ln_ld = 0, ln_kind = 0; float ln_eps = 0.f;
    bool* ln_done = nullptr;
};
int ofx_launch_gemm(const GemmArgs& g, int op_dtype , hipStream_t s);
size_t ofx_gemm_splitk_bytes(int M, int N, int K);
int ofx_gemm_tune(int knob, int value);

struct LnArgs {
    const float* x;
    const int* row_idx;
    const float* gamma;
    const float* beta;
    void* y;
    int rows, D, ldy;
    int out_kind;
    float eps;
    float* stats = nullptr;
};
size_t ofx_gemm_tn_slab_bytes(int M, int N, int K);
int ofx_launch_gemm_tn(const void* A, int lda, const void* B, int ldb, float* C, int ldc, int M, int N, int K, const int* k_dev,
                       void* slab, size_t slab_bytes, int op_dtype, hipStream_t s, int m_valid = 0, int n_valid = 0, int accumulate = 0);
int ofx_launch_layernorm(const LnArgs& a, int op_dtype, hipStream_t s);
struct SplitKLnArgs {
    const float* slab; size_t plane; int splits;
    const float* bias; const float* resid; int ldr;
    float* x; int ldx;
    const float* gamma; const float* beta; void* y; int ldy, out_kind; float eps;
    int rows, D; const int* m_dev;
};
int ofx_launch_splitk_reduce_ln(const SplitKLnArgs& a, int op_dtype, hipStream_t s, bool in_gemm_scope = false);
int ofx_launch_layernorm_dev(const LnArgs& a, const int* rows_dev, int op_dtype, hipStream_t s);
int ofx_launch_pack_lo8(const void* w2_rows, void* dst8, void* scale8, int N, int K, hipStream_t s);
int ofx_launch_pack_rows(const float* src, void* dst, int rows_src, int rows_dst, int K_src, int K_dst, int ld_src,
                         int mode, int op_dtype, hipStream_t s);
int ofx_launch_patchify(const float* px, void* out, int N, int img, int patch, int op_dtype, hipStream_t s);
int ofx_launch_vit_embed_ln(const float* patch_out, const float* cls, const float* pos, const float* g, const float* b,
                            float* x, int N, int S, int D, float eps, hipStream_t s, void* xb, float* stat, int op_dtype, void* xlo);
int ofx_launch_text_embed(const int64_t* ids, const float* tok, const float* pos, float* x, int N, int T, int Tc, int D,
                          int vocab, int shared_first, hipStream_t s);
int ofx_launch_text_eos_index(const int64_t* ids, int* row_idx, int N, int T, int Tc, int eos_id, int shared_first, hipStream_t s);
int ofx_launch_iota_rows(int* idx, int n, int stride, hipStream_t s);
int ofx_launch_l2norm_store(const float* src, float* dst, int rows, int D, int ld, int col, int normalize, hipStream_t s);
int ofx_launch_set_build(const float* x, const uint8_t* mask, const float* prefix, int prefix_stride, int* cu, float* X,
                         int B, int L, int D, hipStream_t s);
int ofx_launch_gather_rows(const void* src, const int* idx, void* dst, int rows, int row_bytes, int src_ld_bytes, hipStream_t s);
int ofx_launch_set_build_indexed(const float* table, int ld, long long n_table, const int* idx, const int* cu_items, const float* prefix,
                                 int prefix_stride, int* cu_rows, float* X, int B, int D, hipStream_t s);
int ofx_preprocess_to(const uint8_t* src, const long long* offsets, const int* heights, const int* widths, int N, int channels, int size,
                      const float* mean, const float* stdv, float* out, void* patches, int patch, int op_dtype, void* ws, size_t ws_bytes, hipStream_t stream);
int ofx_launch_row_stats_cast(const float* X, void* Xb, void* Xlo, float* stat, int rows, int W, float eps, int op_dtype, hipStream_t s);
int ofx_launch_gather_hilo(const void* hi, const void* lo, const int* idx, float* dst, int rows, int W, int op_dtype, hipStream_t s);
int ofx_launch_stats_finalize(const float* part, int slots, int W, float eps, float* stat, int rows, hipStream_t s);
int ofx_launch_fold_pack(const float* Wsrc, const float* gamma, const float* beta, const float* bias, void* Wf, float* col_sum, float* bias_f,
                         int N, int K, int op_dtype, hipStream_t s, int split = 0);
int ofx_launch_cir_prefix(const float* img_emb, const float* txt, float* out, int B, int D, hipStream_t s);
int ofx_launch_cp_head(const float* row0, const float* w, const float* bias, float* logits, int B, int D, hipStream_t s);

// ... 29 lines not shown
    float scale;
    DropArgs drop;
    int qkv_op = 0;
    int fixed_len = 0, causal = 0, mask_ld = 0;
    const int64_t* key_mask = nullptr;
    int shared_first = 0;
    int splits = 1; size_t plane = 0; const float* bias = nullptr;
};
int ofx_launch_set_attention(const SetAttnArgs& a, int op_dtype, hipStream_t s);
int ofx_launch_fused_qkv_attn(const void* X, const void* Wqkv, const float* bias, const float* row_stat, const float* col_sum, void* out,
                              int n_img, int S, int Wm, int heads, int ldx, int ldo, float scale, int op_dtype, hipStream_t s, bool w2 = false);

int ofx_launch_multi_copy(const void* table_host, int n, hipStream_t s);
int ofx_launch_fill_f32(float* p, size_t n, float v, hipStream_t s);
int ofx_launch_transpose_cast(const float* src, void* dst, int R, int C, int ldd, int op_dtype, hipStream_t s, void* row_dst = nullptr, int ld_row = 0);
size_t ofx_colsum_part_floats(int C);
int ofx_launch_colsum(const void* x, int x_kind, int ld, const int* gather, const float* row_scale, float* out0, float* out1, float* out2, int seg,
                      float* part, int C, const int* m_dev, int M, int op_dtype, hipStream_t s, int valid = 0, int accumulate = 0);
size_t ofx_ln_bwd_part_floats(int D);
int ofx_launch_row_map(const int* cu, int* map, int B, int M, hipStream_t s);
int ofx_launch_ln_bwd(const float* dy, const float* x, const float* stats, const float* gamma, const float* add, const int* add_map, float* dx_out, void* dx_op,
                      float* dgamma, float* dbeta, float* dcols, float* part, int D, const int* m_dev, int M, int op_dtype, const DropArgs& drop, hipStream_t s,
                      int accumulate = 0);
int ofx_launch_set_attention_bwd(const void* qkv, const float* d_o, void* dqkv, const int* cu, int nseq, int n_head, int D, int max_len,
                                 float scale, int op_dtype, const DropArgs& drop, int only_row0, hipStream_t s);
int ofx_launch_set_attention_bwd_mfma(const void* qkv, const float* d_o, void* dqkv, const int* cu, int nseq, int n_head, int D, int max_len,
                                      float scale, int op_dtype, const DropArgs& drop, int only_row0, hipStream_t s);
int ofx_launch_drop_rows(float* x, int rows, int cols, const DropArgs& d, hipStream_t s);
int ofx_launch_focal_loss(const float* logits, const float* labels, int B, float alpha, float gamma, float upstream, float* loss, float* dlogits, hipStream_t s,
                          int reduction = 1, float* per_elem = nullptr);
size_t ofx_set_rank_loss_ws(int B, int K);
int ofx_launch_set_rank_loss(const float* y, const float* y_hat, const float* neg, const uint8_t* mask, int B, int K, int D, float margin, float upstream,
                             float* loss, float* dy_hat, float* d_pos, float* d_neg, void* ws, hipStream_t s);
int ofx_launch_set_rank_loss_indexed(const float* table, int ld, int n_table, const int* pos_index, const int* neg_index, const float* y_hat, int B, int K,
                                     int D, float margin, float upstream, float* loss, float* dy_hat, float* d_pos, float* d_neg, void* ws, hipStream_t s);
size_t ofx_adamw_step_ws(long long n_arena);
int ofx_launch_adamw_step(const ofx_opt_segment* segments, int n_segments, float* grad, float* exp_avg, float* exp_avg_sq, long long n_arena,
                          float* step, double lr, double beta1, double beta2, double eps, double weight_decay, double max_norm, double grad_scale,
                          float* grad_norm, int* skipped, void* ws, hipStream_t s);
int ofx_launch_cp_head_bwd(const float* dlogits, const float* w_or_rows, const int* cu, float* dX, void* dXb, float* db, int B, int D, int op_dtype,
                           const DropArgs& head, const DropArgs& below, hipStream_t s, int accumulate = 0);
int ofx_launch_fitb(const float* y, const float* cand, int B, int C, int D, int64_t* idx, float* dist, hipStream_t s);
int ofx_launch_fitb_indexed(const float* table, int ld, int n_table, const int* cand_index, const float* y, int B, int C, int D, const int64_t* answer,
                            int64_t* idx, float* dist, int* n_correct, hipStream_t s);
int ofx_launch_l2_topk(const float* Q, const float* P, int nq, int np, int D, int k, int64_t index_base, int64_t* idx,
                       float* dist, void* ws, size_t ws_bytes, hipStream_t s);
size_t ofx_l2_topk_ws(int nq, int np);
int ofx_launch_l2_topk_grouped(const float* Q, const float* P, int nq, int np, int D, int k, const int* panels, int n_panels, int max_group_rows,
                               const int64_t* gt, int64_t* idx, float* dist, int* gt_pos, void* ws, size_t ws_bytes, hipStream_t s);
int ofx_launch_topk_merge(const int64_t* idx_in, const float* dist_in, int parts, int nq, int k, int64_t* idx, float* dist,
                          hipStream_t s);

extern int g_topk_filter;
```

outfitx_amd/engine.py:

```python
from __future__ import annotations

import ctypes as C
from typing import Dict, List, NamedTuple, Optional, Sequence

import torch

from . import _lib as L


def _ptr(t: Optional[torch.Tensor]) -> Optional[int]:
    return None if t is None else t.data_ptr()


def _stream(device: torch.device) -> int:
    return torch.cuda.current_stream(device).cuda_stream


def _f32c(t: torch.Tensor, device) -> torch.Tensor:
    if t.device != device or t.dtype != torch.float32 or not t.is_contiguous():
        t = t.to(device=device, dtype=torch.float32).contiguous()
    return t


def shared_first_row(ids: torch.Tensor, att: Optional[torch.Tensor]) -> bool:
# ... 253 lines not shown
            self._px_stage = stage
        elif getattr(self, "_px_event", None) is not None:
            self._px_event.synchronize()
        buf = stage.numpy()
        for a, o, n in zip(arrs, offs, nbytes):
            buf[o:o + n] = a.reshape(-1)
        src = stage[:total + 4].to(self.device, non_blocking=True)
        self._px_event = torch.cuda.Event()
        self._px_event.record(torch.cuda.current_stream(self.device))
        self._keep_px = src
        return src, offs, hs, ws_

    def clip_preprocess(self, images: Sequence, size: int, mean: Sequence[float], std: Sequence[float]) -> torch.Tensor:
        src, offs, hs, ws_ = self._stage_images(images)
        N = len(hs)
        out = torch.empty(N, 3, size, size, dtype=torch.float32, device=self.device)
        I = C.POINTER(C.c_int); LL = C.POINTER(C.c_longlong)
        nb = int(self.lib.ofx_clip_preprocess_ws(hs.ctypes.data_as(I), ws_.ctypes.data_as(I), N, 3, size))
        ws = self.workspace(nb)
        m = (C.c_float * 3)(*mean); sd = (C.c_float * 3)(*std)
        with torch.cuda.device(self.device):
            L.check(self.lib.ofx_clip_preprocess(_ptr(src), offs.ctypes.data_as(LL), hs.ctypes.data_as(I), ws_.ctypes.data_as(I), N, 3, size,
                                                 m, sd, _ptr(out), _ptr(ws), ws.numel(), _stream(self.device)), "ofx_clip_preprocess")
        return out

    def vit_u8(self, images: Sequence, mean: Sequence[float], std: Sequence[float], out: torch.Tensor, col: int, normalize: bool) -> None:
        src, offs, hs, ws_ = self._stage_images(images)
        N = len(hs)
        I = C.POINTER(C.c_int); LL = C.POINTER(C.c_longlong)
        nb = int(self.lib.ofx_vit_b32_u8_ws_bytes(self.h, hs.ctypes.data_as(I), ws_.ctypes.data_as(I), N, 3))
        if nb == 0:
            raise ValueError("ofx_vit_b32_u8_ws_bytes: bad image geometry")
        ws = self.workspace(nb)
        m = (C.c_float * 3)(*mean); sd = (C.c_float * 3)(*std)
        with torch.cuda.device(self.device):
            L.check(self.lib.ofx_vit_b32_fwd_u8(self.h, _ptr(src), offs.ctypes.data_as(LL), hs.ctypes.data_as(I), ws_.ctypes.data_as(I), N, 3,
                                                m, sd, _ptr(out), out.stride(0), col, int(normalize), _ptr(ws), ws.numel(),
                                                _stream(self.device)), "ofx_vit_b32_fwd_u8")

    def stage_tokens(self, ids: torch.Tensor, att: Optional[torch.Tensor]):
        def mv(t):
            if t is None:
                return None
            if t.device == self.device and t.dtype == torch.int64 and t.is_contiguous():
                return t
            return t.to(device=self.device, dtype=torch.int64, non_blocking=t.device.type == "cpu" and t.is_pinned()).contiguous()
        return mv(ids), mv(att)

    def text(self, ids: torch.Tensor, att: Optional[torch.Tensor], out: torch.Tensor, col: int, normalize: bool,
             lengths: Optional[Sequence[int]] = None) -> None:
        shared = lengths.shared_first if isinstance(lengths, TextLengths) else shared_first_row(ids, att)
        ids_d, att_d = self.stage_tokens(ids, att)
        N, T = ids_d.shape
        Tc = T if lengths is None else max(1, min(T, max(int(v) for v in lengths)))
        arr = None if lengths is None else (C.c_int * N)(*[int(v) for v in lengths])
        nb = self.ws_bytes(L.OP_TEXT, N, Tc)
        ws = self.workspace(nb)
        shared = bool(shared) and Tc >= 2 and bool(self.desc.txt_x3)
        with torch.cuda.device(self.device):
            L.check(self.lib.ofx_clip_text_fwd_shared(self.h, _ptr(ids_d), _ptr(att_d), arr, N, T, _ptr(out), out.stride(0), col,
                                                      int(normalize), int(shared), _ptr(ws), ws.numel(), _stream(self.device)), "ofx_clip_text_fwd_shared")
        self._keep_ids = (ids_d, att_d)

    def l2_topk(self, Q: torch.Tensor, P: torch.Tensor, k: int, index_base: int = 0):
        Q = _f32c(Q, self.device); P = _f32c(P, self.device)
        nq, D = Q.shape
        npool = P.shape[0]
        idx = torch.empty(nq, k, dtype=torch.int64, device=self.device)
        dist = torch.empty(nq, k, dtype=torch.float32, device=self.device)
        ws = self.workspace(self.ws_bytes(L.OP_TOPK, nq, npool))
        with torch.cuda.device(self.device):
            L.check(self.lib.ofx_l2_topk(self.h, _ptr(Q), _ptr(P), nq, npool, D, k, index_base, _ptr(idx), _ptr(dist),
                                         _ptr(ws), ws.numel(), _stream(self.device)), "ofx_l2_topk")
        return idx, dist

    def l2_topk_grouped(self, Q: torch.Tensor, group_of_query, P: torch.Tensor, pool_offsets, k: int, gt=None, max_ws_bytes: int = 1 << 30):
        Q = _f32c(Q, self.device); P = _f32c(P, self.device)
        nq, D = Q.shape
        npool = P.shape[0]
        grp = torch.as_tensor(group_of_query, device="cpu").to(torch.int64).reshape(-1)
        off = torch.as_tensor(pool_offsets, device="cpu").to(torch.int64).reshape(-1)
        G = off.numel() - 1
        if G < 1 or int(off[0]) != 0 or int(off[-1]) != npool or bool((off[1:] < off[:-1]).any()):
            raise ValueError("pool_offsets must start at 0, be non-decreasing and end at len(P)")
        if grp.numel() != nq:
            raise ValueError(f"group_of_query has {grp.numel()} entries for {nq} queries")
        if nq and (int(grp.min()) < 0 or int(grp.max()) >= G):
            raise ValueError(f"group_of_query must lie in [0, {G})")
        q_lo, q_hi = off[grp], off[grp + 1]
        if bool((q_hi == q_lo).any()):
            raise ValueError("a query's pool is empty")
        gt_h = None
        if gt is not None:
            gt_h = torch.as_tensor(gt).to(device="cpu", dtype=torch.int64).reshape(-1)
            if gt_h.numel() != nq:
                raise ValueError(f"gt has {gt_h.numel()} entries for {nq} queries")
            if bool(((gt_h >= 0) & ((gt_h < q_lo) | (gt_h >= q_hi))).any()):
                raise ValueError("a gt row lies outside its query's pool")
        idx = torch.empty(nq, k, dtype=torch.int64, device=self.device)
        dist = torch.empty(nq, k, dtype=torch.float32, device=self.device)
        gt_pos = torch.empty(nq, dtype=torch.int32, device=self.device) if gt_h is not None else None
        if nq == 0:
            return idx, dist, gt_pos
        max_rows = int((q_hi - q_lo).max())
        need = lambda n: int(self.lib.ofx_l2_topk_grouped_ws(n, npool, max_rows))
        if need(1) > max_ws_bytes:
# ... 226 lines not shown
```

Baseline: 8119.

## Add SPLIT2 outputs for x3 GEMM consumers and a pipelined set-attention kernel

Producers that feed an x3 GEMM (layernorm, set attention, the fc1 epilogue) now write only the hi and lo planes (SPLIT2) instead of hi, lo and a duplicate hi, which cuts the bytes stored per activation. In clip_layer_x3, GEMM argument setup is hoisted ahead of the launches so each producer can pick its output kind from the consumer's GEMM kind. A new wave-pipelined set-attention kernel for short sets (S<=8) handles several head/sequence pairs per wave and prefetches the next pair's Q/K/V while computing the current one. Both paths are on by default through tune knobs 22 and 23. The risk is that a consumer whose kernel choice differs from what is predicted here would read the third plane, which is no longer written.

```diff
diff --git a/include/ofx.h b/include/ofx.h
--- a/include/ofx.h
+++ b/include/ofx.h
@@ -13,7 +13,7 @@
 enum ofx_dtype { OFX_F32 = 0, OFX_BF16 = 1, OFX_F16 = 2 };
 enum ofx_act { OFX_ACT_NONE = 0, OFX_ACT_QUICK_GELU = 1, OFX_ACT_GELU = 2, OFX_ACT_MISH = 3, OFX_ACT_MISH_GRAD = 4 };
 enum ofx_precision { OFX_PREC_BF16 = 0, OFX_PREC_F16 = 1, OFX_PREC_BF16X3 = 2, OFX_PREC_F16W2 = 3 };
-enum ofx_out_kind { OFX_OUT_F32 = 0, OFX_OUT_OP = 1, OFX_OUT_SPLIT3 = 2 };
+enum ofx_out_kind { OFX_OUT_F32 = 0, OFX_OUT_OP = 1, OFX_OUT_SPLIT3 = 2, OFX_OUT_SPLIT2 = 3 };
 
 typedef struct ofx_handle ofx_handle;
 typedef void* ofx_stream;
@@ -152,6 +152,7 @@
                 int lda, int ldc, int ldr, int act, int out_kind, int op_dtype, ofx_stream stream);
 int ofx_gemm_x3(const void* A3, const void* W3, void* C, const float* bias, const float* resid, int M, int N, int K,
                 int lda, int ldc, int ldr, int act, int out_kind, int op_dtype, ofx_stream stream);
+int ofx_gemm_x3_kind(int M, int N, int K, int lda, int op_dtype);
 int ofx_pack_lo8(const void* W2, void* W8, void* scale8, int N, int K, ofx_stream stream);
 int ofx_gemm_w2f8(const void* A, const void* W2, const void* W8, const void* scale8, void* C, const float* bias, const float* resid, int M, int N, int K,
                   int lda, int ldc, int ldr, int act, int out_kind, ofx_stream stream);
@@ -214,6 +215,8 @@
                                int nseq, int seq_len, int width, int n_head, int ldx, int ldo, float scale, int op_dtype, ofx_stream stream);
 int ofx_attention_f32(const float* qkv, void* out, const int64_t* key_mask, int nseq, int seq_len, int n_head, int D, int ldo, int out_kind,
                       int mask_ld, int causal, float scale, int op_dtype, ofx_stream stream);
+int ofx_attention_f32_shared(const float* qkv, void* out, const int64_t* key_mask, int nseq, int seq_len, int n_head, int D, int ldo, int out_kind,
+                             int mask_ld, int causal, int shared_first, float scale, int op_dtype, ofx_stream stream);
 int ofx_convert(const float* src, void* dst, int rows, int cols, int mode, int op_dtype, ofx_stream stream);
 
 #ifdef __cplusplus
diff --git a/outfitx_amd/_lib.py b/outfitx_amd/_lib.py
--- a/outfitx_amd/_lib.py
+++ b/outfitx_amd/_lib.py
@@ -12,6 +12,7 @@
 ACT_NONE, ACT_QUICK_GELU, ACT_GELU, ACT_MISH = 0, 1, 2, 3
 PREC_BF16, PREC_F16, PREC_BF16X3 = 0, 1, 2
 OUT_F32, OUT_OP, OUT_SPLIT3 = 0, 1, 2
+OUT_SPLIT2 = 3
 OP_SET_ENCODER, OP_VIT, OP_TEXT, OP_TOPK = 0, 1, 2, 3
 PREC_F16W2 = 3
 PRECISIONS = {"bf16": PREC_BF16, "f16": PREC_F16, "fp16": PREC_F16, "bf16x3": PREC_BF16X3, "f16w2": PREC_F16W2}
@@ -147,6 +148,7 @@
     "ofx_gemm": (_i, [_vp, _vp, _vp, _vp, _vp, _i, _i, _i, _i, _i, _i, _i, _i, _i, _vp]),
     "ofx_gemm_w2": (_i, [_vp, _vp, _vp, _vp, _vp, _i, _i, _i, _i, _i, _i, _i, _i, _i, _vp]),
     "ofx_gemm_x3": (_i, [_vp, _vp, _vp, _vp, _vp, _i, _i, _i, _i, _i, _i, _i, _i, _i, _vp]),
+    "ofx_gemm_x3_kind": (_i, [_i, _i, _i, _i, _i]),
     "ofx_pack_lo8": (_i, [_vp, _vp, _vp, _i, _i, _vp]),
     "ofx_gemm_w2f8": (_i, [_vp, _vp, _vp, _vp, _vp, _vp, _vp, _i, _i, _i, _i, _i, _i, _i, _i, _vp]),
     "ofx_gemm_w2f8_fold": (_i, [_vp, _vp, _vp, _vp, _vp, _vp, _vp, _vp, _i, _i, _i, _i, _i, _i, _vp]),
@@ -181,6 +183,7 @@
     "ofx_set_attention_op": (_i, [_vp, _vp, _vp, _i, _i, _i, _i, _i, _i, _i, _f, _f, C.c_uint, _i, _i, _vp]),
     "ofx_set_attention_bwd": (_i, [_vp, _vp, _vp, _vp, _i, _i, _i, _i, _i, _f, _f, C.c_uint, _i, _i, _i, _vp]),
     "ofx_attention_f32": (_i, [_vp, _vp, _vp, _i, _i, _i, _i, _i, _i, _i, _i, _f, _i, _vp]),
+    "ofx_attention_f32_shared": (_i, [_vp, _vp, _vp, _i, _i, _i, _i, _i, _i, _i, _i, _i, _f, _i, _vp]),
     "ofx_convert": (_i, [_vp, _vp, _i, _i, _i, _i, _vp]),
 }
 
diff --git a/outfitx_amd/csrc/api.hip b/outfitx_amd/csrc/api.hip
--- a/outfitx_amd/csrc/api.hip
+++ b/outfitx_amd/csrc/api.hip
@@ -575,19 +575,38 @@
     return OFX_OK;
 }
 
+int g_split2 = 1;
+
+static int split_kind_for(const GemmArgs& consumer, int dt) {
+    return g_split2 && ofx_gemm_kind(consumer, dt) == GEMM_X3 ? OFX_OUT_SPLIT2 : OFX_OUT_SPLIT3;
+}
+
 static int clip_layer_x3(const ClipLayer& L, const ClipWs& w, int rows, int nseq, int S, int W, int MLP, int heads, int act,
                          float eps, int causal, const int64_t* key_mask, int mask_ld, int dt, const int* pool_idx, hipStream_t s, bool mfma_attn = false,
                          int shared_first = 0) {
-    LnArgs ln{w.X, nullptr, L.g1, L.be1, w.H, rows, W, 3 * W, OFX_OUT_SPLIT3, eps};
-    TRY(ofx_launch_layernorm(ln, dt, s));
     GemmArgs g1{}; g1.A = w.H; g1.C = w.QKV; g1.M = rows; g1.N = 3 * W;
     use_gemm(g1, L.qkv, W);
     const bool f32_attn = S <= 64 && !mfma_attn;
     OFX_REQUIRE(!shared_first || f32_attn, OFX_EINVAL, "clip_layer_x3: a shared first row needs the fp32 set attention");
     g1.ldc = 3 * W; g1.act = OFX_ACT_NONE; g1.out_kind = f32_attn ? OFX_OUT_F32 : OFX_OUT_OP;
+    float* X = w.X; char* H = w.H; char* U = w.U; int M = rows;
+    if (pool_idx) { X = w.XP; H = w.HP; U = w.UP; M = nseq; }
+    GemmArgs g2{}; g2.A = H; g2.C = X; g2.resid = X; g2.M = M; g2.N = W; g2.ldc = W; g2.ldr = W; g2.act = OFX_ACT_NONE; g2.out_kind = OFX_OUT_F32;
+    use_gemm(g2, L.o, W);
+    if (pool_idx) { g2.slab = w.slab; g2.slab_bytes = w.slab_bytes; }
+    GemmArgs g3{}; g3.A = H; g3.C = U; g3.M = M; g3.N = MLP; g3.ldc = 3 * MLP; g3.act = act; g3.out_kind = OFX_OUT_SPLIT3;
+    use_gemm(g3, L.fc1, W);
+    if (pool_idx) { g3.slab = w.slab; g3.slab_bytes = w.slab_bytes; }
+    GemmArgs g4{}; g4.A = U; g4.C = X; g4.resid = X; g4.M = M; g4.N = W; g4.ldc = W; g4.ldr = W; g4.act = OFX_ACT_NONE; g4.out_kind = OFX_OUT_F32;
+    use_gemm(g4, L.fc2, MLP);
+    if (pool_idx) { g4.slab = w.slab; g4.slab_bytes = w.slab_bytes; }
+    if (ofx_gemm_kind(g3, dt) == GEMM_X3) g3.out_kind = split_kind_for(g4, dt);
+
+    LnArgs ln{w.X, nullptr, L.g1, L.be1, w.H, rows, W, 3 * W, split_kind_for(g1, dt), eps};
+    TRY(ofx_launch_layernorm(ln, dt, s));
     TRY(ofx_launch_gemm(g1, dt, s));
     if (f32_attn) {
-        SetAttnArgs sa{w.QKV, w.H, nullptr, nseq, heads, W, 3 * W, OFX_OUT_SPLIT3, S, 0, 0.125f};
+        SetAttnArgs sa{w.QKV, w.H, nullptr, nseq, heads, W, 3 * W, split_kind_for(g2, dt), S, 0, 0.125f};
         sa.fixed_len = S; sa.causal = causal; sa.key_mask = key_mask; sa.mask_ld = mask_ld; sa.shared_first = shared_first;
         TRY(ofx_launch_set_attention(sa, dt, s));
     } else {
@@ -595,25 +614,14 @@
         at.split3_w = W;
         TRY(ofx_launch_attention_mfma(at, dt, s));
     }
-    float* X = w.X; char* H = w.H; char* U = w.U; int M = rows;
     if (pool_idx) {
         TRY(ofx_launch_gather_rows(w.H, pool_idx, w.HP, nseq, 3 * W * 2, 3 * W * 2, s));
         TRY(ofx_launch_gather_rows(w.X, pool_idx, w.XP, nseq, W * 4, W * 4, s));
-        X = w.XP; H = w.HP; U = w.UP; M = nseq;
-    }
-    GemmArgs g2{}; g2.A = H; g2.C = X; g2.resid = X; g2.M = M; g2.N = W; g2.ldc = W; g2.ldr = W; g2.act = OFX_ACT_NONE; g2.out_kind = OFX_OUT_F32;
-    use_gemm(g2, L.o, W);
-    if (pool_idx) { g2.slab = w.slab; g2.slab_bytes = w.slab_bytes; }
+    }
     TRY(ofx_launch_gemm(g2, dt, s));
-    LnArgs ln2{X, nullptr, L.g2, L.be2, H, M, W, 3 * W, OFX_OUT_SPLIT3, eps};
+    LnArgs ln2{X, nullptr, L.g2, L.be2, H, M, W, 3 * W, split_kind_for(g3, dt), eps};
     TRY(ofx_launch_layernorm(ln2, dt, s));
-    GemmArgs g3{}; g3.A = H; g3.C = U; g3.M = M; g3.N = MLP; g3.ldc = 3 * MLP; g3.act = act; g3.out_kind = OFX_OUT_SPLIT3;
-    use_gemm(g3, L.fc1, W);
-    if (pool_idx) { g3.slab = w.slab; g3.slab_bytes = w.slab_bytes; }
     TRY(ofx_launch_gemm(g3, dt, s));
-    GemmArgs g4{}; g4.A = U; g4.C = X; g4.resid = X; g4.M = M; g4.N = W; g4.ldc = W; g4.ldr = W; g4.act = OFX_ACT_NONE; g4.out_kind = OFX_OUT_F32;
-    use_gemm(g4, L.fc2, MLP);
-    if (pool_idx) { g4.slab = w.slab; g4.slab_bytes = w.slab_bytes; }
     return ofx_launch_gemm(g4, dt, s);
 }
 
@@ -1150,6 +1158,9 @@
         case 17: g_topk_filter = value != 0; return OFX_OK;
         case 20: g_x3_vit_f32_attn = value != 0; return OFX_OK;
         case 21: g_text_shared_first = value != 0; return OFX_OK;
+        case 22: g_split2 = value != 0; return OFX_OK;
+        case 23: if (value < 0 || value > 32) { ofx_set_error("ofx_tune(23): %d is not in [0, 32] (blocks per CU of the pipelined set attention; 0 = the one-pair-per-block kernel)", value); return OFX_EINVAL; }
+                 g_attn_pipe = value; return OFX_OK;
         default: ofx_set_error("ofx_tune: unknown knob %d", knob); return OFX_EINVAL;
     }
 }
@@ -1173,6 +1184,10 @@
                            int lda, int ldc, int ldr, int act, int out_kind, int op_dtype, ofx_stream stream) {
     GemmArgs g = op_gemm(A3, W3, C, bias, resid, M, N, 3 * K, lda, ldc, ldr, act, out_kind); g.k_mult = 3;
     return ofx_launch_gemm(g, op_dtype, (hipStream_t)stream);
+}
+extern "C" int ofx_gemm_x3_kind(int M, int N, int K, int lda, int op_dtype) {
+    GemmArgs g{}; g.M = M; g.N = N; g.K = 3 * K; g.lda = lda; g.k_mult = 3;
+    return ofx_gemm_kind(g, op_dtype);
 }
 extern "C" int ofx_pack_lo8(const void* W2, void* W8, void* scale8, int N, int K, ofx_stream stream) {
     return ofx_launch_pack_lo8(W2, W8, scale8, N, K, (hipStream_t)stream);
@@ -1428,6 +1443,13 @@
     a.fixed_len = seq_len; a.causal = causal; a.key_mask = key_mask; a.mask_ld = mask_ld;
     return ofx_launch_set_attention(a, op_dtype, (hipStream_t)stream);
 }
+extern "C" int ofx_attention_f32_shared(const float* qkv, void* out, const int64_t* key_mask, int nseq, int seq_len, int n_head, int D, int ldo, int out_kind,
+                                        int mask_ld, int causal, int shared_first, float scale, int op_dtype, ofx_stream stream) {
+    OFX_REQUIRE(qkv && out && nseq > 0 && op_dtype_ok(op_dtype), OFX_EINVAL, "attention_f32_shared: bad argument (a NULL pointer, nseq = %d or op_dtype = %d)", nseq, op_dtype);
+    SetAttnArgs a{qkv, out, nullptr, nseq, n_head, D, ldo, out_kind, seq_len, 0, scale};
+    a.fixed_len = seq_len; a.causal = causal; a.key_mask = key_mask; a.mask_ld = mask_ld; a.shared_first = shared_first ? 1 : 0;
+    return ofx_launch_set_attention(a, op_dtype, (hipStream_t)stream);
+}
 extern "C" int ofx_convert(const float* src, void* dst, int rows, int cols, int mode, int op_dtype, ofx_stream stream) {
     return ofx_launch_pack_rows(src, dst, rows, rows, cols, cols, cols, mode, op_dtype, (hipStream_t)stream);
 }
diff --git a/outfitx_amd/csrc/attention.hip b/outfitx_amd/csrc/attention.hip
--- a/outfitx_amd/csrc/attention.hip
+++ b/outfitx_amd/csrc/attention.hip
@@ -1,4 +1,7 @@
+#include "attn_pairs.h"
 #include "attn_wave.h"
+
+int g_attn_pipe = 1;
 
 namespace {
 
@@ -253,7 +256,7 @@
     __syncthreads();
     auto store_row = [&](int i, int c8) {
         const f32x4 x0 = *(const f32x4*)(qs + i * STR + c8), x1 = *(const f32x4*)(qs + i * STR + c8 + 4);
-        store8<T>(a.out, (size_t)row_of(i) * a.ldo + h * HD + c8, x0, x1, a.out_kind, D);
+        store8<T, true>(a.out, (size_t)row_of(i) * a.ldo + h * HD + c8, x0, x1, a.out_kind, D);
     };
     if constexpr (!WIDE) {
         const int c8 = (lane & 7) * 8, r8 = lane >> 3;
@@ -263,6 +266,144 @@
         }
     } else {
         for (int f = lane + q0 * C8; f < nq * C8; f += 64) store_row(f / C8, (f % C8) * 8);
+    }
+}
+
+__device__ __forceinline__ float sa8_dot(const float* q_row, const float* k_row) {
+#pragma clang fp contract(off)
+    const f32x4* qp = (const f32x4*)q_row;
+    const f32x4* kp = (const f32x4*)k_row;
+    float d = 0.f;
+#pragma unroll
+    for (int c = 0; c < 16; ++c) {
+        const f32x4 x = qp[c], y = kp[c];
+        float t = x[1] * y[1];
+        t = __builtin_fmaf(x[0], y[0], t);
+        t = __builtin_fmaf(x[2], y[2], t);
+        t = __builtin_fmaf(x[3], y[3], t);
+        d = d + t;
+    }
+    return d;
+}
+__device__ __forceinline__ float sa8_pv(const float* row, const float (&v)[8], int S) {
+#pragma clang fp contract(off)
+    float acc = 0.f;
+#pragma unroll
+    for (int j = 0; j < 8; ++j) acc = __builtin_fmaf(v[j], j < S ? row[j] : 0.f, acc);
+    return acc;
+}
+struct SetPipeRegs {
+    f32x4 q[2], k[2];
+    float v[8];
+    long long mk;
+};
+
+template <typename T>
+__global__ __launch_bounds__(64 * ATTN_PIPE_WAVES) void set_attention_pipe_kernel(SetK a) {
+#pragma clang fp contract(off)
+    constexpr int SMAX = 8, STR = 68, SCS = SMAX + 4, WF = 2 * SMAX * STR + SMAX * SCS;
+    __shared__ __attribute__((aligned(16))) float smem[ATTN_PIPE_WAVES * WF];
+    const int lane = threadIdx.x & 63, wave = threadIdx.x >> 6;
+    float* qs = smem + wave * WF;
+    float* ks = qs + SMAX * STR;
+    float* sc = ks + SMAX * STR;
+    const bool sh = a.shared_first != 0;
+    int first, count;
+    attn_pair_run(blockIdx.x, wave, gridDim.x, (a.nseq + (sh ? 1 : 0)) * a.n_head, first, count);
+    if (count <= 0) return;
+    const int D = a.D, end = first + count;
+    const int c4 = (lane & 15) * 4, rsub = lane >> 4;
+    struct Pair { int h, r0, S, q0, mb; bool sh; };
+    auto pair_of = [&](int p) {
+        const int b = p / a.n_head;
+        const bool sh_q0 = sh && b == a.nseq;
+        Pair g;
+        g.h = p % a.n_head;
+        g.r0 = sh ? (sh_q0 ? 0 : b * (a.fixed_S - 1)) : b * a.fixed_S;
+        g.S = sh_q0 ? 1 : a.fixed_S;
+        g.S = g.S < SMAX ? g.S : SMAX;
+        g.q0 = sh && !sh_q0 ? 1 : 0;
+        g.mb = sh_q0 ? 0 : b;
+        g.sh = sh;
+        return g;
+    };
+    auto row_of = [](const Pair& g, int j) { return g.sh && j == 0 ? 0 : g.r0 + j; };
+    auto fetch = [&](const Pair& g, SetPipeRegs& r) {
+#pragma unroll
+        for (int t = 0; t < 2; ++t) {
+            const int j = 4 * t + rsub;
+            r.q[t] = f32x4{0.f, 0.f, 0.f, 0.f}; r.k[t] = r.q[t];
+            if (j < g.S) {
+                const float* rp = (const float*)a.qkv + (size_t)row_of(g, j) * 3 * D + g.h * 64 + c4;
+                if (j >= g.q0) r.q[t] = *(const f32x4*)rp;
+                r.k[t] = *(const f32x4*)(rp + D);
+            }
+        }
+#pragma unroll
+        for (int j = 0; j < SMAX; ++j) r.v[j] = j < g.S ? ((const float*)a.qkv)[(size_t)row_of(g, j) * 3 * D + 2 * D + g.h * 64 + lane] : 0.f;
+        r.mk = 1;
+        if (a.key_mask && lane < g.S) r.mk = a.key_mask[(size_t)g.mb * a.mask_ld + lane];
+    };
+    float vreg[SMAX];
+    unsigned dead_keys = 0;
+    auto stage = [&](const Pair& g, const SetPipeRegs& r) {
+#pragma unroll
+        for (int t = 0; t < 2; ++t) {
+            const int j = 4 * t + rsub;
+            if (j < g.S) {
+                if (j >= g.q0) *(f32x4*)(qs + j * STR + c4) = r.q[t];
+                *(f32x4*)(ks + j * STR + c4) = r.k[t];
+            }
+        }
+#pragma unroll
+        for (int j = 0; j < SMAX; ++j) vreg[j] = r.v[j];
+        dead_keys = (unsigned)__ballot(r.mk == 0);
+    };
+    SetPipeRegs nx;
+    Pair cur = pair_of(first);
+    fetch(cur, nx);
+    stage(cur, nx);
+    for (int p = first; p < end; ++p) {
+        const bool has_next = p + 1 < end;
+        Pair nxt = cur;
+        if (has_next) { nxt = pair_of(p + 1); fetch(nxt, nx); }
+        asm volatile("s_waitcnt lgkmcnt(0)" ::: "memory");
+        const int S = cur.S, q0 = cur.q0, nq = cur.S, h = cur.h;
+        for (int e = lane; e < (nq - q0) * S; e += 64) {
+            const int i = q0 + e / S, j = e % S;
+            const float d = sa8_dot(qs + i * STR, ks + j * STR);
+            bool dead = a.causal && j > i;
+            if (!dead) dead = (dead_keys >> j) & 1;
+            sc[i * SCS + j] = dead ? -INFINITY : d * a.scale;
+        }
+        asm volatile("s_waitcnt lgkmcnt(0)" ::: "memory");
+        if (lane >= q0 && lane < nq) {
+            float* row = sc + lane * SCS;
+            float m = -INFINITY;
+            for (int j = 0; j < S; ++j) m = fmaxf(m, row[j]);
+            if (m == -INFINITY) m = 0.f;
+            float sum = 0.f;
+            for (int j = 0; j < S; ++j) { const float e = expf(row[j] - m); row[j] = e; sum += e; }
+            const float inv = sum > 0.f ? 1.0f / sum : 0.f;
+            for (int j = 0; j < S; ++j) row[j] *= inv;
+        }
+        asm volatile("s_waitcnt lgkmcnt(0)" ::: "memory");
+        if (a.out_kind == 0) {
+            for (int i = q0; i < nq; ++i) ((float*)a.out)[(size_t)row_of(cur, i) * a.ldo + h * 64 + lane] = sa8_pv(sc + i * SCS, vreg, S);
+            asm volatile("s_waitcnt lgkmcnt(0)" ::: "memory");
+            if (has_next) stage(nxt, nx);
+        } else {
+            for (int i = q0; i < nq; ++i) qs[i * STR + lane] = sa8_pv(sc + i * SCS, vreg, S);
+            asm volatile("s_waitcnt lgkmcnt(0)" ::: "memory");
+            const int c8 = (lane & 7) * 8, i = lane >> 3;
+            const bool mine = i >= q0 && i < nq;
+            f32x4 x0 = {0.f, 0.f, 0.f, 0.f}, x1 = x0;
+            if (mine) { x0 = *(const f32x4*)(qs + i * STR + c8); x1 = *(const f32x4*)(qs + i * STR + c8 + 4); }
+            asm volatile("s_waitcnt lgkmcnt(0)" ::: "memory");
+            if (has_next) stage(nxt, nx);
+            if (mine) store8<T, true>(a.out, (size_t)row_of(cur, i) * a.ldo + h * 64 + c8, x0, x1, a.out_kind, D);
+        }
+        cur = nxt;
     }
 }
 
@@ -498,7 +639,8 @@
     const bool wide = g.D == g.n_head * 96;
     OFX_REQUIRE(g.max_len >= 1 && g.max_len <= 64, OFX_ESHAPE, "set_attention: %d rows per sequence exceed 64", g.max_len);
     OFX_REQUIRE(g.max_len <= 32 || !g.drop.thresh, OFX_ESHAPE, "set_attention: dropout columns are keyed query * 32 + key");
-    OFX_REQUIRE(g.ldo >= (g.out_kind == 2 ? 3 * g.D : g.D) && (g.out_kind == 0 || g.ldo % 8 == 0), OFX_ESHAPE, "set_attention: bad ldo=%d (operand-type rows leave as 16-byte stores)", g.ldo);
+    OFX_REQUIRE(g.out_kind >= 0 && g.out_kind <= 3, OFX_ESHAPE, "set_attention: out_kind=%d", g.out_kind);
+    OFX_REQUIRE(g.ldo >= (g.out_kind >= 2 ? 3 * g.D : g.D) && (g.out_kind == 0 || g.ldo % 8 == 0), OFX_ESHAPE, "set_attention: bad ldo=%d (operand-type rows leave as 16-byte stores)", g.ldo);
     OFX_REQUIRE(g.cu_seqlens || (g.fixed_len >= 1 && g.fixed_len <= g.max_len), OFX_EINVAL, "set_attention: needs cu_seqlens or a fixed length <= max_len");
     SetK k;
     k.qkv = g.qkv; k.out = (char*)g.out; k.cu = g.cu_seqlens; k.nseq = g.nseq; k.n_head = g.n_head; k.D = g.D; k.ldo = g.ldo;
@@ -511,6 +653,13 @@
     k.splits = g.splits > 1 ? g.splits : 1; k.plane = g.plane; k.bias = g.bias;
     const int grid = (g.nseq + (g.shared_first ? 1 : 0)) * g.n_head;
     ProfScope prof(PROF_ATTN, s);
+    if (g_attn_pipe && !g.cu_seqlens && !g.qkv_op && !wide && g.splits <= 1 && !g.drop.thresh && !g.only_row0 && g.fixed_len <= 8) {
+        const int blocks = attn_pipe_grid(grid, device_cu_count(), g_attn_pipe == 1 ? 4 : g_attn_pipe);
+        if (op_dtype == OFX_F16) hipLaunchKernelGGL((set_attention_pipe_kernel<f16_t>), dim3(blocks), dim3(64 * ATTN_PIPE_WAVES), 0, s, k);
+        else hipLaunchKernelGGL((set_attention_pipe_kernel<bf16_t>), dim3(blocks), dim3(64 * ATTN_PIPE_WAVES), 0, s, k);
+        OFX_LAUNCH_CHECK();
+        return OFX_OK;
+    }
 #define SA(T, N) do { if (wide) { if (g.qkv_op) hipLaunchKernelGGL((set_attention_kernel<T, N, T, 96>), dim3(grid), dim3(64), 0, s, k); \
                                       else hipLaunchKernelGGL((set_attention_kernel<T, N, float, 96>), dim3(grid), dim3(64), 0, s, k); } \
                       else if (g.qkv_op) hipLaunchKernelGGL((set_attention_kernel<T, N, T>), dim3(grid), dim3(64), 0, s, k); \
diff --git a/outfitx_amd/csrc/attn_pairs.h b/outfitx_amd/csrc/attn_pairs.h
--- /dev/null
+++ b/outfitx_amd/csrc/attn_pairs.h
@@ -0,0 +1,22 @@
+#pragma once
+
+#if defined(__HIP__)
+#define OFX_PAIRS_FN __host__ __device__ inline __attribute__((always_inline))
+#else
+#define OFX_PAIRS_FN inline __attribute__((always_inline))
+#endif
+
+constexpr int ATTN_PIPE_WAVES = 4;
+
+OFX_PAIRS_FN void attn_pair_run(int block, int wave, int nblocks, int npairs, int& first, int& count) {
+    const int nw = nblocks * ATTN_PIPE_WAVES, g = block * ATTN_PIPE_WAVES + wave;
+    const int base = npairs / nw, rem = npairs % nw;
+    first = g * base + (g < rem ? g : rem);
+    count = base + (g < rem ? 1 : 0);
+}
+
+OFX_PAIRS_FN int attn_pipe_grid(int npairs, int cu_count, int per_cu) {
+    const int want = cu_count * per_cu, need = (npairs + ATTN_PIPE_WAVES - 1) / ATTN_PIPE_WAVES;
+    const int g = want < need ? want : need;
+    return g < 1 ? 1 : g;
+}
diff --git a/outfitx_amd/csrc/gemm.hip b/outfitx_amd/csrc/gemm.hip
--- a/outfitx_amd/csrc/gemm.hip
+++ b/outfitx_amd/csrc/gemm.hip
@@ -131,6 +131,18 @@
 }
 size_t ofx_gemm_splitk_bytes(int M, int N, int K) { return gemm_splitk_slab_bytes(M, N, K, g_knobs); }
 
+static GemmShape gemm_shape_of(const GemmArgs& g, int op_dtype) {
+    const bool producer = g.xb_out || g.stat_part || g.xlo;
+    GemmShape sh;
+    sh.M = g.M; sh.N = g.N; sh.K = g.K; sh.lda = g.lda; sh.a_wrap = g.a_wrap; sh.k_mult = g.k_mult;
+    sh.f16 = op_dtype == OFX_F16; sh.has_w8 = g.W8 && g.w8_scale; sh.has_m_dev = g.m_dev != nullptr;
+    sh.can_split = g.slab && !producer && !g.row_stat; sh.defer = g.defer_splits != nullptr;
+    sh.ln_fusable = g.ln_gamma && g.out_kind == 0 && g.act == OFX_ACT_NONE && !g.aux_out && !g.drop.thresh;
+    sh.out_kind = g.out_kind; sh.resid = g.resid != nullptr; sh.aux = g.aux_out != nullptr; sh.xlo = g.xlo != nullptr;
+    return sh;
+}
+int ofx_gemm_kind(const GemmArgs& g, int op_dtype) { return gemm_plan(gemm_shape_of(g, op_dtype), g_knobs, device_cu_count()).kind; }
+
 int ofx_launch_gemm(const GemmArgs& g, int op_dtype, hipStream_t s) {
     OFX_REQUIRE(g.M > 0 && g.N > 0 && g.K > 0, OFX_ESHAPE, "gemm: empty problem M=%d N=%d K=%d", g.M, g.N, g.K);
     OFX_REQUIRE(g.N % BN == 0, OFX_ESHAPE, "gemm: N=%d must be a multiple of %d (pad the weight at pack time)", g.N, BN);
@@ -138,7 +150,8 @@
     OFX_REQUIRE(g.a_wrap == 0 || (g.a_wrap > 0 && g.a_wrap % BK == 0 && g.K % g.a_wrap == 0), OFX_ESHAPE, "gemm: a_wrap=%d must be a multiple of %d dividing K=%d", g.a_wrap, BK, g.K);
     const int ka = g.a_wrap ? g.a_wrap : g.K;
     OFX_REQUIRE(g.lda >= ka && g.lda % 8 == 0, OFX_ESHAPE, "gemm: lda=%d must be >= K and a multiple of 8", g.lda);
-    OFX_REQUIRE(g.ldc % (g.out_kind == 0 ? 4 : 8) == 0 && g.ldc >= (g.out_kind == 2 ? 3 * g.N : g.N), OFX_ESHAPE, "gemm: bad ldc=%d", g.ldc);
+    OFX_REQUIRE(g.out_kind >= 0 && g.out_kind <= 3, OFX_ESHAPE, "gemm: out_kind=%d", g.out_kind);
+    OFX_REQUIRE(g.ldc % (g.out_kind == 0 ? 4 : 8) == 0 && g.ldc >= (g.out_kind >= 2 ? 3 * g.N : g.N), OFX_ESHAPE, "gemm: bad ldc=%d", g.ldc);
     OFX_REQUIRE(!g.resid || (g.ldr % 4 == 0 && g.ldr >= g.N), OFX_ESHAPE, "gemm: bad ldr=%d", g.ldr);
     OFX_REQUIRE(((uintptr_t)g.A % 16 == 0) && ((uintptr_t)g.W % 16 == 0) && ((uintptr_t)g.C % 16 == 0), OFX_EINVAL,
                 "gemm: operands must be 16-byte aligned");
@@ -154,13 +167,8 @@
     OFX_REQUIRE(!(g.row_stat || producer) || !g.resid, OFX_EINVAL, "gemm: LayerNorm folding takes no residual (a producer's stream is (xb_out, xlo))");
     OFX_REQUIRE(!producer || g.act == OFX_ACT_NONE, OFX_EINVAL, "gemm: a LayerNorm-fold producer has no activation");
 
-    GemmShape sh;
-    sh.M = g.M; sh.N = g.N; sh.K = g.K; sh.lda = g.lda; sh.a_wrap = g.a_wrap; sh.k_mult = g.k_mult;
-    sh.f16 = op_dtype == OFX_F16; sh.has_w8 = g.W8 && g.w8_scale; sh.has_m_dev = g.m_dev != nullptr;
-    sh.can_split = g.slab && !producer && !g.row_stat; sh.defer = g.defer_splits != nullptr;
-    sh.ln_fusable = g.ln_gamma && g.out_kind == 0 && g.act == OFX_ACT_NONE && !g.aux_out && !g.drop.thresh;
-    sh.out_kind = g.out_kind; sh.resid = g.resid != nullptr; sh.aux = g.aux_out != nullptr; sh.xlo = g.xlo != nullptr;
-    const GemmPlan pl = gemm_plan(sh, g_knobs, device_cu_count());
+    const GemmPlan pl = gemm_plan(gemm_shape_of(g, op_dtype), g_knobs, device_cu_count());
+    OFX_REQUIRE(g.out_kind != 3 || pl.kind == GEMM_X3, OFX_EINVAL, "gemm: the [hi | lo | -] output (out_kind 3) exists in gemm_x3_kernel's epilogue only; this launch plans kind %d", pl.kind);
     if (pl.splits > 1) OFX_REQUIRE(g.slab_bytes >= (size_t)pl.splits * g.M * g.N * 4, OFX_EWORKSPACE, "gemm: split-K slab too small");
 
     if (g_ofx_prof_on) ofx_prof_set_tag(g.M, g.N, pl.k_logical, pl.kind, pl.kmul, pl.bytes);
diff --git a/outfitx_amd/csrc/gemm_common.h b/outfitx_amd/csrc/gemm_common.h
--- a/outfitx_amd/csrc/gemm_common.h
+++ b/outfitx_amd/csrc/gemm_common.h
@@ -123,7 +123,7 @@
 constexpr int EPI2_BYTES_PER_WAVE = 16 * 64 * 4;
 constexpr int EPI_CONST_BIAS = 128, EPI_CONST_CSUM = 256, EPI_CONST_BYTES_PER_WAVE = 2048;
 
-template <typename T, int ACT, int FOLD = 0, int RAMP = 0, int NP = 8, int JW = 4, int J0 = 0>
+template <typename T, int ACT, int FOLD = 0, int RAMP = 0, int NP = 8, int JW = 4, int J0 = 0, bool S2 = false>
 __device__ __forceinline__ void epilogue2(const KArgs& p, OFX_LDS char* ep, f32x4 (&acc)[NP][JW], int gm0, int gn0, int lane,
                                           OFX_LDS float* st = nullptr, OFX_LDS const float* cst = nullptr) {
     typedef typename OpT<T>::v8 v8;
@@ -246,7 +246,7 @@
 #pragma unroll
                         for (int e = 0; e < 4; ++e) { v0[e] += (float)h[e] + (float)l[e]; v1[e] += (float)h[4 + e] + (float)l[4 + e]; }
                     }
-                    store8<T>(p.C, (size_t)gm * p.ldc + gn, v0, v1, FOLD == 3 ? 1 : p.out_kind, p.N, FOLD == 3 ? p.xlo : nullptr);
+                    store8<T, S2>(p.C, (size_t)gm * p.ldc + gn, v0, v1, FOLD == 3 ? 1 : p.out_kind, p.N, FOLD == 3 ? p.xlo : nullptr);
                     if (FOLD == 3) {
                         const float ssum = row8_sum(((v0[0] + v0[1]) + (v0[2] + v0[3])) + ((v1[0] + v1[1]) + (v1[2] + v1[3])));
                         const float ssq = row8_sum(((v0[0] * v0[0] + v0[1] * v0[1]) + (v0[2] * v0[2] + v0[3] * v0[3])) +
@@ -325,29 +325,29 @@
 #undef OFX_EPD
 }
 
-template <typename T, int NP = 8, int JW = 4, int J0 = 0>
+template <typename T, int NP = 8, int JW = 4, int J0 = 0, bool S2 = false>
 __device__ __forceinline__ void epilogue2_dispatch(const KArgs& p, OFX_LDS char* ep, f32x4 (&acc)[NP][JW], int gm0, int gn0, int lane,
                                                    OFX_LDS float* st = nullptr, OFX_LDS const float* cst = nullptr) {
     if (p.row_stat) {
         switch (p.act) {
-            case OFX_ACT_QUICK_GELU: epilogue2<T, OFX_ACT_QUICK_GELU, 2, 0, NP, JW, J0>(p, ep, acc, gm0, gn0, lane, st, cst); break;
-            case OFX_ACT_GELU: epilogue2<T, OFX_ACT_GELU, 2, 0, NP, JW, J0>(p, ep, acc, gm0, gn0, lane, st, cst); break;
-            default: epilogue2<T, OFX_ACT_NONE, 2, 0, NP, JW, J0>(p, ep, acc, gm0, gn0, lane, st, cst); break;
+            case OFX_ACT_QUICK_GELU: epilogue2<T, OFX_ACT_QUICK_GELU, 2, 0, NP, JW, J0, S2>(p, ep, acc, gm0, gn0, lane, st, cst); break;
+            case OFX_ACT_GELU: epilogue2<T, OFX_ACT_GELU, 2, 0, NP, JW, J0, S2>(p, ep, acc, gm0, gn0, lane, st, cst); break;
+            default: epilogue2<T, OFX_ACT_NONE, 2, 0, NP, JW, J0, S2>(p, ep, acc, gm0, gn0, lane, st, cst); break;
         }
         return;
     }
     if (p.xlo) {
-        epilogue2<T, OFX_ACT_NONE, 3, 1, NP, JW, J0>(p, ep, acc, gm0, gn0, lane, nullptr, cst);
+        epilogue2<T, OFX_ACT_NONE, 3, 1, NP, JW, J0, S2>(p, ep, acc, gm0, gn0, lane, nullptr, cst);
         return;
     }
     switch (p.act) {
-        case OFX_ACT_QUICK_GELU: epilogue2<T, OFX_ACT_QUICK_GELU, 0, 0, NP, JW, J0>(p, ep, acc, gm0, gn0, lane, nullptr, cst); break;
-        case OFX_ACT_GELU: epilogue2<T, OFX_ACT_GELU, 0, 0, NP, JW, J0>(p, ep, acc, gm0, gn0, lane, nullptr, cst); break;
-        case OFX_ACT_MISH: epilogue2<T, OFX_ACT_MISH, 0, 0, NP, JW, J0>(p, ep, acc, gm0, gn0, lane, nullptr, cst); break;
-        case OFX_ACT_MISH_GRAD: epilogue2<T, OFX_ACT_MISH_GRAD, 0, 0, NP, JW, J0>(p, ep, acc, gm0, gn0, lane, nullptr, cst); break;
+        case OFX_ACT_QUICK_GELU: epilogue2<T, OFX_ACT_QUICK_GELU, 0, 0, NP, JW, J0, S2>(p, ep, acc, gm0, gn0, lane, nullptr, cst); break;
+        case OFX_ACT_GELU: epilogue2<T, OFX_ACT_GELU, 0, 0, NP, JW, J0, S2>(p, ep, acc, gm0, gn0, lane, nullptr, cst); break;
+        case OFX_ACT_MISH: epilogue2<T, OFX_ACT_MISH, 0, 0, NP, JW, J0, S2>(p, ep, acc, gm0, gn0, lane, nullptr, cst); break;
+        case OFX_ACT_MISH_GRAD: epilogue2<T, OFX_ACT_MISH_GRAD, 0, 0, NP, JW, J0, S2>(p, ep, acc, gm0, gn0, lane, nullptr, cst); break;
         default:
-            if (p.resid && p.out_kind == 0) epilogue2<T, OFX_ACT_NONE, 0, 1, NP, JW, J0>(p, ep, acc, gm0, gn0, lane, nullptr, cst);
-            else epilogue2<T, OFX_ACT_NONE, 0, 0, NP, JW, J0>(p, ep, acc, gm0, gn0, lane, nullptr, cst);
+            if (p.resid && p.out_kind == 0) epilogue2<T, OFX_ACT_NONE, 0, 1, NP, JW, J0, S2>(p, ep, acc, gm0, gn0, lane, nullptr, cst);
+            else epilogue2<T, OFX_ACT_NONE, 0, 0, NP, JW, J0, S2>(p, ep, acc, gm0, gn0, lane, nullptr, cst);
             break;
     }
 }
diff --git a/outfitx_amd/csrc/gemm_plan.h b/outfitx_amd/csrc/gemm_plan.h
--- a/outfitx_amd/csrc/gemm_plan.h
+++ b/outfitx_amd/csrc/gemm_plan.h
@@ -110,7 +110,7 @@
     p.k_logical = g.K / p.kmul;
     const double ab = kind == GEMM_X3 ? 2.0 * g.M * (g.K / 3) * 2 : 2.0 * g.M * (g.a_wrap ? g.a_wrap : g.K);
     const double wb = kind == GEMM_W2F8 ? 3.0 * g.N * g.a_wrap : (kind == GEMM_X3 ? 2.0 * g.N * (g.K / 3) * 2 : 2.0 * g.N * g.K);
-    double ob = g.out_kind == 0 ? 4.0 : (g.out_kind == 2 ? 6.0 : 2.0);
+    double ob = g.out_kind == 0 ? 4.0 : (g.out_kind == 2 ? 6.0 : (g.out_kind == 3 ? 4.0 : 2.0));
     if (g.xlo) ob = 8.0;
     else if (g.resid) ob += 4.0;
     if (g.aux) ob += 4.0;
diff --git a/outfitx_amd/csrc/gemm_x3.hip b/outfitx_amd/csrc/gemm_x3.hip
--- a/outfitx_amd/csrc/gemm_x3.hip
+++ b/outfitx_amd/csrc/gemm_x3.hip
@@ -96,7 +96,7 @@
         OFX_LDS char* ep = estage + wave * EPI2_BYTES_PER_WAVE;
         OFX_LDS float* st = nullptr;
         if (p.row_stat && p.out_kind != 0) st = (OFX_LDS float*)(estage + 8 * EPI2_BYTES_PER_WAVE + wave * 1024);
-        epilogue2_dispatch<T, 4, 4, 0>(p, ep, acc, m0 + wr * 64, n0 + wc * 64, ln, st);
+        epilogue2_dispatch<T, 4, 4, 0, true>(p, ep, acc, m0 + wr * 64, n0 + wc * 64, ln, st);
         if (!has_next) break;
         w.advance();
     }
diff --git a/outfitx_amd/csrc/norm_act.hip b/outfitx_amd/csrc/norm_act.hip
--- a/outfitx_amd/csrc/norm_act.hip
+++ b/outfitx_amd/csrc/norm_act.hip
@@ -31,7 +31,7 @@
         for (int c = 0; c < NCH; ++c) {
             const int col = (lane + 64 * c) * 4;
             const f32x4 g = *(const f32x4*)(a.gamma + col), b = *(const f32x4*)(a.beta + col);
-            store4<T>(a.y, (size_t)r * a.ldy + col, v[c] * rstd * g + b, a.out_kind, D);
+            store4<T, true>(a.y, (size_t)r * a.ldy + col, v[c] * rstd * g + b, a.out_kind, D);
         }
     }
 }
@@ -41,7 +41,8 @@
 int ofx_launch_layernorm_dev(const LnArgs& a, const int* rows_dev, int op_dtype, hipStream_t s) {
     OFX_REQUIRE(a.D == 512 || a.D == 768 || a.D == 1024 || a.D == 1536, OFX_ESHAPE, "layernorm: D=%d not in {512,768,1024,1536}", a.D);
     OFX_REQUIRE(a.rows > 0, OFX_ESHAPE, "layernorm: rows=%d", a.rows);
-    OFX_REQUIRE(a.ldy % 4 == 0 && a.ldy >= (a.out_kind == 2 ? 3 * a.D : a.D), OFX_ESHAPE, "layernorm: bad ldy=%d", a.ldy);
+    OFX_REQUIRE(a.out_kind >= 0 && a.out_kind <= 3, OFX_ESHAPE, "layernorm: out_kind=%d", a.out_kind);
+    OFX_REQUIRE(a.ldy % 4 == 0 && a.ldy >= (a.out_kind >= 2 ? 3 * a.D : a.D), OFX_ESHAPE, "layernorm: bad ldy=%d", a.ldy);
     int grid = (a.rows + 3) / 4;
     if (grid > 8192) grid = 8192;
     ProfScope prof(PROF_NORM, s);
@@ -85,7 +86,7 @@
         for (int i = 0; i < nw; ++i) tq += part[1][i];
         const float rstd = rsqrtf(tq * (1.0f / D) + a.eps);
         const f32x4 g = *(const f32x4*)(a.gamma + col), b = *(const f32x4*)(a.beta + col);
-        store4<T>(a.y, (size_t)r * a.ldy + col, t * rstd * g + b, a.out_kind, D);
+        store4<T, true>(a.y, (size_t)r * a.ldy + col, t * rstd * g + b, a.out_kind, D);
         __syncthreads();
     }
 }
@@ -94,7 +95,8 @@
 int ofx_launch_splitk_reduce_ln(const SplitKLnArgs& a, int op_dtype, hipStream_t s, bool in_gemm_scope) {
     OFX_REQUIRE(splitk_reduce_ln_width_ok(a.D), OFX_ESHAPE, "splitk_reduce_ln: D=%d not in {512,768,1024,1536}", a.D);
     OFX_REQUIRE(a.rows > 0 && a.splits >= 1 && a.ldx % 4 == 0 && a.ldx >= a.D && (!a.resid || (a.ldr % 4 == 0 && a.ldr >= a.D)), OFX_ESHAPE, "splitk_reduce_ln: bad shape");
-    OFX_REQUIRE(a.ldy % 4 == 0 && a.ldy >= (a.out_kind == 2 ? 3 * a.D : a.D), OFX_ESHAPE, "splitk_reduce_ln: bad ldy=%d", a.ldy);
+    OFX_REQUIRE(a.out_kind >= 0 && a.out_kind <= 3, OFX_ESHAPE, "splitk_reduce_ln: out_kind=%d", a.out_kind);
+    OFX_REQUIRE(a.ldy % 4 == 0 && a.ldy >= (a.out_kind >= 2 ? 3 * a.D : a.D), OFX_ESHAPE, "splitk_reduce_ln: bad ldy=%d", a.ldy);
     const int grid = a.rows > 8192 ? 8192 : a.rows;
     ProfScope prof(PROF_NORM, s, 0.0, false, !in_gemm_scope);
     if (a.D > 1024) {
diff --git a/outfitx_amd/csrc/ofx_common.h b/outfitx_amd/csrc/ofx_common.h
--- a/outfitx_amd/csrc/ofx_common.h
+++ b/outfitx_amd/csrc/ofx_common.h
@@ -69,7 +69,7 @@
 
 template <typename T>
 __device__ __forceinline__ T lo_of(float v, T hi) { return (T)(v - (float)hi); }
-template <typename T, int NV>
+template <typename T, int NV, bool S2 = false>
 __device__ __forceinline__ void store_cols(void* y, size_t off, const f32x4 (&v)[NV], int out_kind, int D, void* ylo = nullptr) {
     typedef T vt __attribute__((ext_vector_type(4 * NV)));
     if (out_kind == 0) {
@@ -82,23 +82,26 @@
     for (int e = 0; e < 4 * NV; ++e) hi[e] = (T)v[e >> 2][e & 3];
     T* p = (T*)y + off;
     *(vt*)p = hi;
-    if (out_kind == 2 || ylo) {
+    if (out_kind == 2 || (S2 && out_kind == 3) || ylo) {
         vt lo;
 #pragma unroll
         for (int e = 0; e < 4 * NV; ++e) lo[e] = lo_of<T>(v[e >> 2][e & 3], hi[e]);
         if (ylo) *(vt*)((T*)ylo + off) = lo;
-        else { *(vt*)(p + D) = lo; *(vt*)(p + 2 * D) = hi; }
-    }
-}
-template <typename T>
+        else {
+            *(vt*)(p + D) = lo;
+            if (!S2 || out_kind == 2) *(vt*)(p + 2 * D) = hi;
+        }
+    }
+}
+template <typename T, bool S2 = false>
 __device__ __forceinline__ void store4(void* y, size_t off, f32x4 v, int out_kind, int D, void* ylo = nullptr) {
     const f32x4 vs[1] = {v};
-    store_cols<T, 1>(y, off, vs, out_kind, D, ylo);
-}
-template <typename T>
+    store_cols<T, 1, S2>(y, off, vs, out_kind, D, ylo);
+}
+template <typename T, bool S2 = false>
 __device__ __forceinline__ void store8(void* y, size_t off, f32x4 v0, f32x4 v1, int out_kind, int D, void* ylo = nullptr) {
     const f32x4 vs[2] = {v0, v1};
-    store_cols<T, 2>(y, off, vs, out_kind, D, ylo);
+    store_cols<T, 2, S2>(y, off, vs, out_kind, D, ylo);
 }
 
 __device__ __forceinline__ float act_quick_gelu(float u) { return u * __builtin_amdgcn_rcpf(1.0f + __builtin_amdgcn_exp2f(-2.4554669595930157f * u)); }
@@ -274,6 +277,7 @@
     bool* ln_done = nullptr;
 };
 int ofx_launch_gemm(const GemmArgs& g, int op_dtype , hipStream_t s);
+int ofx_gemm_kind(const GemmArgs& g, int op_dtype);
 size_t ofx_gemm_splitk_bytes(int M, int N, int K);
 int ofx_gemm_tune(int knob, int value);
 
@@ -409,3 +413,4 @@
                           hipStream_t s);
 
 extern int g_topk_filter;
+extern int g_attn_pipe;
diff --git a/outfitx_amd/engine.py b/outfitx_amd/engine.py
--- a/outfitx_amd/engine.py
+++ b/outfitx_amd/engine.py
@@ -329,6 +329,8 @@
         shared = lengths.shared_first if isinstance(lengths, TextLengths) else shared_first_row(ids, att)
         ids_d, att_d = self.stage_tokens(ids, att)
         N, T = ids_d.shape
+        if out.dim() != 2 or out.shape[0] < N:
+            raise ValueError(f"text: out holds {tuple(out.shape)} for {N} texts")
         Tc = T if lengths is None else max(1, min(T, max(int(v) for v in lengths)))
         arr = None if lengths is None else (C.c_int * N)(*[int(v) for v in lengths])
         nb = self.ws_bytes(L.OP_TEXT, N, Tc)
```

After: 8174 (median of 6 runs). No clear change (+0.7%).
